# nonl4331/raytracing-rust

Hardware: AMD Instinct MI355X
Metric: Msamples/s on rtweekend1.ssml 1920x1080x1024spp (higher is better)
Workload: dtype f32

## Files before the change

### include/rt_hip.h

```cpp
#ifndef RT_HIP_H
#define RT_HIP_H

#include <stdint.h>

#ifdef __cplusplus
extern "C" {
#endif

#define RT_ABI_VERSION 2u

typedef enum rt_status {
	RT_OK = 0,
	RT_ERR_INVALID_ARGUMENT = -1,
	RT_ERR_NO_DEVICE = -2,
	RT_ERR_HIP = -3,
	RT_ERR_OUT_OF_MEMORY = -4,
	RT_ERR_UNSUPPORTED = -5
} rt_status;

typedef enum rt_texture_type {
	RT_TEX_CHECKERED = 0,
	RT_TEX_SOLID = 1,
	RT_TEX_IMAGE = 2,
	RT_TEX_LERP = 3,
// ... 113 lines not shown
	uint32_t max_depth;
	uint32_t rr_threshold;
	uint32_t shard_index;
	uint32_t shard_count;
	uint32_t tile_width;
	uint32_t tile_height;
	int32_t output_layout;
	uint32_t sample_split;
	uint32_t reserved0;
} rt_render_opts;

void rt_render_opts_default(rt_render_opts *opts);

typedef struct rt_hit_record {
	float t;
	float point[3];
	float error[3];
	float normal[3];
	float uv[2];
	int32_t has_uv;
	int32_t out;
	uint32_t material;
	uint32_t found;
	uint64_t index;
} rt_hit_record;

typedef struct rt_ray_desc {
	float origin[3];
	float direction[3];
} rt_ray_desc;

typedef struct rt_bvh_node {
	float min[3];
	float max[3];
	int64_t children[2];
	uint64_t primitive_offset;
	uint64_t number_primitives;
} rt_bvh_node;

typedef struct rt_scene rt_scene;

const char *rt_last_error(void);
uint32_t rt_abi_version(void);
int rt_device_count(void);

int rt_camera_new(rt_camera *out, const float origin[3], const float lookat[3], const float vup[3],
                  float fov_degrees, float aspect_ratio, float aperture, float focus_dist);

int rt_scene_create(const rt_scene_desc *desc, int device, rt_scene **out);
#define RT_DEVICE_NONE (-1)
void rt_scene_destroy(rt_scene *scene);

int rt_scene_create_multi(const rt_scene_desc *desc, const int *devices, uint32_t n_devices, rt_scene **out);
int rt_scene_device_count(const rt_scene *scene, uint32_t *n_devices);
typedef enum rt_gather_mode { RT_GATHER_NONE = 0, RT_GATHER_RCCL = 1, RT_GATHER_PEER = 2, RT_GATHER_PEER_STAGED = 3, RT_GATHER_SAME_DEVICE = 4 } rt_gather_mode;
int rt_scene_gather_info(const rt_scene *scene, int *mode, char *note, uint64_t note_capacity);
int rt_rccl_probe(int *usable, char *note, uint64_t note_capacity);
int rt_scene_auto_sample_split(const rt_scene *scene, const rt_render_opts *opts, uint32_t *split);

int rt_scene_counts(const rt_scene *scene, uint64_t *n_nodes, uint64_t *n_primitives, uint64_t *n_lights);
int rt_scene_get_nodes(const rt_scene *scene, rt_bvh_node *out, uint64_t capacity);
int rt_scene_get_primitive_order(const rt_scene *scene, uint64_t *out, uint64_t capacity);
int rt_scene_get_lights(const rt_scene *scene, uint64_t *out, uint64_t capacity);
int rt_scene_wide_info(const rt_scene *scene, uint64_t *n_wide_nodes, uint32_t *root_ref, uint32_t *stack_depth);
int rt_scene_get_wide_nodes(const rt_scene *scene, void *out, uint64_t capacity_nodes);
int rt_scene_get_leaf_boxes(const rt_scene *scene, float *out, uint64_t capacity_slots);
int rt_scene_get_wide_nodes_compact(const rt_scene *scene, void *out, uint64_t capacity_nodes);
int rt_scene_get_leaf_boxes_compact(const rt_scene *scene, float *out, uint64_t capacity_leaves, uint64_t *n_leaves);

typedef struct rt_sky_info {
	uint32_t res_x, res_y;
	uint32_t guide_k;
	uint32_t inv_res_ok;
	float inv_res_x, inv_res_y;
	uint64_t table_bytes;
} rt_sky_info;
int rt_scene_sky_info(const rt_scene *scene, rt_sky_info *info);
int rt_scene_get_sky_tables(const rt_scene *scene, float *row_cdf, uint64_t capacity_rows, float *marginal_cdf, uint64_t capacity_marginal,
                            uint8_t *guide, uint64_t capacity_guide);

int rt_scene_set_traversal(rt_scene *scene, int mode);
typedef enum rt_tuning_key { RT_TUNE_TRAVERSAL = 0, RT_TUNE_FEATURE_SET = 1, RT_TUNE_SCENE_IN_LDS = 2, RT_TUNE_SCHEDULE = 3, RT_TUNE_WALK = 4,
                             RT_TUNE_STACK_CAP = 5, RT_TUNE_EXCHANGE = 6, RT_TUNE_WHOLE_PIXEL_SHARE = 7, RT_TUNE_RADIANCE_GROUPS = 8,
                             RT_TUNE_SKY_RUN = 10 } rt_tuning_key;
int rt_scene_set_tuning(rt_scene *scene, int key, int value);
int rt_plan_work_items(const rt_render_opts *opts, uint32_t split, int share, uint64_t resident_waves, uint32_t *whole_claims,
                       uint64_t *n_items);

int rt_render(rt_scene *scene, const rt_camera *camera, const rt_render_opts *opts, float *out_rgb,
              uint64_t *rays_shot);

int rt_render_device(rt_scene *scene, const rt_camera *camera, const rt_render_opts *opts, float *d_out_rgb,
                     uint64_t *d_rays_shot, void *hip_stream);

int rt_render_output_floats(const rt_render_opts *opts, uint64_t *n_floats);
int rt_shard_pixel_order(const rt_render_opts *opts, uint64_t *out, uint64_t capacity);

typedef struct rt_sampler_progress {
	uint64_t samples_completed;
	uint64_t rays_shot;
	const float *current_image;
	uint64_t n_floats;
} rt_sampler_progress;
typedef int (*rt_presentation_update)(void *data, const rt_sampler_progress *progress, uint64_t samples_done);
int rt_sample_image(rt_scene *scene, const rt_camera *camera, const rt_render_opts *opts, uint64_t batch,
                    rt_presentation_update update, void *data);

int rt_last_kernel_ms(rt_scene *scene, float *ms, uint32_t *n_launches);

typedef struct rt_launch_info {
	int32_t method;
	int32_t pruned;
	int32_t fine;
	int32_t sky_in_lds;
	int32_t scene_in_lds;
	int32_t feature_set;
	uint32_t block_threads;
	uint32_t n_blocks;
	uint32_t blocks_per_cu;
	uint32_t waves_per_simd;
	uint32_t lds_bytes;
	uint32_t n_cus;
	uint32_t sample_split;
	uint32_t whole_claims;
	uint64_t n_items;
	uint32_t sky_run;
	uint32_t reserved;
	char kernel[152];
} rt_launch_info;
int rt_last_launch_info(const rt_scene *scene, rt_launch_info *out);

int rt_output_rgb8(const float *rgb, uint64_t n_values, float gamma, uint8_t *out);
int rt_output_save(const char *filename, const float *rgb, uint32_t width, uint32_t height, float gamma);

int rt_output_rgb8_device(rt_scene *scene, const float *d_rgb, uint64_t n_values, float gamma, uint8_t *d_out, void *hip_stream);
int rt_render_rgb8(rt_scene *scene, const rt_camera *camera, const rt_render_opts *opts, float gamma, uint8_t *out_rgb8,
                   uint64_t *rays_shot);

int rt_check_hit(rt_scene *scene, const rt_ray_desc *rays, uint64_t n_rays, rt_hit_record *out);
int rt_check_hit_index(rt_scene *scene, const rt_ray_desc *rays, const uint64_t *object_index, uint64_t n_rays,
                       rt_hit_record *out);

typedef struct rt_radiance_opts {
	uint64_t seed, sample_begin;
	uint32_t samples_per_ray;
	int32_t  render_method;
	uint32_t max_depth;
	uint32_t rr_threshold;
	uint32_t reserved[2];
} rt_radiance_opts;
int rt_radiance_opts_default(rt_radiance_opts *out);
int rt_radiance(rt_scene *scene, const rt_ray_desc *rays, const uint64_t *streams , uint64_t n_rays,
                const rt_radiance_opts *opts, float *out_rgb);
int rt_radiance_device(rt_scene *scene, const rt_ray_desc *d_rays, const uint64_t *d_streams , uint64_t n_rays,
                       const rt_radiance_opts *opts, float *d_out_rgb, void *hip_stream);

typedef struct rt_aov_buffers {
	float *albedo;
	float *normal;
	float *depth;
	float *coverage;
	uint32_t *primitive;
	uint32_t *material;
} rt_aov_buffers;
int rt_render_aov(rt_scene *scene, const rt_camera *camera, const rt_render_opts *opts, const rt_aov_buffers *host_out);
int rt_render_aov_device(rt_scene *scene, const rt_camera *camera, const rt_render_opts *opts, const rt_aov_buffers *device_out,
                         void *hip_stream);
// ... 266 lines not shown
	uint32_t reserved[6];
} rt_bloom_opts;
int rt_bloom_opts_default(rt_bloom_opts *out);
int rt_bloom_workspace_bytes(const rt_bloom_opts *opts, uint64_t *bytes);
int rt_bloom_device(rt_scene *scene, const float *d_rgb, const rt_bloom_opts *opts, const rt_display_state *d_state, void *d_workspace,
                    float *d_out, void *hip_stream);
int rt_bloom(rt_scene *scene, const float *host_rgb, const rt_bloom_opts *opts, const rt_display_state *host_state, float *host_out);

typedef struct rt_upscale_opts {
	uint32_t src_width, src_height;
	uint32_t dst_width, dst_height;
	float sigma_normal;
	float depth_tolerance;
	uint32_t reserved[8];
} rt_upscale_opts;
typedef struct rt_upscale_inputs {
	const float *color;
	const float *src_albedo, *src_normal, *src_depth;
	const float *dst_albedo, *dst_normal, *dst_depth;
} rt_upscale_inputs;
int rt_upscale_opts_default(rt_upscale_opts *out);
int rt_upscale_device(rt_scene *scene, const rt_upscale_inputs *device_in, const rt_upscale_opts *opts, float *d_out, uint8_t *d_stage,
                      void *hip_stream);
int rt_upscale(rt_scene *scene, const rt_upscale_inputs *host_in, const rt_upscale_opts *opts, float *host_out, uint8_t *host_stage);
int rt_render_upscaled(rt_scene *scene, const rt_camera *camera, const rt_render_opts *opts, uint32_t src_width, uint32_t src_height,
                       const rt_denoise_opts *dopts, const rt_upscale_opts *uopts, float *out, float *out_src, uint64_t *rays_shot);

int rt_selftest_division(float divisor, float *reciprocal, int *exact);

#define RT_SELFTEST_LEAN_CLASSES 9
int rt_selftest_lean(int device, uint64_t n_per_thread, uint64_t seed, uint64_t mismatches[RT_SELFTEST_LEAN_CLASSES]);

enum {
	RT_SHORT_FORM_RCP_REFINED = 0,
	RT_SHORT_FORM_INV_ONE_PAIR = 1,
	RT_SHORT_FORM_INV_TWO_PAIRS = 2,
	RT_SHORT_FORM_SQRT_RAW = 3,
	RT_SHORT_FORM_SQRT_BOTH = 4
};
#define RT_SHORT_FORMS 5
enum { RT_SHORT_SITE_RAY_NEW_PAIR = 0, RT_SHORT_SITE_RAY_NEW_FULL = 1 };
#define RT_SHORT_SITES 2
typedef struct rt_short_form_count {
	uint64_t tested;
	uint64_t mismatches;
	uint32_t first_mismatch;
	uint32_t reserved;
} rt_short_form_count;
typedef struct rt_short_forms_result {
	rt_short_form_count form[RT_SHORT_FORMS];
	uint64_t sqrt_raw_exact, sqrt_raw_high, sqrt_raw_low, sqrt_raw_other;
	uint64_t site_tested;
	uint64_t site_mismatches[RT_SHORT_SITES];
	uint32_t in_use;
	uint32_t reserved;
} rt_short_forms_result;
int rt_selftest_short_forms(int device, const float *operands, uint64_t n_operands, rt_short_forms_result *out);

enum { RT_DIV_FORM_ONE_PAIR = 0, RT_DIV_FORM_TWO_PAIRS = 1 };
#define RT_DIV_FORMS 2
enum { RT_DIV_SITE_FIX = 0, RT_DIV_SITE_DIV3_FIX = 1, RT_DIV_SITE_MIS_LIGHT_TERM = 2, RT_DIV_SITE_ATAN2 = 3 };
#define RT_DIV_SITES 4
typedef struct rt_div_forms_slice {
	const uint32_t *denominators;
	uint64_t n_denominators;
	uint32_t first_denominator;
	uint32_t reserved;
	const int32_t *exponents;
	uint64_t n_exponent_pairs;
} rt_div_forms_slice;
typedef struct rt_div_forms_result {
	uint64_t tested;
	uint64_t mismatches[RT_DIV_FORMS];
	uint32_t first_numerator[RT_DIV_FORMS];
	uint32_t first_denominator[RT_DIV_FORMS];
	uint64_t site_tested;
	uint64_t site_in_domain;
	uint64_t site_mismatches[RT_DIV_SITES];
	uint32_t in_use;
	uint32_t reserved;
} rt_div_forms_result;
int rt_selftest_div_forms(int device, const rt_div_forms_slice *slice, const float *operands, uint64_t n_operand_pairs, rt_div_forms_result *out);
int rt_selftest_sky_pdf_forms(rt_scene *scene, const float *dirs, uint64_t m, float *out_pdf_pair, float *out_pdf_default);

enum { RT_FRAME_FORMS_TESTED = 0, RT_FRAME_FORMS_FRAME_MISMATCHES = 1, RT_FRAME_FORMS_FRAME_SHORT = 2, RT_FRAME_FORMS_FRAME_PLAIN = 3,
       RT_FRAME_FORMS_RAY_MISMATCHES = 4, RT_FRAME_FORMS_RAY_SHORT = 5, RT_FRAME_FORMS_RAY_PLAIN = 6, RT_FRAME_FORMS_IN_USE = 7 };
#define RT_FRAME_FORMS_COUNTS 8
enum { RT_FRAME_FORM_FRAME_SHORT = 0, RT_FRAME_FORM_RAY_NORM_ONE_PAIR = 1 };
int rt_selftest_frame_forms(int device, const float *vectors, uint64_t n_vectors, uint64_t counts[RT_FRAME_FORMS_COUNTS]);

enum { RT_GEN_KEYS_TESTED = 0, RT_GEN_KEYS_STATE_MISMATCHES = 1, RT_GEN_KEYS_DRAW_MISMATCHES = 2, RT_GEN_KEYS_ITEM_STATE_MISMATCHES = 3,
       RT_GEN_KEYS_ITEM_DRAW_MISMATCHES = 4, RT_GEN_KEYS_ZERO_BLOCKS = 5, RT_GEN_KEYS_IN_USE = 6 };
#define RT_GEN_KEYS_COUNTS 7
#define RT_GEN_KEYS_CASE_WORDS 4
enum { RT_GEN_KEYS_FORM_TABLE = 0, RT_GEN_KEYS_FORM_ITEM_PRODUCT = 1 };
int rt_selftest_gen_keys(int device, uint64_t seed, const uint32_t *cases, uint64_t n_cases, uint64_t counts[RT_GEN_KEYS_COUNTS]);
void rt_philox_round_keys(uint64_t seed, uint32_t keys[20]);

enum { RT_PAIR_SHADOW_TESTED = 0, RT_PAIR_SHADOW_MISMATCHES = 1, RT_PAIR_SHADOW_ASKED_MISMATCHES = 2, RT_PAIR_SHADOW_ASKED = 3 };
#define RT_PAIR_SHADOW_COUNTS 4
#define RT_PAIR_SHADOW_CASE_FLOATS 10
int rt_selftest_pair_shadow(int device, const float *cases, uint64_t n_cases, uint64_t counts[RT_PAIR_SHADOW_COUNTS]);
enum { RT_PAIR_SHADOW_WALK_TESTED = 0, RT_PAIR_SHADOW_WALK_MISMATCHES = 1, RT_PAIR_SHADOW_WALK_ASKED = 2, RT_PAIR_SHADOW_WALK_ASKED_BOTH = 3,
       RT_PAIR_SHADOW_WALK_ASKED_WITH_OCCLUDED = 4 };
#define RT_PAIR_SHADOW_WALK_COUNTS 5
#define RT_PAIR_SHADOW_WALK_CASE_FLOATS 16
int rt_selftest_pair_shadow_walk(int device, const float *cases, uint64_t n_cases, uint64_t counts[RT_PAIR_SHADOW_WALK_COUNTS]);

int rt_selftest_pair_primary(rt_scene *scene, const float origin[3], uint32_t *valid, uint64_t *mismatches);

int rt_selftest_sky_tiles(rt_scene *scene, const rt_camera *camera, const rt_render_opts *opts, uint8_t *out_flags, uint64_t n_tiles);

int rt_selftest_sky(rt_scene *scene, int tables_in_lds, uint64_t seed, uint64_t n, float *out_dirs, float *out_pdf_of_sample,
                    const float *dirs, uint64_t m, float *out_pdf);

#ifdef __cplusplus
}
#endif
#endif
```

### raytracing-rust_amd/abi.py

```python
import ctypes as C

RT_ABI_VERSION = 2
RT_GATHER_NONE, RT_GATHER_RCCL, RT_GATHER_PEER, RT_GATHER_PEER_STAGED, RT_GATHER_SAME_DEVICE = 0, 1, 2, 3, 4

RT_OK = 0
RT_ERR_INVALID_ARGUMENT = -1
RT_ERR_NO_DEVICE = -2
RT_ERR_HIP = -3
RT_ERR_OUT_OF_MEMORY = -4
RT_ERR_UNSUPPORTED = -5

RT_TEX_CHECKERED, RT_TEX_SOLID, RT_TEX_IMAGE, RT_TEX_LERP, RT_TEX_PERLIN = range(5)
RT_MAT_EMIT, RT_MAT_LAMBERTIAN, RT_MAT_TROWBRIDGE_REITZ, RT_MAT_REFLECT, RT_MAT_REFRACT = range(5)
RT_PRIM_SPHERE, RT_PRIM_TRIANGLE, RT_PRIM_MESH_TRIANGLE = range(3)
RT_SPLIT_SAH, RT_SPLIT_MIDDLE, RT_SPLIT_EQUAL_COUNTS = range(3)
RT_METHOD_NAIVE, RT_METHOD_MIS = range(2)
RT_LAYOUT_FRAME, RT_LAYOUT_SHARD = range(2)
RT_TUNE_TRAVERSAL, RT_TUNE_FEATURE_SET, RT_TUNE_SCENE_IN_LDS, RT_TUNE_SCHEDULE, RT_TUNE_WALK, RT_TUNE_STACK_CAP, RT_TUNE_EXCHANGE, RT_TUNE_WHOLE_PIXEL_SHARE = range(8)
RT_TUNE_RADIANCE_GROUPS = 8
RT_TUNE_SKY_RUN = 10

NO_INDEX = 0xFFFFFFFFFFFFFFFF
RT_DEVICE_NONE = -1

f32x3 = C.c_float * 3


class TextureDesc(C.Structure):
    _fields_ = [
        ("type", C.c_int32),
        ("colour_one", f32x3),
        ("colour_two", f32x3),
        ("image_rgb", C.POINTER(C.c_float)),
        ("image_width", C.c_uint32),
        ("image_height", C.c_uint32),
        ("perlin_ran_vecs", C.POINTER(C.c_float)),
        ("perlin_perm", C.POINTER(C.c_uint32)),
    ]


class MaterialDesc(C.Structure):
    _fields_ = [
        ("type", C.c_int32),
        ("texture", C.c_uint32),
        ("param", C.c_float),
        ("ior", f32x3),
        ("metallic", C.c_float),
    ]


class _Sphere(C.Structure):
    _fields_ = [("centre", f32x3), ("radius", C.c_float)]


class _MeshTriangle(C.Structure):
    _fields_ = [("mesh", C.c_uint32), ("point_indices", C.c_uint32 * 3), ("normal_indices", C.c_uint32 * 3)]


class _Triangle(C.Structure):
    _fields_ = [("data", C.c_uint64)]


class _PrimUnion(C.Union):
    _fields_ = [("sphere", _Sphere), ("mesh_triangle", _MeshTriangle), ("triangle", _Triangle)]


class PrimitiveDesc(C.Structure):
    _fields_ = [("type", C.c_int32), ("material", C.c_uint32), ("u", _PrimUnion)]


class TriangleData(C.Structure):
    _fields_ = [("points", C.c_float * 9), ("normals", C.c_float * 9)]


class MeshDesc(C.Structure):
    _fields_ = [
        ("vertices", C.POINTER(C.c_float)),
        ("n_vertices", C.c_uint64),
        ("normals", C.POINTER(C.c_float)),
        ("n_normals", C.c_uint64),
    ]


class SkyDesc(C.Structure):
    _fields_ = [
        ("texture", C.c_uint32),
        ("material", C.c_uint32),
        ("sampler_res_x", C.c_uint32),
        ("sampler_res_y", C.c_uint32),
    ]


class SceneDesc(C.Structure):
    _fields_ = [
        ("abi_version", C.c_uint32),
        ("n_textures", C.c_uint32),
        ("textures", C.POINTER(TextureDesc)),
        ("n_materials", C.c_uint32),
        ("n_meshes", C.c_uint32),
        ("materials", C.POINTER(MaterialDesc)),
        ("meshes", C.POINTER(MeshDesc)),
        ("n_primitives", C.c_uint64),
# ... 523 lines not shown
    "rt_sampler_progress": (SamplerProgressC, 32),
    "rt_launch_info": (LaunchInfo, 224),
    "rt_sky_info": (SkyInfo, 32),
    "rt_aov_buffers": (AovBuffers, 48),
    "rt_aov_chain_opts": (AovChainOpts, 32),
    "rt_aov_chain_buffers": (AovChainBuffers, 56),
    "rt_matte_opts": (MatteOpts, 32),
    "rt_matte_buffers": (MatteBuffers, 24),
    "rt_ao_opts": (AoOpts, 32),
    "rt_ao_buffers": (AoBuffers, 16),
    "rt_radiance_opts": (RadianceOpts, 40),
    "rt_noise_opts": (NoiseOpts, 32),
    "rt_noise_summary": (NoiseSummary, 16),
    "rt_noise_buffers": (NoiseBuffers, 40),
    "rt_noise_result": (NoiseResult, 40),
    "rt_adaptive_result": (AdaptiveResult, 40),
    "rt_lens_camera": (LensCamera, 100),
    "rt_robust_opts": (RobustOpts, 32),
    "rt_robust_buffers": (RobustBuffers, 40),
    "rt_denoise_opts": (DenoiseOpts, 48),
    "rt_denoise_inputs": (DenoiseInputs, 40),
    "rt_temporal_opts": (TemporalOpts, 96),
    "rt_temporal_inputs": (TemporalInputs, 32),
    "rt_display_opts": (DisplayOpts, 104),
    "rt_display_state": (DisplayState, 16),
    "rt_bloom_opts": (BloomOpts, 64),
    "rt_dof_opts": (DofOpts, 64),
    "rt_upscale_opts": (UpscaleOpts, 56),
    "rt_upscale_inputs": (UpscaleInputs, 56),
    "rt_short_form_count": (ShortFormCount, 24),
    "rt_short_forms_result": (ShortFormsResult, 184),
    "rt_div_forms_slice": (DivFormsSlice, 40),
    "rt_div_forms_result": (DivFormsResult, 96),
}

EXPORTED_SYMBOLS = [
    "rt_last_error",
    "rt_abi_version",
    "rt_device_count",
    "rt_render_opts_default",
    "rt_camera_new",
    "rt_scene_create",
    "rt_scene_create_multi",
    "rt_scene_device_count",
    "rt_scene_destroy",
    "rt_scene_counts",
    "rt_scene_get_nodes",
    "rt_scene_get_primitive_order",
    "rt_scene_get_lights",
    "rt_scene_wide_info",
    "rt_scene_get_wide_nodes",
    "rt_scene_get_leaf_boxes",
    "rt_scene_get_wide_nodes_compact",
    "rt_scene_auto_sample_split",
    "rt_scene_gather_info",
    "rt_rccl_probe",
    "rt_selftest_division",
    "rt_scene_get_leaf_boxes_compact",
    "rt_scene_sky_info",
    "rt_scene_get_sky_tables",
    "rt_scene_set_traversal",
    "rt_scene_set_tuning",
    "rt_render",
    "rt_sample_image",
    "rt_render_device",
    "rt_render_output_floats",
    "rt_shard_pixel_order",
    "rt_plan_work_items",
    "rt_last_kernel_ms",
    "rt_last_launch_info",
    "rt_output_rgb8",
    "rt_output_save",
    "rt_output_rgb8_device",
    "rt_render_rgb8",
    "rt_check_hit",
    "rt_check_hit_index",
    "rt_radiance_opts_default",
    "rt_radiance",
    "rt_radiance_device",
    "rt_selftest_lean",
    "rt_selftest_short_forms",
    "rt_selftest_div_forms",
    "rt_selftest_sky_pdf_forms",
    "rt_selftest_frame_forms",
    "rt_selftest_gen_keys",
    "rt_philox_round_keys",
    "rt_selftest_pair_shadow",
    "rt_selftest_pair_shadow_walk",
    "rt_selftest_pair_primary",
    "rt_selftest_sky_tiles",
    "rt_selftest_sky",
    "rt_render_aov",
    "rt_render_aov_device",
    "rt_aov_chain_opts_default",
    "rt_render_aov_chain",
    "rt_render_aov_chain_device",
    "rt_matte_opts_default",
    "rt_render_matte",
    "rt_render_matte_device",
    "rt_matte_extract",
    "rt_matte_extract_device",
    "rt_ao_opts_default",
    "rt_render_ao",
    "rt_render_ao_device",
    "rt_denoise_opts_default",
    "rt_denoise_workspace_bytes",
    "rt_denoise",
    "rt_denoise_device",
    "rt_render_denoised",
    "rt_noise_opts_default",
    "rt_render_noise",
    "rt_render_noise_device",
    "rt_noise_tiles",
    "rt_noise_tiles_device",
    "rt_render_converged",
    "rt_render_denoised_split",
    "rt_render_adaptive",
    "rt_render_tiles",
    "rt_render_tiles_device",
    "rt_noise_select_tiles",
    "rt_noise_select_tiles_device",
    "rt_lens_camera_new",
    "rt_render_lens",
    "rt_render_lens_device",
    "rt_robust_opts_default",
    "rt_render_robust",
    "rt_render_robust_device",
    "rt_robust_combine",
    "rt_robust_combine_device",
    "rt_render_denoised_robust",
    "rt_temporal_opts_default",
    "rt_temporal_history_bytes",
    "rt_temporal_workspace_bytes",
    "rt_denoise_temporal_device",
    "rt_denoise_temporal",
    "rt_denoise_temporal_reset",
    "rt_display_opts_default",
    "rt_display_workspace_bytes",
    "rt_display_output_bytes",
    "rt_display_device",
    "rt_display",
    "rt_display_reset",
    "rt_bloom_opts_default",
    "rt_bloom_workspace_bytes",
    "rt_bloom_device",
    "rt_bloom",
    "rt_dof_opts_default",
    "rt_dof_opts_from_camera",
    "rt_dof_workspace_bytes",
    "rt_dof_device",
    "rt_dof",
    "rt_render_dof",
    "rt_upscale_opts_default",
    "rt_upscale_device",
    "rt_upscale",
    "rt_render_upscaled",
]


def channels(table, struct):
    out = {}
    for name, shape in table.items():
        if isinstance(shape, dict):
            out.update(channels(shape, getattr(struct, name)))
        else:
            out[name] = (struct, dict(struct._fields_)[name]._type_, shape)
# ... 56 lines not shown
```

### raytracing-rust_amd/csrc/rt_api.cpp

```cpp
#include <hip/hip_runtime.h>

#include <cstdio>
#include <cstdlib>
#include <algorithm>
#include <cmath>
#include <cstring>
#include <string>
#include <vector>

#include "../../include/rt_hip.h"
#include "../../include/rt_detmath.h"
#include <dlfcn.h>
#include "rt_api_internal.h"
#include "rt_render.h"

using namespace rt;

thread_local std::string g_error;

constexpr uint32_t kFineAboveTriangles = 4096;
constexpr uint32_t kFineAboveSpheres = 32768;

struct RcclApi {
	void *lib = nullptr;
// ... 204 lines not shown
				return bail(rc);
		}
	}
	if ((rc = upload(s, h.dev_nodes.data(), h.dev_nodes.size(), &D.nodes)) != RT_OK) return bail(rc);
	if (!h.dev_nodes4.empty()) {
		if ((rc = upload(s, h.dev_nodes4c.data(), h.dev_nodes4c.size(), &D.nodes4)) != RT_OK) return bail(rc);
		if ((rc = upload(s, h.leaf_box_c.data(), h.leaf_box_c.size(), &D.leaf_box)) != RT_OK) return bail(rc);
	}
	if ((rc = upload(s, h.dev_prims.data(), h.dev_prims.size(), &D.prims)) != RT_OK) return bail(rc);
	if ((rc = upload(s, h.dev_shade.data(), h.dev_shade.size(), &D.shade)) != RT_OK) return bail(rc);
	if ((rc = upload(s, h.prim_rank.data(), h.prim_rank.size(), &D.prim_rank)) != RT_OK) return bail(rc);
	if (&h == &s->host && h.primitive_order.size() < 0xFFFFFFFFull) {
		std::vector<uint32_t> desc(h.primitive_order.size());
		for (size_t i = 0; i < desc.size(); ++i)
			desc[i] = (uint32_t)h.primitive_order[i];
		const uint32_t *d_desc = nullptr;
		if ((rc = upload(s, desc.data(), desc.size(), &d_desc)) != RT_OK) return bail(rc);
		s->d_prim_desc = const_cast<uint32_t *>(d_desc);
	}
	{
		const uint32_t *d_big = nullptr;
		if ((rc = upload(s, h.big_leaves.data(), h.big_leaves.size(), &d_big)) != RT_OK) return bail(rc);
		D.big_leaves = reinterpret_cast<const uint2 *>(d_big);
	}
	if ((rc = upload(s, h.materials.data(), h.materials.size(), &D.materials)) != RT_OK) return bail(rc);
	if ((rc = upload(s, textures.data(), textures.size(), &D.textures)) != RT_OK) return bail(rc);
	if ((rc = upload(s, h.dev_lights.data(), h.dev_lights.size(), &D.lights)) != RT_OK) return bail(rc);
	const float *d_sky = nullptr;
	if ((rc = upload(s, h.sky_cdf.data(), h.sky_cdf.size(), &d_sky)) != RT_OK) return bail(rc);
	const uint8_t *d_guide = nullptr;
	if ((rc = upload(s, h.sky_guide.data(), h.sky_guide.size(), &d_guide)) != RT_OK) return bail(rc);
	{
		auto pad16 = [](size_t n) { return (n + 15) & ~(size_t)15; };
		const size_t sizes[8] = {h.dev_nodes.size() * sizeof(DevNode),      h.dev_prims.size() * sizeof(DevPrim),
		                         h.dev_shade.size() * sizeof(DevShade),     h.prim_rank.size() * 4,
		                         h.materials.size() * sizeof(DevMaterial),  textures.size() * sizeof(DevTexture),
		                         h.dev_lights.size() * 4,                   h.big_leaves.size() * 4};
		const void *srcs[8] = {h.dev_nodes.data(), h.dev_prims.data(), h.dev_shade.data(), h.prim_rank.data(),
		                       h.materials.data(), textures.data(),  h.dev_lights.data(), h.big_leaves.data()};
		size_t total = 0;
		for (int i = 0; i < 8; ++i) {
			blob_off[i] = (uint32_t)total;
			total += pad16(sizes[i]);
		}
		if (total <= 12 * 1024) {
			blob.assign(total / 4, 0u);
			for (int i = 0; i < 8; ++i)
				if (sizes[i])
					std::memcpy(reinterpret_cast<char *>(blob.data()) + blob_off[i], srcs[i], sizes[i]);
			if ((rc = upload(s, blob.data(), blob.size(), &D.blob)) != RT_OK) return bail(rc);
			D.blob_bytes = (uint32_t)total;
			D.off_nodes = blob_off[0]; D.off_prims = blob_off[1]; D.off_shade = blob_off[2]; D.off_rank = blob_off[3];
			D.off_materials = blob_off[4]; D.off_textures = blob_off[5]; D.off_lights = blob_off[6]; D.off_big_leaves = blob_off[7];
		}
	}

	D.n_nodes = (uint32_t)h.dev_nodes.size();
	D.n_prims = (uint32_t)h.dev_prims.size();
	D.n_lights = (uint32_t)h.dev_lights.size();
	D.n_materials = (uint32_t)h.materials.size();
	D.n_textures = (uint32_t)h.textures.size();
	D.root_ref = h.root_ref;
	D.root4_ref = h.root4_ref;
	D.n_nodes4 = (uint32_t)h.dev_nodes4.size();
	std::memcpy(D.root_min, h.root_min, sizeof D.root_min);
	std::memcpy(D.root_max, h.root_max, sizeof D.root_max);
	D.stack_depth = h.stack_depth;
	s->stack_depth_narrow = h.stack_depth_narrow;
	D.has_triangles = h.has_triangles ? 1u : 0u;
	D.single_light = h.dev_lights.size() == 1 ? h.dev_lights[0] : kNoPrim;
	D.sky.texture = h.sky.texture;
	D.sky.material = mat_handle_make(h.sky.material, h.materials[h.sky.material].type, h.materials[h.sky.material].tex_type);
	D.sky.res_x = h.sky.sampler_res_x;
	D.sky.res_y = h.sky.sampler_res_y;
	D.sky.row_cdf = d_sky;
	D.sky.marginal_cdf = d_sky + (size_t)h.sky.sampler_res_y * (h.sky.sampler_res_x + 1u);
	D.sky.guide = h.sky_guide_k ? d_guide : nullptr;
	D.sky.guide_k = h.sky_guide_k;
	{
		float rc_pi = 0.0f, rc_tau = 0.0f;
		if (!verified_reciprocal(RT_PI, &rc_pi) || !verified_reciprocal(RT_TAU, &rc_tau) || rc_pi != 1.0f / RT_PI || rc_tau != 1.0f / RT_TAU)
			return bail(fail(RT_ERR_UNSUPPORTED, "self-check failed: division by pi / 2 pi through their reciprocals is not exact on this host (the kernels assume it)"));
		sky_reciprocals(h.sky, &D.sky.inv_res_ok, &D.sky.inv_res_x, &D.sky.inv_res_y);
		bool tame = true;
		for (const DevMaterial &m : h.materials) {
			if (m.type != RT_MAT_LAMBERTIAN)
				continue;
			tame = tame && m.tex_type == RT_TEX_SOLID;
			for (int k = 0; k < 3; ++k) {
				const float pr = std::fabs(m.tex_c1[k] * m.param);
				tame = tame && (pr == 0.0f || (pr >= 0x1p-30f && pr <= 0x1p30f));
			}
		}
		for (const DevShade &sh : h.dev_shade)
			for (int k = 0; k < 3; ++k)
				tame = tame && std::fabs(sh.n0[k]) <= 0x1p20f && std::fabs(sh.n1[k]) <= 0x1p20f && std::fabs(sh.n2[k]) <= 0x1p20f;
		D.lambert_tame = tame ? 1u : 0u;
	}

	void *p = nullptr;
	if (hipMalloc(&p, sizeof(uint32_t)) != hipSuccess) return bail(fail(RT_ERR_OUT_OF_MEMORY, "hipMalloc work counter"));
	s->allocations.push_back(p);
	s->d_work_counter = static_cast<uint32_t *>(p);
	if (hipMalloc(&p, sizeof(unsigned long long)) != hipSuccess) return bail(fail(RT_ERR_OUT_OF_MEMORY, "hipMalloc rays"));
	s->allocations.push_back(p);
	s->d_rays = static_cast<unsigned long long *>(p);
	if (hipStreamCreate(&s->stream) != hipSuccess) return bail(fail(RT_ERR_HIP, "hipStreamCreate failed"));
	if (hipEventCreate(&s->ev_start) != hipSuccess || hipEventCreate(&s->ev_stop) != hipSuccess)
		return bail(fail(RT_ERR_HIP, "hipEventCreate failed"));
	{
		bool cmat = false, ctex = false;
		for (const DevMaterial &m : h.materials)
			cmat = cmat || (m.type != RT_MAT_EMIT && m.type != RT_MAT_LAMBERTIAN);
		for (const DevTexture &t : textures)
			ctex = ctex || (t.type != RT_TEX_SOLID && t.type != RT_TEX_LERP);
		if (cmat || ctex)
			s->feature_set = 2;
		else if (h.has_triangles || !h.lights.empty())
			s->feature_set = 1;
		else
			s->feature_set = 0;
		s->min_feature_set = s->feature_set;
		if (h.dev_nodes.size() == 1 && (h.root_ref & kLeafFlag) == 0u) {
			const DevNode &n0 = h.dev_nodes[0];
			s->pair_tree = (n0.c0 & kLeafFlag) && (n0.c1 & kLeafFlag) && ((n0.c0 >> 26) & 31u) == 1u && ((n0.c1 >> 26) & 31u) == 1u;
			for (const DevPrim &q : h.dev_prims) {
				uint32_t meta;
				std::memcpy(&meta, &q.a[3], sizeof meta);
				const DevMaterial &m = h.materials[mat_handle_index(meta >> 2)];
				s->pair_tree = s->pair_tree && m.type == RT_MAT_LAMBERTIAN && m.tex_type == RT_TEX_SOLID;
			}
			s->pair_tree = s->pair_tree && h.materials[h.sky.material].type == RT_MAT_EMIT;
			s->pair_tree = s->pair_tree && D.lambert_tame != 0u;
			for (const DevPrim &q : h.dev_prims)
				s->pair_tree = s->pair_tree && q.b[1] != 0.0f;
			if (s->pair_tree) {
				DevPairScene &q = s->pair;
				std::memcpy(q.c0min, n0.c0min, sizeof q.c0min); std::memcpy(q.c0max, n0.c0max, sizeof q.c0max);
				std::memcpy(q.c1min, n0.c1min, sizeof q.c1min); std::memcpy(q.c1max, n0.c1max, sizeof q.c1max);
				q.slot0 = n0.c0 & kLeafSlotMask;
				q.slot1 = n0.c1 & kLeafSlotMask;
				q.rank0 = h.prim_rank[q.slot0];
				q.rank1 = h.prim_rank[q.slot1];
				const uint32_t slots[2] = {q.slot0, q.slot1};
				for (int k = 0; k < 2; ++k) {
					const DevPrim &pr = h.dev_prims[slots[k]];
					uint32_t meta;
					std::memcpy(&meta, &pr.a[3], sizeof meta);
					const DevMaterial &m = h.materials[mat_handle_index(meta >> 2)];
					q.sphere[k][0] = pr.a[0]; q.sphere[k][1] = pr.a[1]; q.sphere[k][2] = pr.a[2]; q.sphere[k][3] = pr.b[0];
					q.lambert[k][0] = m.tex_c1[0]; q.lambert[k][1] = m.tex_c1[1]; q.lambert[k][2] = m.tex_c1[2]; q.lambert[k][3] = m.param;
				}
				q.inv_radius[0] = h.dev_prims[q.slot0].b[1];
				q.inv_radius[1] = h.dev_prims[q.slot1].b[1];
				const DevMaterial &sky = h.materials[h.sky.material];
				q.sky_param = sky.param;
				q.sky_tex_type = sky.tex_type;
				std::memcpy(q.sky_c1, sky.tex_c1, sizeof q.sky_c1);
				std::memcpy(q.sky_c2, sky.tex_c2, sizeof q.sky_c2);
			}
		}
	}
	if (const char *e = std::getenv("RT_HIP_TRAVERSAL")) {
		if (std::strcmp(e, "exhaustive") == 0) s->traversal_mode = 0;
		if (std::strcmp(e, "pruned") == 0) s->traversal_mode = 1;
	}
// ... 202 lines not shown
	}
	return RT_OK;
}

int rt_scene_device_count(const rt_scene *s, uint32_t *n_devices)
{
	if (!s || !n_devices)
		return fail(RT_ERR_INVALID_ARGUMENT, "null argument");
	*n_devices = s->device == RT_DEVICE_NONE ? 0u : (uint32_t)(1 + s->peers.size());
	return RT_OK;
}

int rt_scene_set_traversal(rt_scene *s, int mode)
{
	if (!s || mode < -1 || mode > 1)
		return fail(RT_ERR_INVALID_ARGUMENT, "bad arguments");
	s->traversal_mode = mode;
	for (rt_scene *m : s->peers)
		m->traversal_mode = mode;
	return RT_OK;
}

static int set_tuning_one(rt_scene *s, int key, int value);
int rt_scene_set_tuning(rt_scene *s, int key, int value)
{
	if (!s)
		return fail(RT_ERR_INVALID_ARGUMENT, "null scene");
	const int rc = set_tuning_one(s, key, value);
	for (rt_scene *m : s->peers)
		if (rc == RT_OK) {
			(void)set_tuning_one(m, key, value);
		}
	return rc;
}
static int set_tuning_one(rt_scene *s, int key, int value)
{
	switch (key) {
	case RT_TUNE_TRAVERSAL:
		return rt_scene_set_traversal(s, value);
	case RT_TUNE_FEATURE_SET:
		if (value < s->min_feature_set || value > 2)
			return fail(RT_ERR_INVALID_ARGUMENT, "feature set must be between the scene's own and 2");
		s->feature_set = value;
		s->feature_set_forced = true;
		return RT_OK;
	case RT_TUNE_SCHEDULE:
		if (value < -1 || value > 1)
			return fail(RT_ERR_INVALID_ARGUMENT, "schedule must be -1, 0 or 1");
		s->schedule_mode = value;
		return RT_OK;
	case RT_TUNE_SCENE_IN_LDS:
		s->scene_lds_allowed = value != 0;
		return RT_OK;
	case RT_TUNE_STACK_CAP:
		if (value < 0 || value > 96)
			return fail(RT_ERR_INVALID_ARGUMENT, "stack cap must be 0 (automatic) or 1..96 entries");
		s->stack_cap_override = (uint32_t)value;
		return RT_OK;
	case RT_TUNE_EXCHANGE:
		if (value < 0 || value > 1)
			return fail(RT_ERR_INVALID_ARGUMENT, "exchange must be 0 (off) or 1 (on where the kernel has it)");
		s->exchange_mode = value;
		return RT_OK;
	case RT_TUNE_WHOLE_PIXEL_SHARE:
		if (value < -1 || value > 16)
			return fail(RT_ERR_INVALID_ARGUMENT, "whole-pixel share must be -1 (automatic) or 0..16 (sixteenths of a shard's tiles)");
		s->whole_share = value;
		return RT_OK;
	case RT_TUNE_WALK:
		if (value < 0 || value > 1)
			return fail(RT_ERR_INVALID_ARGUMENT, "walk must be 0 (automatic) or 1 (two-child walk for every ray)");
		s->dev.narrow_only = (uint32_t)value;
		return RT_OK;
	case RT_TUNE_RADIANCE_GROUPS:
		if (value < 0 || value > 65536)
			return fail(RT_ERR_INVALID_ARGUMENT, "radiance groups must be 0 (automatic) or 1..65536 workgroups");
		s->radiance_groups = (uint32_t)value;
		return RT_OK;
	case RT_TUNE_SKY_RUN:
		if (value < -1 || value > 1)
			return fail(RT_ERR_INVALID_ARGUMENT, "sky run must be -1 (automatic), 0 (off) or 1 (on where the kernel has it)");
		s->sky_run = value;
		return RT_OK;
	default:
		return fail(RT_ERR_INVALID_ARGUMENT, "unknown tuning key");
	}
}

int rt_scene_counts(const rt_scene *s, uint64_t *n_nodes, uint64_t *n_primitives, uint64_t *n_lights)
{
	if (!s)
		return fail(RT_ERR_INVALID_ARGUMENT, "null scene");
	if (n_nodes) *n_nodes = s->host.nodes.size();
	if (n_primitives) *n_primitives = s->host.primitive_order.size();
	if (n_lights) *n_lights = s->host.lights.size();
	return RT_OK;
}
int rt_scene_get_nodes(const rt_scene *s, rt_bvh_node *out, uint64_t capacity)
{
	if (!s || !out || capacity < s->host.nodes.size())
		return fail(RT_ERR_INVALID_ARGUMENT, "bad arguments");
	for (size_t i = 0; i < s->host.nodes.size(); ++i) {
		const HostNode &n = s->host.nodes[i];
		std::memcpy(out[i].min, n.min, 12);
		std::memcpy(out[i].max, n.max, 12);
		out[i].children[0] = n.child[0];
		out[i].children[1] = n.child[1];
		out[i].primitive_offset = n.primitive_offset;
		out[i].number_primitives = n.number_primitives;
	}
	return RT_OK;
}
int rt_scene_get_primitive_order(const rt_scene *s, uint64_t *out, uint64_t capacity)
{
	if (!s || !out || capacity < s->host.primitive_order.size())
		return fail(RT_ERR_INVALID_ARGUMENT, "bad arguments");
	std::memcpy(out, s->host.primitive_order.data(), s->host.primitive_order.size() * sizeof(uint64_t));
	return RT_OK;
}
int rt_scene_wide_info(const rt_scene *s, uint64_t *n_wide_nodes, uint32_t *root_ref, uint32_t *stack_depth)
{
	if (!s)
		return fail(RT_ERR_INVALID_ARGUMENT, "null scene");
	if (n_wide_nodes) *n_wide_nodes = s->host.dev_nodes4.size();
	if (root_ref) *root_ref = s->host.root4_ref;
	if (stack_depth) *stack_depth = s->host.stack_depth;
	return RT_OK;
}
int rt_scene_get_wide_nodes(const rt_scene *s, void *out, uint64_t capacity_nodes)
{
	if (!s || !out || capacity_nodes < s->host.dev_nodes4.size())
		return fail(RT_ERR_INVALID_ARGUMENT, "bad arguments");
	std::memcpy(out, s->host.dev_nodes4.data(), s->host.dev_nodes4.size() * sizeof(DevNodeQ4));
	return RT_OK;
}
int rt_scene_get_leaf_boxes(const rt_scene *s, float *out, uint64_t capacity_slots)
{
	if (!s || !out || capacity_slots < s->host.leaf_box.size())
		return fail(RT_ERR_INVALID_ARGUMENT, "bad arguments");
	std::memcpy(out, s->host.leaf_box.data(), s->host.leaf_box.size() * sizeof(DevLeafBox));
	return RT_OK;
}
int rt_scene_get_wide_nodes_compact(const rt_scene *s, void *out, uint64_t capacity_nodes)
{
	if (!s || !out || capacity_nodes < s->host.dev_nodes4c.size())
		return fail(RT_ERR_INVALID_ARGUMENT, "bad arguments");
	std::memcpy(out, s->host.dev_nodes4c.data(), s->host.dev_nodes4c.size() * sizeof(DevNodeQ4));
	return RT_OK;
}
int rt_scene_get_leaf_boxes_compact(const rt_scene *s, float *out, uint64_t capacity_leaves, uint64_t *n_leaves)
{
	if (!s)
		return fail(RT_ERR_INVALID_ARGUMENT, "null scene");
	if (n_leaves)
		*n_leaves = s->host.leaf_box_c.size();
	if (!out)
		return n_leaves ? RT_OK : fail(RT_ERR_INVALID_ARGUMENT, "bad arguments");
	if (capacity_leaves < s->host.leaf_box_c.size())
		return fail(RT_ERR_INVALID_ARGUMENT, "bad arguments");
	std::memcpy(out, s->host.leaf_box_c.data(), s->host.leaf_box_c.size() * sizeof(DevLeafBox));
	return RT_OK;
}
int rt_scene_sky_info(const rt_scene *s, rt_sky_info *info)
{
	if (!s || !info)
		return fail(RT_ERR_INVALID_ARGUMENT, "null argument");
// ... 540 lines not shown
				if (head->gather_mode == RT_GATHER_RCCL)
					HIP_TRY(hipStreamWaitEvent(stream, members[m]->ev_shard, 0));
				HIP_TRY(hipMemcpyPeerAsync(head->d_gather_rays + m, head->device, members[m]->d_member_rays, members[m]->device, sizeof(unsigned long long), stream));
			}
		}
		HIP_TRY(launch_sum_u64(stream, head->d_gather_rays, n, reinterpret_cast<unsigned long long *>(d_rays_shot)));
	}
	if (!capturing) {
		HIP_TRY(hipEventRecord(head->ev_gathered, stream));
		head->gathered_once = true;
	}
	return RT_OK;
}

int rt_render_device(rt_scene *s, const rt_camera *camera, const rt_render_opts *o, float *d_out_rgb, uint64_t *d_rays_shot,
                     void *hip_stream)
{
	if (!s || !camera || !o || !d_out_rgb)
		return fail(RT_ERR_INVALID_ARGUMENT, "null argument");
	if (!s->peers.empty() && !s->member_call) {
		if (s->device == RT_DEVICE_NONE)
			return fail(RT_ERR_NO_DEVICE, "host-only scene");
		return render_device_multi(s, camera, o, d_out_rgb, d_rays_shot, static_cast<hipStream_t>(hip_stream));
	}
	ShardGeometry g;
	int rc = shard_geometry(o, g);
	if (rc != RT_OK)
		return rc;
	if (s->device == RT_DEVICE_NONE)
		return fail(RT_ERR_NO_DEVICE, "host-only scene (RT_DEVICE_NONE): rendering needs a GPU, there is no CPU fallback");
	if (o->render_method != RT_METHOD_NAIVE && o->render_method != RT_METHOD_MIS)
		return fail(RT_ERR_INVALID_ARGUMENT, "unknown render method");
	if (o->samples_per_pixel == 0 || o->samples_per_pixel >= (1ull << 32))
		return fail(RT_ERR_INVALID_ARGUMENT, "samples_per_pixel must be in [1, 2^32)");
	if (o->output_layout != RT_LAYOUT_FRAME && o->output_layout != RT_LAYOUT_SHARD)
		return fail(RT_ERR_INVALID_ARGUMENT, "unknown output layout");
	HIP_TRY(hipSetDevice(s->device));
	hipStream_t stream = static_cast<hipStream_t>(hip_stream);
	if (g.n_work == 0) {
		HIP_TRY(launch_reset(stream, s->d_work_counter, reinterpret_cast<unsigned long long *>(d_rays_shot), d_out_rgb,
		                     o->output_layout == RT_LAYOUT_FRAME ? (size_t)(o->width * o->height * 3) : 0));
		s->timed = false;
		return RT_OK;
	}

	RenderLaunchPlan plan;
	rc = plan_render_launch(s, o, g, &plan);
	if (rc != RT_OK)
		return rc;
	const DevRenderParams &P = plan.P;
	float *render_target = d_out_rgb;
	if (plan.split > 1u) {
		const size_t need = (size_t)g.n_work * plan.split * 3;
		rc = grow_device_buffer(s->d_partial, s->partial_floats, need);
		if (rc != RT_OK)
			return rc;
		render_target = s->d_partial;
	}
	if (P.stack_ovf_depth != 0u) {
		const size_t need = (size_t)plan.n_blocks * plan.block_threads * P.stack_ovf_depth;
		rc = grow_device_buffer(s->d_stack_ovf, s->stack_ovf_words, need);
		if (rc != RT_OK)
			return rc;
	}
	{
		size_t zero_floats = 0;
		if (o->output_layout == RT_LAYOUT_FRAME && o->shard_count > 1)
			zero_floats = (size_t)(o->width * o->height * 3);
		if (o->output_layout == RT_LAYOUT_SHARD)
			zero_floats = (size_t)(g.n_work * 3);
		HIP_TRY(launch_reset(stream, s->d_work_counter, reinterpret_cast<unsigned long long *>(d_rays_shot), d_out_rgb, zero_floats));
	}
	fill_launch_info(plan, o, s->n_cus, &s->last_launch);
	const bool sky_run = sky_run_applies(s, plan.feature_set, g.n_work, P.tile_log2_w != 0xFFFFFFFFu);
	s->last_launch.sky_run = sky_run ? 1u : 0u;
	const DevCamera cam = dev_camera(camera);
	DevPairPrimary primary{};
	if (plan.feature_set == 3)
		pair_primary_terms(s->pair, plan.dev.root_min, plan.dev.root_max, v3(cam.origin[0], cam.origin[1], cam.origin[2]), primary);
	const DevSkyTiles sky_tiles = sky_tiles_block(s, primary, cam, (uint32_t)o->width, (uint32_t)o->height, sky_run);
	HIP_TRY(hipEventRecord(s->ev_start, stream));
	HIP_TRY(launch_render(o->render_method, plan.prune, plan.fine, plan.sky_lds, plan.feature_set, plan.n_blocks, plan.lds_bytes, stream, plan.dev, cam, P,
	                      render_target, reinterpret_cast<unsigned long long *>(d_rays_shot), s->d_work_counter, s->d_stack_ovf, plan.xchg,
	                      plan.feature_set == 3 ? &s->pair : nullptr, plan.feature_set == 3 ? &primary : nullptr, plan.block_threads, sky_tiles));
	HIP_TRY(hipEventRecord(s->ev_stop, stream));
	if (plan.split > 1u)
		HIP_TRY(launch_combine(stream, P, s->d_partial, d_out_rgb));
	s->timed = true;
	s->n_launches = 1;
	return RT_OK;
}

int rt_render(rt_scene *s, const rt_camera *camera, const rt_render_opts *o, float *out_rgb, uint64_t *rays_shot)
{
	if (!s || !camera || !o)
		return fail(RT_ERR_INVALID_ARGUMENT, "null argument");
	if (int rc = need_device(s); rc != RT_OK)
		return rc;
	uint64_t n_floats = 0;
	int rc = rt_render_output_floats(o, &n_floats);
	if (rc != RT_OK)
		return rc;
	if (n_floats == 0) {
		if (rays_shot)
			*rays_shot = 0;
		return RT_OK;
	}
	if (!out_rgb)
		return fail(RT_ERR_INVALID_ARGUMENT, "null argument");
	HIP_TRY(hipSetDevice(s->device));
	rc = ensure_frame_buffers(s, n_floats, false);
	if (rc != RT_OK)
		return rc;
	float *d_out = s->d_prog[0];
	rc = rt_render_device(s, camera, o, d_out, reinterpret_cast<uint64_t *>(s->d_rays), s->stream);
	if (rc != RT_OK)
		return rc;
	Staging st{s};
	st.download(out_rgb, d_out, n_floats * sizeof(float));
	st.download(rays_shot, s->d_rays, sizeof(uint64_t));
	return st.finish("render");
}

int rt_output_rgb8_device(rt_scene *s, const float *d_rgb, uint64_t n_values, float gamma, uint8_t *d_out, void *hip_stream)
{
	if (!s || !d_rgb || !d_out)
		return fail(RT_ERR_INVALID_ARGUMENT, "null argument");
	if (s->device == RT_DEVICE_NONE)
		return fail(RT_ERR_NO_DEVICE, "host-only scene (RT_DEVICE_NONE): this call needs a GPU (rt_output_rgb8 is the host-side conversion)");
	if (n_values == 0)
		return RT_OK;
	HIP_TRY(hipSetDevice(s->device));
	HIP_TRY(launch_quantise(static_cast<hipStream_t>(hip_stream), d_rgb, (size_t)n_values, 1.0f / gamma, d_out));
	return RT_OK;
}

int rt_render_rgb8(rt_scene *s, const rt_camera *camera, const rt_render_opts *o, float gamma, uint8_t *out_rgb8, uint64_t *rays_shot)
{
	if (!s || !camera || !o)
		return fail(RT_ERR_INVALID_ARGUMENT, "null argument");
	if (int rc = need_device(s); rc != RT_OK)
		return rc;
	uint64_t n_values = 0;
	int rc = rt_render_output_floats(o, &n_values);
	if (rc != RT_OK)
		return rc;
	if (n_values == 0) {
		if (rays_shot)
			*rays_shot = 0;
		return RT_OK;
	}
	if (!out_rgb8)
		return fail(RT_ERR_INVALID_ARGUMENT, "null argument");
	HIP_TRY(hipSetDevice(s->device));
	rc = ensure_frame_buffers(s, n_values, false);
	if (rc != RT_OK)
		return rc;
	rc = grow_device_buffer(s->d_rgb8, s->d_rgb8_bytes, (size_t)n_values);
	if (rc != RT_OK)
		return rc;
	float *d_frame = s->d_prog[0];
	rc = rt_render_device(s, camera, o, d_frame, reinterpret_cast<uint64_t *>(s->d_rays), s->stream);
	if (rc != RT_OK)
		return rc;
	Staging st{s};
	st.e = launch_quantise(s->stream, d_frame, (size_t)n_values, 1.0f / gamma, s->d_rgb8);
	st.download(out_rgb8, s->d_rgb8, n_values);
// ... 116 lines not shown
```

### raytracing-rust_amd/csrc/rt_api_internal.h

```cpp
#pragma once
#include <hip/hip_runtime.h>

#include <cstdint>
#include <cstring>
#include <string>
#include <vector>

#include "../../include/rt_hip.h"
#include "rt_build.h"
#include "rt_layout.h"
#include "rt_types.h"
#include "rt_sky_tiles.h"

extern thread_local std::string g_error;

inline int fail(int code, const std::string &msg)
{
	g_error = msg;
	return code;
}
inline int hip_fail(hipError_t e, const char *what)
{
	g_error = std::string(what) + ": " + hipGetErrorString(e);
	return e == hipErrorOutOfMemory ? RT_ERR_OUT_OF_MEMORY : RT_ERR_HIP;
}
#define HIP_TRY(expr)                       \
	do {                                    \
		hipError_t e_ = (expr);             \
		if (e_ != hipSuccess)               \
			return hip_fail(e_, #expr);     \
	} while (0)
#define RT_TRY(expr)            \
	do {                        \
		const int rc_ = (expr); \
		if (rc_ != RT_OK)       \
			return rc_;         \
	} while (0)

constexpr uint32_t kPruneAbove = 100;

constexpr int kWholeShareDefault = -1;

struct rt_scene {
	int device = 0;
	rt::HostScene host;
	rt::DevScene dev{};
	std::vector<void *> allocations;
	hipStream_t stream = nullptr;
	uint32_t *d_work_counter = nullptr;
	unsigned long long *d_rays = nullptr;
	hipEvent_t ev_start = nullptr, ev_stop = nullptr;
	bool timed = false;
	uint32_t n_launches = 0;
	int n_cus = 0;
	int traversal_mode = -1;
	int schedule_mode = -1;
	int feature_set = 2;
	int min_feature_set = 0;
	bool pair_tree = false, feature_set_forced = false;
	rt::DevPairScene pair{};
	bool scene_lds_allowed = true;
	float *d_partial = nullptr;
	size_t partial_floats = 0;
	float *d_prog[2] = {nullptr, nullptr};
	float *h_prog[2] = {nullptr, nullptr};
	unsigned long long *d_prog_rays = nullptr;
	unsigned long long *h_prog_rays = nullptr;
	size_t d_prog_floats[2] = {0, 0}, h_prog_floats[2] = {0, 0};
	hipStream_t copy_stream = nullptr;
	hipEvent_t ev_batch[2] = {nullptr, nullptr}, ev_copy[2] = {nullptr, nullptr};
	size_t max_lds = 65536;
	rt_launch_info last_launch{};
	uint32_t stack_cap_override = 0;
	int exchange_mode = 0;
	int whole_share = kWholeShareDefault;
	uint32_t radiance_groups = 0;
	int sky_run = -1;
	uint32_t stack_depth_narrow = 2;
	uint32_t *d_stack_ovf = nullptr;
	size_t stack_ovf_words = 0;
	uint8_t *d_rgb8 = nullptr;
	size_t d_rgb8_bytes = 0;
	std::vector<rt_scene *> peers;
	bool member_call = false;
	float *d_shard = nullptr;
	size_t shard_floats = 0;
	unsigned long long *d_member_rays = nullptr;
	hipEvent_t ev_shard = nullptr;
	hipEvent_t ev_begin = nullptr;
	float *d_gather = nullptr;
	size_t gather_floats = 0;
	unsigned long long *d_gather_rays = nullptr;
	void *nccl_comms = nullptr;
	int gather_mode = 0;
	std::string gather_note;
	hipEvent_t ev_gathered = nullptr;
	bool gathered_once = false;
	uint32_t *d_prim_desc = nullptr;
	char *d_denoise = nullptr;
	size_t d_denoise_bytes = 0;
	char *d_temporal = nullptr;
	uint32_t temporal_w = 0, temporal_h = 0;
	int temporal_cur = -1;
	rt_camera temporal_prev{};
	char *d_display = nullptr;
	size_t d_display_bytes = 0;
	uint32_t display_w = 0, display_h = 0;
	bool display_has_state = false;
	char *d_noise = nullptr;
	size_t d_noise_bytes = 0;
	char *d_bloom = nullptr;
	size_t d_bloom_bytes = 0;
	char *d_dof = nullptr;
	size_t d_dof_bytes = 0;
};

uint32_t auto_sample_split(int n_cus, uint64_t frame_pixels, uint64_t spp, uint32_t n_sharers);
struct WorkItems { uint64_t whole_claims, n_items; };
WorkItems plan_work_items(uint64_t tiles, uint64_t tile_pixels, uint32_t split, bool tiled, int share, uint64_t resident_waves);

constexpr size_t kSkyLdsLimit = 96 * 1024;
inline size_t sky_table_bytes(uint32_t res_x, uint32_t res_y, uint32_t guide_k)
{
	if ((res_x | res_y) == 0u)
		return 0;
	return ((size_t)res_y * (res_x + 1u) + res_y + 1u) * 4 + (size_t)(res_y + 1u) * guide_k;
}

inline bool scene_prunes(const rt_scene *s)
{
	return s->traversal_mode == -1 ? s->dev.n_prims > kPruneAbove : s->traversal_mode == 1;
}

inline int four_wave_traversal(const rt_scene *s, bool *prune, rt::DevScene *dev)
{
	*prune = scene_prunes(s);
	*dev = s->dev;
	const bool walks_wide = *prune && dev->nodes4 != nullptr && dev->narrow_only == 0u;
	if (!walks_wide || rt::four_wave_stack_lds_bytes(*dev) > s->max_lds) {
		if (walks_wide)
			dev->narrow_only = 1u;
		dev->stack_depth = s->stack_depth_narrow;
	}
	if (rt::four_wave_stack_lds_bytes(*dev) > s->max_lds)
		return fail(RT_ERR_UNSUPPORTED, "traversal stacks exceed the LDS of one CU");
	return RT_OK;
}

inline uint32_t path_lane_groups(const rt_scene *s, size_t lds_bytes, uint32_t waves, uint64_t wanted)
{
	const uint64_t by_lds = std::max<uint64_t>(1, (160u * 1024u) / std::max<size_t>(1, lds_bytes));
	const uint64_t resident = (uint64_t)std::max(1, s->n_cus) * std::min<uint64_t>(waves, by_lds);
	uint64_t groups = std::min<uint64_t>(wanted, resident);
	if (s->radiance_groups != 0u)
		groups = std::min<uint64_t>(groups, s->radiance_groups);
	return (uint32_t)std::max<uint64_t>(groups, 1);
}


struct TileGrid { uint32_t tiles_x; uint64_t count; };
// ... 144 lines not shown
```

### raytracing-rust_amd/csrc/rt_api_query.cpp

```cpp
#include <hip/hip_runtime.h>

#include <algorithm>
#include <cstring>
#include <vector>

#include "../../include/rt_hip.h"
#include "rt_api_internal.h"
#include "rt_query.h"
#include "rt_radiance.h"
#include "rt_selftest.h"
#include "rt_gen_keys.h"

using namespace rt;

#ifdef RT_STATS
extern "C" int rt_debug_trace_queue(rt_scene *s, const rt_ray_desc *rays, uint64_t n, int waves, uint32_t cap, float *out_t, uint32_t *out_prim,
                                    float *ms, unsigned long long *node_steps)
{
	if (!s || !rays || !out_t || !out_prim || n == 0 || n >= (1ull << 31) || s->device == RT_DEVICE_NONE || s->dev.nodes4 == nullptr)
		return fail(RT_ERR_INVALID_ARGUMENT, "bad arguments (or no wide tree)");
	HIP_TRY(hipSetDevice(s->device));
	cap = std::min(std::max(cap, 1u), s->dev.stack_depth);
	const uint32_t ovf_depth = s->dev.stack_depth - cap;
	const uint32_t n_blocks = (uint32_t)s->n_cus * (uint32_t)waves;
// ... 304 lines not shown
	out->in_use = short_forms_in_use();
	return RT_OK;
}

int rt_selftest_div_forms(int device, const rt_div_forms_slice *slice, const float *operands, uint64_t n_operand_pairs, rt_div_forms_result *out)
{
	if (!out || (slice != nullptr) == (operands != nullptr))
		return fail(RT_ERR_INVALID_ARGUMENT, "bad arguments (a slice or operands, not both)");
	if (operands && (n_operand_pairs == 0 || n_operand_pairs > (1ull << 20)))
		return fail(RT_ERR_INVALID_ARGUMENT, "bad arguments (1 to 2^20 operand pairs)");
	if (slice) {
		if (!slice->exponents || slice->n_denominators == 0 || slice->n_exponent_pairs == 0 || slice->n_denominators > (1ull << 17) ||
		    slice->n_exponent_pairs > (1ull << 17) || slice->n_denominators * slice->n_exponent_pairs > (1ull << 17))
			return fail(RT_ERR_INVALID_ARGUMENT, "bad slice (n_denominators * n_exponent_pairs in [1, 2^17])");
		if (!slice->denominators && (uint64_t)slice->first_denominator + slice->n_denominators > (1ull << 23))
			return fail(RT_ERR_INVALID_ARGUMENT, "bad slice (the range leaves the 2^23 significands)");
		for (uint64_t k = 0; k < 2 * slice->n_exponent_pairs; ++k)
			if (slice->exponents[k] < -126 || slice->exponents[k] > 127)
				return fail(RT_ERR_INVALID_ARGUMENT, "bad slice (binary exponents in [-126, 127])");
	}
	unsigned long long host[kDivCounts] = {};
	for (int k = 0; k < RT_DIV_FORMS; ++k)
		host[kDivCountFirst + k] = ~0ull;
	if (operands) {
		RT_TRY(run_cases(device, operands, (size_t)n_operand_pairs * 2 * sizeof(float), host, kDivCounts, "selftest_div_forms",
		                 [&](unsigned long long *d, void *d_pairs) { return launch_div_sites(nullptr, static_cast<const float *>(d_pairs), n_operand_pairs, d); }));
	} else {
		const uint64_t n_den = slice->denominators ? slice->n_denominators : 0, n_exp = 2 * slice->n_exponent_pairs;
		std::vector<uint32_t> tail(n_exp + n_den);
		std::memcpy(tail.data(), slice->exponents, n_exp * sizeof(int32_t));
		if (n_den)
			std::memcpy(tail.data() + n_exp, slice->denominators, n_den * sizeof(uint32_t));
		RT_TRY(run_cases(device, tail.data(), tail.size() * sizeof(uint32_t), host, kDivCounts, "selftest_div_forms", [&](unsigned long long *d, void *d_tail) {
			DevDivForms D;
			D.exponents = static_cast<const int32_t *>(d_tail);
			D.n_exponent_pairs = (uint32_t)slice->n_exponent_pairs;
			D.denominators = n_den ? static_cast<const uint32_t *>(d_tail) + n_exp : nullptr;
			D.n_denominators = (uint32_t)slice->n_denominators;
			D.first_denominator = slice->first_denominator;
			D.counts = d;
			return launch_div_forms(nullptr, D);
		}));
	}
	std::memset(out, 0, sizeof *out);
	out->tested = host[kDivCountTested];
	for (int k = 0; k < RT_DIV_FORMS; ++k) {
		out->mismatches[k] = host[kDivCountBad + k];
		if (slice && out->mismatches[k]) {
			const unsigned long long index = host[kDivCountFirst + k];
			const uint64_t pair_index = index >> 23, ep = pair_index / slice->n_denominators, j = pair_index - ep * slice->n_denominators;
			const uint32_t d_sig = (slice->denominators ? slice->denominators[j] : slice->first_denominator + (uint32_t)j) & 0x007FFFFFu;
			out->first_numerator[k] = (uint32_t)(127 + slice->exponents[2 * ep]) << 23 | ((uint32_t)index & 0x007FFFFFu);
			out->first_denominator[k] = (uint32_t)(127 + slice->exponents[2 * ep + 1]) << 23 | d_sig;
		}
	}
	out->site_tested = host[kDivCountSiteTested];
	out->site_in_domain = host[kDivCountSiteInDomain];
	for (int k = 0; k < RT_DIV_SITES; ++k)
		out->site_mismatches[k] = host[kDivCountSiteBad + k];
	out->in_use = div_forms_in_use();
	return RT_OK;
}

int rt_selftest_sky_pdf_forms(rt_scene *s, const float *dirs, uint64_t m, float *out_pdf_pair, float *out_pdf_default)
{
	if (!s || !dirs || !out_pdf_pair || !out_pdf_default || m == 0 || m > (1ull << 24))
		return fail(RT_ERR_INVALID_ARGUMENT, "bad arguments (1 to 2^24 directions)");
	if ((s->host.sky.sampler_res_x | s->host.sky.sampler_res_y) == 0u)
		return fail(RT_ERR_INVALID_ARGUMENT, "the sky is not samplable (sampler_res 0 x 0)");
	if (int rc = need_device(s); rc != RT_OK)
		return rc;
	Layout L;
	const auto p_dirs = L.add<float>(3 * m), p_pair = L.add<float>(m), p_default = L.add<float>(m);
	RT_TRY(sky_buffer(s, L));
	Staging st{s};
	st.put(L, p_dirs, dirs);
	if (st.ok())
		st.e = launch_sky_pdf_forms(s->stream, s->dev, L.at(p_dirs), m, L.at(p_pair), L.at(p_default));
	st.get(out_pdf_pair, L, p_pair);
	st.get(out_pdf_default, L, p_default);
	return sky_finish(st, L, "selftest_sky_pdf_forms");
}

int rt_selftest_pair_shadow(int device, const float *cases, uint64_t n_cases, uint64_t counts[RT_PAIR_SHADOW_COUNTS])
{
	return run_case_table<RT_PAIR_SHADOW_COUNTS>(device, cases, n_cases, RT_PAIR_SHADOW_CASE_FLOATS * sizeof(float), counts, "selftest_pair_shadow",
	                                             launch_pair_shadow);
}
int rt_selftest_pair_shadow_walk(int device, const float *cases, uint64_t n_cases, uint64_t counts[RT_PAIR_SHADOW_WALK_COUNTS])
{
	return run_case_table<RT_PAIR_SHADOW_WALK_COUNTS>(device, cases, n_cases, RT_PAIR_SHADOW_WALK_CASE_FLOATS * sizeof(float), counts,
	                                                  "selftest_pair_shadow_walk", launch_pair_shadow_walk);
}
int rt_selftest_frame_forms(int device, const float *vectors, uint64_t n_vectors, uint64_t counts[RT_FRAME_FORMS_COUNTS])
{
	RT_TRY(run_case_table<RT_FRAME_FORMS_COUNTS>(device, vectors, n_vectors, 3 * sizeof(float), counts, "selftest_frame_forms", launch_frame_forms));
	counts[RT_FRAME_FORMS_IN_USE] = frame_forms_in_use();
	return RT_OK;
}
int rt_selftest_gen_keys(int device, uint64_t seed, const uint32_t *cases, uint64_t n_cases, uint64_t counts[RT_GEN_KEYS_COUNTS])
{
	RT_TRY(run_case_table<RT_GEN_KEYS_COUNTS>(device, cases, n_cases, RT_GEN_KEYS_CASE_WORDS * sizeof(uint32_t), counts, "selftest_gen_keys",
	                                          [seed](hipStream_t stream, const uint32_t *d_cases, uint64_t n, unsigned long long *d_counts) {
		                                          return launch_gen_keys(stream, seed, d_cases, n, d_counts);
	                                          }));
	counts[RT_GEN_KEYS_IN_USE] = gen_keys_in_use();
	return RT_OK;
}

void rt_philox_round_keys(uint64_t seed, uint32_t keys[20])
{
	if (!keys)
		return;
	DevGenKeys K;
	philox_round_keys(seed, K);
	for (int r = 0; r < 10; ++r) {
		keys[2 * r] = K.key[r][0];
		keys[2 * r + 1] = K.key[r][1];
	}
}

int rt_selftest_pair_primary(rt_scene *s, const float origin[3], uint32_t *valid, uint64_t *mismatches)
{
	if (!s || !origin || !valid || !mismatches)
		return fail(RT_ERR_INVALID_ARGUMENT, "null argument");
	if (int rc = need_device(s); rc != RT_OK)
		return rc;
	if (!s->pair_tree)
		return fail(RT_ERR_UNSUPPORTED, "not a scene the two-sphere kernels take");
	DevPairPrimary host{};
	pair_primary_terms(s->pair, s->dev.root_min, s->dev.root_max, v3(origin[0], origin[1], origin[2]), host);
	unsigned long long bad = 0;
	RT_TRY(run_cases(s->device, nullptr, 0, &bad, 1, "selftest_pair_primary", [&](unsigned long long *d, void *) {
		return launch_selftest_pair_primary(nullptr, s->pair, s->dev.root_min, s->dev.root_max, origin, host, d);
	}));
	*valid = host.valid;
	*mismatches = bad;
	return RT_OK;
}

int rt_selftest_sky_tiles(rt_scene *s, const rt_camera *camera, const rt_render_opts *o, uint8_t *out_flags, uint64_t n_tiles)
{
	if (!s || !camera || !o || !out_flags)
		return fail(RT_ERR_INVALID_ARGUMENT, "null argument");
	if (int rc = need_device(s); rc != RT_OK)
		return rc;
	if (o->width < 2 || o->height < 2 || o->width >= 65536 || o->height >= 65536)
		return fail(RT_ERR_INVALID_ARGUMENT, "width and height must be in [2, 65536)");
	const FrameTiling t = frame_tiling(o);
	if (n_tiles != (uint64_t)t.tiles_x * t.tiles_y)
		return fail(RT_ERR_INVALID_ARGUMENT, "n_tiles must be the tiles of the frame the options describe");
	std::memset(out_flags, 0, (size_t)n_tiles);
	uint32_t log2_w = 0;
	while (log2_w < 7u && (1u << log2_w) != t.tile_w)
		++log2_w;
	if (!s->pair_tree || t.tile_w * t.tile_h != 64u || log2_w >= 7u)
		return RT_OK;
	const DevCamera cam = dev_camera(camera);
	DevPairPrimary primary{};
	pair_primary_terms(s->pair, s->dev.root_min, s->dev.root_max, v3(cam.origin[0], cam.origin[1], cam.origin[2]), primary);
	const DevSkyTiles block = sky_tiles_block(s, primary, cam, (uint32_t)o->width, (uint32_t)o->height, true);
	std::vector<unsigned long long> words((size_t)((n_tiles + 7u) / 8u), 0ull);
	RT_TRY(run_cases(s->device, nullptr, 0, words.data(), words.size(), "selftest_sky_tiles", [&](unsigned long long *d, void *) {
		return launch_sky_tiles(nullptr, block, (uint32_t)o->width, (uint32_t)o->height, log2_w, t.tiles_x, n_tiles, reinterpret_cast<uint8_t *>(d));
	}));
	std::memcpy(out_flags, words.data(), (size_t)n_tiles);
// ... 5 lines not shown
```

### raytracing-rust_amd/csrc/rt_lean.h

```cpp
#pragma once

#include "rt_vec.h"

namespace rt {


RT_FN void lean_sincos(float x, float &s, float &c)
{
	const float k = rintf(x * 0.636619746685028076172f);
	float r = fmaf(-k, 1.57079637050628662109f, x);
	r = fmaf(-k, -4.37113882867379282984e-08f, r);
	r = fmaf(-k, -1.71512451000588185479e-15f, r);
	const int q = (int)k;
	const float sk = rt_sin_kernel(r), ck = rt_cos_kernel(r);
	const bool odd = (q & 1) != 0;
	const float sv = odd ? ck : sk;
	const float cv = odd ? sk : ck;
	s = (q & 2) ? -sv : sv;
	c = ((q + 1) & 2) ? -cv : cv;
}

RT_FN float lean_acos_with(float x, float sqrt_half_one_minus_abs)
{
	const bool big = fabsf(x) > 0.5f;
	const float k = rt_asin_kernel(big ? sqrt_half_one_minus_abs : x);
	const float two_k = 2.0f * k;
	return big ? (x > 0.0f ? two_k : RT_PI - two_k) : RT_FRAC_PI_2 - k;
}
RT_FN float lean_acos(float x) { return lean_acos_with(x, sqrtf(0.5f * (1.0f - fabsf(x)))); }

RT_FN float lean_atan_unit_with(float t, float q)
{
	const bool upper = t > 0.414213567972183227539f;
	const float u = upper ? q : t;
	const float z = u * u;
	float p = fmaf(8.05374449538e-2f, z, -1.38776856032e-1f);
	p = fmaf(p, z, 1.99777106478e-1f);
	p = fmaf(p, z, -3.33329491539e-1f);
	return (upper ? RT_FRAC_PI_4 : 0.0f) + fmaf(p * z, u, u);
}
template <class DivA, class DivB> RT_FN float lean_atan2_with(float y, float x, DivA div_ratio, DivB div_octant)
{
	const float ax = fabsf(x), ay = fabsf(y);
	const bool swap = ay > ax;
	const float t = div_ratio(swap ? ax : ay, swap ? ay : ax);
	const float a = lean_atan_unit_with(t, div_octant(t - 1.0f, t + 1.0f));
	float r = swap ? RT_FRAC_PI_2 - a : a;
	r = (ax == ay) ? RT_FRAC_PI_4 : r;
	r = (ax == 0.0f && ay == 0.0f) ? 0.0f : r;
	if (rt_f32_bits(x) & 0x80000000u)
		r = RT_PI - r;
	r = (rt_f32_bits(y) & 0x80000000u) ? -r : r;
	return (x != x || y != y) ? x + y : r;
}
RT_FN float lean_atan2_portable(float y, float x)
{
	return lean_atan2_with(y, x, [](float n, float d) { return n / d; }, [](float n, float d) { return n / d; });
}

RT_FN float div_by_verified(float x, float c, float rc)
{
	const float q0 = x * rc;
	const float e = fmaf(-c, q0, x);
	return fmaf(e, rc, q0);
}
constexpr float kRcpPi = 1.0f / RT_PI, kRcpTau = 1.0f / RT_TAU;

enum class LeanInvForm { two_pairs, refined };
constexpr LeanInvForm lean_inv_form(bool pair) { return pair ? LeanInvForm::refined : LeanInvForm::two_pairs; }
enum class LeanDivForm { two_pairs, one_pair };
constexpr LeanDivForm lean_div_form(bool pair) { return pair ? LeanDivForm::one_pair : LeanDivForm::two_pairs; }
#ifndef RT_PAIR_RAY_NORM_SHORT
#define RT_PAIR_RAY_NORM_SHORT 1
#endif
#ifndef RT_PAIR_FRAME_SHORT
#define RT_PAIR_FRAME_SHORT 1
#endif
constexpr bool lean_ray_norm_short(bool pair) { return pair && RT_PAIR_RAY_NORM_SHORT != 0; }
enum class LeanFrameForm { plain, guarded_short };
constexpr LeanFrameForm lean_frame_form(bool pair) { return pair && RT_PAIR_FRAME_SHORT != 0 ? LeanFrameForm::guarded_short : LeanFrameForm::plain; }
#ifndef RT_PAIR_GEN_KEYS
#define RT_PAIR_GEN_KEYS 0
#endif
#ifndef RT_PAIR_GEN_ITEM_PRODUCT
#define RT_PAIR_GEN_ITEM_PRODUCT 0
#endif
constexpr bool lean_gen_keys(bool pair) { return pair && RT_PAIR_GEN_KEYS != 0; }
constexpr int lean_gen_keys_lead(bool pair) { return lean_gen_keys(pair) ? RT_PAIR_GEN_KEYS - 1 : 0; }
constexpr bool lean_gen_item_product(bool pair) { return lean_gen_keys(pair) && RT_PAIR_GEN_ITEM_PRODUCT != 0; }

#if defined(__HIP_DEVICE_COMPILE__)

__device__ __forceinline__ float lean_rcp_refined(float d)
{
	const float r0 = __builtin_amdgcn_rcpf(d);
	const float e = __builtin_fmaf(-d, r0, 1.0f);
	return __builtin_fmaf(e, r0, r0);
}
__device__ __forceinline__ float lean_div_core(float n, float d, float r1)
{
	const float q0 = n * r1;
	const float e1 = __builtin_fmaf(-d, q0, n);
	const float q1 = __builtin_fmaf(e1, r1, q0);
	const float e2 = __builtin_fmaf(-d, q1, n);
	return __builtin_fmaf(e2, r1, q1);
}
__device__ __forceinline__ float lean_div(float n, float d) { return lean_div_core(n, d, lean_rcp_refined(d)); }
__device__ __forceinline__ float lean_div_fix(float n, float d)
{
	return __builtin_amdgcn_div_fixupf(lean_div_core(n, d, lean_rcp_refined(d)), d, n);
}
__device__ __forceinline__ float lean_inv(float d)
{
	const float r1 = lean_rcp_refined(d);
	const float e1 = __builtin_fmaf(-d, r1, 1.0f);
	const float q1 = __builtin_fmaf(e1, r1, r1);
	const float e2 = __builtin_fmaf(-d, q1, 1.0f);
	return __builtin_fmaf(e2, r1, q1);
}
__device__ __forceinline__ float lean_inv_gfx950(float d) { return lean_rcp_refined(d); }
template <bool PAIR> __device__ __forceinline__ float lean_inv_for(float d)
{
	return lean_inv_form(PAIR) == LeanInvForm::refined ? lean_inv_gfx950(d) : lean_inv(d);
}
__device__ __forceinline__ V3 lean_div3(V3 v, float d)
{
	const float r1 = lean_rcp_refined(d);
	return V3{lean_div_core(v.x, d, r1), lean_div_core(v.y, d, r1), lean_div_core(v.z, d, r1)};
}
__device__ __forceinline__ V3 lean_div3_fix(V3 v, float d)
{
	const float r1 = lean_rcp_refined(d);
	return V3{__builtin_amdgcn_div_fixupf(lean_div_core(v.x, d, r1), d, v.x), __builtin_amdgcn_div_fixupf(lean_div_core(v.y, d, r1), d, v.y),
	          __builtin_amdgcn_div_fixupf(lean_div_core(v.z, d, r1), d, v.z)};
}

__device__ __forceinline__ float lean_div_core_gfx950(float n, float d, float r1)
{
	const float q0 = n * r1;
	const float e = __builtin_fmaf(-d, q0, n);
	return __builtin_fmaf(e, r1, q0);
}
template <bool PAIR> __device__ __forceinline__ float lean_div_core_for(float n, float d, float r1)
{
	return lean_div_form(PAIR) == LeanDivForm::one_pair ? lean_div_core_gfx950(n, d, r1) : lean_div_core(n, d, r1);
}
template <bool PAIR> __device__ __forceinline__ float lean_div_for(float n, float d) { return lean_div_core_for<PAIR>(n, d, lean_rcp_refined(d)); }
template <bool PAIR> __device__ __forceinline__ float lean_div_fix_for(float n, float d)
{
	return __builtin_amdgcn_div_fixupf(lean_div_core_for<PAIR>(n, d, lean_rcp_refined(d)), d, n);
}
template <bool PAIR> __device__ __forceinline__ V3 lean_div3_for(V3 v, float d)
{
	const float r1 = lean_rcp_refined(d);
	return V3{lean_div_core_for<PAIR>(v.x, d, r1), lean_div_core_for<PAIR>(v.y, d, r1), lean_div_core_for<PAIR>(v.z, d, r1)};
}
template <bool PAIR> __device__ __forceinline__ V3 lean_div3_fix_for(V3 v, float d)
{
	const float r1 = lean_rcp_refined(d);
	return V3{__builtin_amdgcn_div_fixupf(lean_div_core_for<PAIR>(v.x, d, r1), d, v.x), __builtin_amdgcn_div_fixupf(lean_div_core_for<PAIR>(v.y, d, r1), d, v.y),
	          __builtin_amdgcn_div_fixupf(lean_div_core_for<PAIR>(v.z, d, r1), d, v.z)};
}

__device__ __forceinline__ float lean_sqrt(float x)
{
	const float s = __builtin_amdgcn_sqrtf(x);
	const float s_dn = __uint_as_float(__float_as_uint(s) - 1u);
	const float s_up = __uint_as_float(__float_as_uint(s) + 1u);
	const float r_dn = __builtin_fmaf(-s_dn, s, x);
	const float r_up = __builtin_fmaf(-s_up, s, x);
	float r = (r_dn <= 0.0f) ? s_dn : s;
	r = (r_up > 0.0f) ? s_up : r;
// ... 38 lines not shown
```

### raytracing-rust_amd/csrc/rt_render.h

```cpp
#pragma once
#include <hip/hip_runtime.h>
#include "rt_types.h"
#include "rt_sky_tiles.h"

namespace rt {
size_t render_lds_bytes(const DevScene &S, bool sky_lds, bool scene_lds, uint32_t waves_per_block, uint32_t stack_cap);
uint32_t render_waves_per_simd(int feature_set, bool fine);
uint32_t render_block_threads(int feature_set, bool fine, bool xchg = false);
uint32_t render_max_block_threads(int feature_set, bool fine, bool xchg);
hipError_t render_occupancy(int method, bool prune, bool fine, bool sky_lds, int feature_set, size_t lds_bytes, int *blocks_per_cu, bool xchg,
                            uint32_t block_threads = 0);
bool render_exchange_available(int method, bool prune, bool fine, int feature_set);
size_t render_exchange_lds_bytes(uint32_t slots);
uint32_t render_exchange_max_slots();
size_t render_exchange_fine_lds_bytes(uint32_t waves_per_block);

hipError_t launch_reset(hipStream_t stream, uint32_t *work_counter, unsigned long long *rays_shot, float *out, size_t n_out_floats);
hipError_t launch_render(int method, bool prune, bool fine, bool sky_lds, int feature_set, uint32_t n_blocks, size_t lds_bytes, hipStream_t stream,
                         const DevScene &S, const DevCamera &cam, const DevRenderParams &P, float *out,
                         unsigned long long *rays_shot, uint32_t *work_counter, uint32_t *stack_ovf, bool xchg, const DevPairScene *pair,
                         const DevPairPrimary *primary, uint32_t block_threads, const DevSkyTiles &sky_tiles);
hipError_t launch_combine(hipStream_t stream, const DevRenderParams &P, const float *partial, float *out);
hipError_t launch_scatter_shard(hipStream_t stream, const DevRenderParams &P, const float *shard, float *frame);
hipError_t launch_sum_u64(hipStream_t stream, const unsigned long long *parts, uint32_t n, unsigned long long *out);
hipError_t launch_quantise(hipStream_t stream, const float *rgb, size_t n_values, float inv_gamma, uint8_t *out);
}
```

### raytracing-rust_amd/csrc/rt_render.hip

```cpp
#include "rt_shade.h"
#include "rt_gen_keys.h"
#include "rt_sky_tiles.h"
#include "rt_render.h"

namespace rt {

enum : int {
	PH_GEN = 0,
	PH_NODE = 1,
	PH_LEAF = 2,
	PH_SHADE = 3,
	PH_LIGHT = 4,
	PH_SCATTER = 5,
	PH_NARROW = 6,
	PH_COUNT = 7,
	PH_NEED_PIXEL = 7,
	PH_DONE = 8,
	PH_WALK = 9
};

#ifndef RT_PQ_SPLIT
#define RT_PQ_SPLIT 1
#endif
#ifndef RT_LIGHT_PHASE_THRESHOLD
// ... 37 lines not shown
#endif
#ifndef RT_FUSE_REGIONS
#define RT_FUSE_REGIONS(spheres_only) true
#endif
#ifndef RT_BODY_ALWAYS
#define RT_BODY_ALWAYS(spheres_only) true
#endif
#ifndef RT_SPHERES_MAX_BLOCK
#define RT_SPHERES_MAX_BLOCK 768
#endif
#ifndef RT_PAIR_WAVES
#define RT_PAIR_WAVES 6
#endif
#ifndef RT_SPHERES_WAVES
#define RT_SPHERES_WAVES 4
#endif
#ifndef RT_SPHERES_COARSE_WAVES
#define RT_SPHERES_COARSE_WAVES 6
#endif

__device__ __forceinline__ float power_heuristic(float pdf_a, float pdf_b)
{
	const float a_sq = pdf_a * pdf_a;
	return a_sq / (a_sq + pdf_b * pdf_b);
}

__device__ __forceinline__ bool work_to_pixel(const DevRenderParams &P, uint32_t w, uint32_t &x, uint32_t &y)
{
	const uint32_t tile_pixels = P.tile_w * P.tile_h;
	const uint32_t k = w / tile_pixels;
	const uint32_t in = w - k * tile_pixels;
	const uint32_t tile = P.shard_index + k * P.shard_count;
	const uint32_t ty = tile / P.tiles_x;
	const uint32_t tx = tile - ty * P.tiles_x;
	x = tx * P.tile_w + in % P.tile_w;
	y = ty * P.tile_h + in / P.tile_w;
	return x < P.width && y < P.height;
}

template <class F, bool FINE = false, bool XCHG = false> struct KernelShape {
	static constexpr bool spheres_only = !(F::tri || F::lights || F::cmat || F::ctex);
	static constexpr bool simple = !spheres_only && !(F::cmat || F::ctex);
	static constexpr int waves_per_simd = (F::cmat || F::ctex) ? (FINE ? RT_FULL_FINE_WAVES : (XCHG ? 3 : RT_FULL_WAVES))
	                                      : (F::pair ? RT_PAIR_WAVES : (spheres_only ? ((FINE || XCHG) ? RT_SPHERES_WAVES : RT_SPHERES_COARSE_WAVES)
	                                                                                 : (FINE ? RT_SIMPLE_FINE_WAVES : (XCHG ? 4 : RT_SIMPLE_COARSE_WAVES))));
	static constexpr int block = (FINE && XCHG) ? 512 : (spheres_only ? RT_SPHERES_BLOCK : ((simple && !FINE) ? RT_SIMPLE_COARSE_BLOCK : 256));
	static constexpr int max_block = ((spheres_only || simple) && !FINE && !XCHG && block == 512) ? RT_SPHERES_MAX_BLOCK : block;
};

#ifdef RT_STATS
#define RT_SECTION(k) do { const unsigned long long now_ = wall_clock64(); st_sect[(k)] += now_ - st_mark; st_mark = now_; } while (0)
#else
#define RT_SECTION(k) do { } while (0)
#endif
#ifdef RT_STATS
__device__ unsigned long long g_stats[64];
__device__ unsigned long long g_hist[4][65];
#endif

constexpr uint32_t kXchgBStride = 44, kXchgPStride = 12;
constexpr uint32_t kXchgMaxSlots = 64;
constexpr uint32_t kXchgMinLanes = 4;
constexpr uint32_t kXchgRecWords = 60;
constexpr uint32_t kXchgFineSlots = 64;
constexpr uint32_t kXchgFineHdr = 8 + 2 * 64;
#ifndef RT_XCHG_SHADERS
#define RT_XCHG_SHADERS 1
#endif
constexpr uint32_t kXchgShaderWaves = RT_XCHG_SHADERS;
enum : uint32_t { XS_EMPTY = 0, XS_FULL = 1, XS_BUSY = 2 };

struct RenderArgs {
	DevScene S;
	DevCamera cam;
	DevRenderParams P;
	float *out;
	unsigned long long *rays_shot;
	uint32_t *work_counter;
	uint32_t *stack_ovf;
	DevPairScene pair;
	DevPairPrimary primary;
	DevGenKeys gen_keys;
	DevSkyTiles sky_tiles;
};
#if defined(__HIP_DEVICE_COMPILE__)
typedef const __attribute__((address_space(4))) RenderArgs *KArgs;
#else
typedef const RenderArgs *KArgs;
#endif

template <int METHOD, bool PRUNE, bool FINE, bool SKY_LDS, class F, bool XCHG = false>
__global__ __launch_bounds__((KernelShape<F, FINE, XCHG>::max_block), (KernelShape<F, FINE, XCHG>::waves_per_simd)) void render_kernel(const RenderArgs args_by_value)
{
	extern __shared__ __align__(16) uint32_t lds[];
	const uint32_t lane = threadIdx.x & 63u;
	const uint32_t wave = threadIdx.x >> 6;

	(void)args_by_value;
#if defined(__HIP_DEVICE_COMPILE__)
	const KArgs K = (KArgs)__builtin_amdgcn_kernarg_segment_ptr();
	auto kargs = [&]() -> KArgs {
		KArgs k = K;
		asm volatile("" : "+s"(k));
		return k;
	};
#else
	const KArgs K = &args_by_value;
	auto kargs = [&]() -> KArgs { return K; };
#endif
	DevPairScene PS = {};
	auto load_pair_boxes = [&]() {
		if constexpr (F::pair) {
			const KArgs k = kargs();
#pragma unroll
			for (int i = 0; i < 3; ++i) {
				PS.c0min[i] = k->pair.c0min[i]; PS.c0max[i] = k->pair.c0max[i];
				PS.c1min[i] = k->pair.c1min[i]; PS.c1max[i] = k->pair.c1max[i];
			}
		}
	};
	auto load_pair_scene = [&](auto with_boxes) {
		if constexpr (F::pair) {
			if constexpr (decltype(with_boxes)::value)
				load_pair_boxes();
			const KArgs k = kargs();
#pragma unroll
			for (int i = 0; i < 3; ++i) {
				PS.sky_c1[i] = k->pair.sky_c1[i]; PS.sky_c2[i] = k->pair.sky_c2[i];
			}
			PS.slot0 = k->pair.slot0; PS.slot1 = k->pair.slot1; PS.rank0 = k->pair.rank0; PS.rank1 = k->pair.rank1;
#pragma unroll
			for (int i = 0; i < 4; ++i) {
				PS.sphere[0][i] = k->pair.sphere[0][i]; PS.sphere[1][i] = k->pair.sphere[1][i];
				PS.lambert[0][i] = k->pair.lambert[0][i]; PS.lambert[1][i] = k->pair.lambert[1][i];
			}
			PS.inv_radius[0] = k->pair.inv_radius[0]; PS.inv_radius[1] = k->pair.inv_radius[1];
			PS.sky_param = k->pair.sky_param;
			PS.sky_tex_type = k->pair.sky_tex_type;
		}
	};
	DevPairPrimary PP = {};
	auto load_pair_primary = [&]() {
		if constexpr (F::pair) {
			const KArgs k = kargs();
#pragma unroll
			for (int i = 0; i < 3; ++i) {
				PP.box[0][0][i] = k->primary.box[0][0][i]; PP.box[0][1][i] = k->primary.box[0][1][i];
				PP.box[1][0][i] = k->primary.box[1][0][i]; PP.box[1][1][i] = k->primary.box[1][1][i];
			}
#pragma unroll
			for (int i = 0; i < 4; ++i) {
				PP.sphere[0][i] = k->primary.sphere[0][i]; PP.sphere[1][i] = k->primary.sphere[1][i];
			}
			PP.valid = k->primary.valid;
		}
	};
	const DevScene S_global = K->S;
	const DevRenderParams P = K->P;
	uint32_t *const stack_ovf = K->stack_ovf;
	DevScene S = S_global;

	SkyTables T;
	uint32_t sky_words = 0;
	if (SKY_LDS) {
		const uint32_t n_rows = S.sky.res_y * (S.sky.res_x + 1u);
		const uint32_t n_all = n_rows + S.sky.res_y + 1u;
// ... 23 lines not shown
	if (!FINE && P.scene_in_lds) {
		uint32_t *lds_blob = lds + sky_words;
		blob_words = S.blob_bytes / 4u;
		for (uint32_t i = threadIdx.x; i < blob_words; i += blockDim.x)
			lds_blob[i] = S.blob[i];
		__syncthreads();
		const char *b = reinterpret_cast<const char *>(lds_blob);
		S.nodes = reinterpret_cast<const DevNode *>(b + S.off_nodes);
		S.prims = reinterpret_cast<const DevPrim *>(b + S.off_prims);
		S.shade = reinterpret_cast<const DevShade *>(b + S.off_shade);
		S.prim_rank = reinterpret_cast<const uint32_t *>(b + S.off_rank);
		S.materials = reinterpret_cast<const DevMaterial *>(b + S.off_materials);
		S.textures = reinterpret_cast<const DevTexture *>(b + S.off_textures);
		S.lights = reinterpret_cast<const uint32_t *>(b + S.off_lights);
		S.big_leaves = reinterpret_cast<const uint2 *>(b + S.off_big_leaves);
	}
	StackMem SM;
	SM.cap = P.stack_cap;
	SM.ovf_depth = P.stack_ovf_depth;
	SM.ovf = stack_ovf;
	SM.region = lds + sky_words + blob_words;
	uint32_t *stk = SM.region + wave * (P.stack_cap * kStackStride) + lane;
	uint32_t *pool = nullptr;
	if constexpr (XCHG) {
		pool = lds + (((uint32_t)(SM.region - lds) + (blockDim.x >> 6) * (P.stack_cap * kStackStride) + 3u) & ~3u);
		if (FINE) {
			if (threadIdx.x < kXchgFineHdr)
				pool[threadIdx.x] = threadIdx.x == 3u ? kXchgShaderWaves : (threadIdx.x == 4u ? (blockDim.x >> 6) - kXchgShaderWaves : 0u);
		} else if (threadIdx.x < 4u) {
			pool[threadIdx.x] = 0u;
		}
		__syncthreads();
	}

#ifdef RT_STATS
	unsigned long long st_iters[2] = {0, 0}, st_active[2] = {0, 0}, st_gen = 0, st_hist[8] = {};
	unsigned long long st_sect[16] = {}, st_mark = wall_clock64();
	unsigned long long st_fine_clock[PH_COUNT + 1] = {};
	unsigned long long st_fine_iters[PH_COUNT] = {}, st_fine_active[PH_COUNT] = {};
#endif
	const bool sky_samplable = sky_can_sample(S);
	constexpr bool kWholeItems = F::pair && !FINE;
	static_assert(!(kWholeItems && XCHG), "the exchange's records carry chunk_begin and chunk_end, not chunk_c: no whole-pixel items there");
	constexpr int known_path = F::known_materials ? kMatLambertian : kMatRead;
	constexpr bool kKeyedGen = kWholeItems && lean_gen_keys(F::pair);
	constexpr bool kItemProduct = kWholeItems && lean_gen_item_product(F::pair);
	constexpr bool kSkyRun = kWholeItems && RT_PAIR_SKY_RUN != 0;

	int ph = PH_NEED_PIXEL;
	rt_rng rng = {1u, 2u, 3u, 4u};
	Ray ray;
	ray.o = ray.d = ray.inv = ray.shear = v3s(0.0f);
	uint32_t node = kRefDone;
	int sp = 0;
	float best_t = 0.0f;
	uint32_t best_prim = kNoPrim;
	bool any_hit = false;
	V3 thr = v3s(1.0f), outp = v3s(0.0f), mean = v3s(0.0f), wo = v3s(0.0f);
	Hit hit;
	hit.t = 0.0f;
	hit.point = hit.error = hit.normal = v3s(0.0f);
	hit.err_dot = 0.0f;
	hit.uvx = hit.uvy = 0.0f;
	hit.has_uv = hit.out = false;
	uint32_t mat = 0;
	uint32_t depth = 0, out_index = 0, pixel_index = 0, px = 0, py = 0;
	uint32_t sample_i = 0, chunk_begin = 0, chunk_end = P.spp, chunk_c = 0;
	uint32_t ray_count = 0;
	unsigned long long rays_total = 0;
	bool primary = true;
	uint32_t gen_hi0 = 0, gen_lo0 = 0;
	struct LightCtx {
		V3 l_wi;
		float pdf_multiplier;
		float t_limit;
		uint32_t skip;
		bool have_shadow, shadow_is_sky;
	};
	LightCtx PL;
	PL.l_wi = v3s(0.0f);
	PL.pdf_multiplier = 1.0f;
	PL.t_limit = 0.0f;
	PL.skip = kNoPrim;
	PL.have_shadow = PL.shadow_is_sky = false;

	auto begin_walk = [&](bool shadow) {
		any_hit = shadow;
		best_t = 0.0f;
		best_prim = kNoPrim;
		sp = 0;
		if (!FINE) {
			ph = PH_NODE;
			return;
		}
		if (XCHG) {
			ph = PH_WALK;
			return;
		}
		if (root_box_misses(S, ray)) {
			node = kRefDone;
			ph = shadow ? PH_SCATTER : PH_SHADE;
		} else if (S.narrow_only != 0u || !ray_is_regular(ray)) {
			ph = PH_NARROW;
		} else {
			node = S.root4_ref;
			ph = ref_is_leaf(node) ? PH_LEAF : PH_NODE;
		}
	};
	auto start_walk = [&]() {
		sp = 0;
		if (root_box_misses(S, ray)) {
			node = kRefDone;
			ph = any_hit ? PH_SCATTER : PH_SHADE;
		} else if (S.narrow_only != 0u || !ray_is_regular(ray)) {
			ph = PH_NARROW;
		} else {
			node = S.root4_ref;
			ph = ref_is_leaf(node) ? PH_LEAF : PH_NODE;
		}
	};
	auto after_step = [&]() {
		if (node == kRefDone)
			ph = any_hit ? PH_SCATTER : PH_SHADE;
		else
			ph = ref_is_leaf(node) ? PH_LEAF : PH_NODE;
	};
	auto finalize = [&](bool filter) {
		V3 c = outp;
		if (filter && (contains_nan(c) || !is_finite_any(c)))
			c = v3s(0.0f);
		if (P.sample_split > 1u) {
			mean.x += c.x;
			mean.y += c.y;
			mean.z += c.z;
		} else {
			const float i_f = (float)(sample_i + 1u);
			mean.x += (c.x - mean.x) / i_f;
			mean.y += (c.y - mean.y) / i_f;
			mean.z += (c.z - mean.z) / i_f;
		}
		rays_total += ray_count;
		sample_i += 1;
		if (sample_i == chunk_end) {
			const KArgs k = kargs();
			float *const out = k->out;
			out[3u * (size_t)out_index + 0u] = mean.x;
			out[3u * (size_t)out_index + 1u] = mean.y;
			out[3u * (size_t)out_index + 2u] = mean.z;
			ph = PH_NEED_PIXEL;
			if constexpr (kWholeItems) {
				const uint32_t log2_s = k->P.tile_log2_w >> 8;
				const uint32_t c1 = (chunk_c & (kWholePixel - 1u)) + 1u;
				if ((chunk_c & kWholePixel) != 0u && (c1 >> log2_s) == 0u) {
					chunk_c += 1u;
					chunk_end = (uint32_t)(((uint64_t)(c1 + 1u) * k->P.spp) >> log2_s);
					out_index += k->P.n_work;
					mean = v3s(0.0f);
					ph = PH_GEN;
				}
			}
		} else {
			ph = PH_GEN;
		}
	};

	auto do_gen = [&]() {
		const KArgs k = kargs();
		const uint64_t seed = ((uint64_t)k->P.seed_hi << 32) | k->P.seed_lo;
		const uint64_t sample_begin = ((uint64_t)k->P.sample_begin_hi << 32) | k->P.sample_begin_lo;
		const V3 cam_o = v3(k->cam.origin[0], k->cam.origin[1], k->cam.origin[2]);
		const V3 cam_ll = v3(k->cam.lower_left[0], k->cam.lower_left[1], k->cam.lower_left[2]);
		const V3 cam_h = v3(k->cam.horizontal[0], k->cam.horizontal[1], k->cam.horizontal[2]);
		const V3 cam_v = v3(k->cam.vertical[0], k->cam.vertical[1], k->cam.vertical[2]);
		const uint32_t w1 = here_(k->P.width - 1u), h1 = here_(k->P.height - 1u);
		if constexpr (kKeyedGen) {
			uint32_t hi0 = gen_hi0, lo0 = gen_lo0;
			if constexpr (!kItemProduct)
				philox_pixel_product(pixel_index, hi0, lo0);
			rng_seed_keyed<lean_gen_keys_lead(F::pair)>(&rng, &k->gen_keys, hi0, lo0, sample_begin + chunk_begin + sample_i);
		} else {
			rt_rng_seed(&rng, seed, (uint64_t)pixel_index, sample_begin + chunk_begin + sample_i);
		}
		RT_SECTION(15);
		const float jx = rt_rng_range_f32(&rng, 0.0f, 1.0f) + (float)px, jy = rt_rng_range_f32(&rng, 0.0f, 1.0f) + (float)py;
		float u, v;
		if (here_(k->P.w1h1_ok) != 0u) {
			u = div_by_verified(jx, (float)w1, k->P.inv_w1);
			v = 1.0f - div_by_verified(jy, (float)h1, k->P.inv_h1);
		} else {
			u = div_tame_fix_(jx, (float)w1);
			v = 1.0f - div_tame_fix_(jy, (float)h1);
		}
		ray = ray_new<F>(cam_o, cam_ll + cam_h * u + cam_v * v - cam_o);
		(void)rt_rng_f32(&rng);
		thr = v3s(1.0f);
		outp = v3s(0.0f);
		depth = 0;
		ray_count = 0;
		primary = true;
		begin_walk(false);
	
	};

	auto gen_direction = [&]() -> V3 {
		const KArgs k = kargs();
		const uint64_t seed = ((uint64_t)k->P.seed_hi << 32) | k->P.seed_lo;
		const uint64_t sample_begin = ((uint64_t)k->P.sample_begin_hi << 32) | k->P.sample_begin_lo;
		const V3 cam_o = v3(k->cam.origin[0], k->cam.origin[1], k->cam.origin[2]);
		const V3 cam_ll = v3(k->cam.lower_left[0], k->cam.lower_left[1], k->cam.lower_left[2]);
		const V3 cam_h = v3(k->cam.horizontal[0], k->cam.horizontal[1], k->cam.horizontal[2]);
		const V3 cam_v = v3(k->cam.vertical[0], k->cam.vertical[1], k->cam.vertical[2]);
		const uint32_t w1 = here_(k->P.width - 1u), h1 = here_(k->P.height - 1u);
		if constexpr (kKeyedGen) {
			uint32_t hi0 = gen_hi0, lo0 = gen_lo0;
			if constexpr (!kItemProduct)
				philox_pixel_product(pixel_index, hi0, lo0);
			rng_seed_keyed<lean_gen_keys_lead(F::pair)>(&rng, &k->gen_keys, hi0, lo0, sample_begin + chunk_begin + sample_i);
		} else {
			rt_rng_seed(&rng, seed, (uint64_t)pixel_index, sample_begin + chunk_begin + sample_i);
		}
		RT_SECTION(15);
		const float jx = rt_rng_range_f32(&rng, 0.0f, 1.0f) + (float)px, jy = rt_rng_range_f32(&rng, 0.0f, 1.0f) + (float)py;
		float u, v;
		if (here_(k->P.w1h1_ok) != 0u) {
			u = div_by_verified(jx, (float)w1, k->P.inv_w1);
			v = 1.0f - div_by_verified(jy, (float)h1, k->P.inv_h1);
		} else {
			u = div_tame_fix_(jx, (float)w1);
			v = 1.0f - div_tame_fix_(jy, (float)h1);
		}
		return cam_ll + cam_h * u + cam_v * v - cam_o;
	};
	auto do_sky_sample = [&]() {
		const V3 d = ray_new_dir<F>(gen_direction());
		Hit nh;
		uint32_t nmat;
		make_sky_hit_lean<F>(S, nh, nmat);
		outp = v3s(0.0f) + emission_of_hit<F>(S, PS, nmat, true, nh, d);
		ray_count = METHOD == 0 ? 1u : 0u;
		finalize(METHOD == 0);
	};

#ifdef RT_STATS
	unsigned long long st_lane_nodes = 0, st_lane_prims = 0, st_lane_maxsp = 0, st_sky_samples = 0, st_sky_runs = 0, st_sky_clock = 0, st_allsky_clock = 0, st_allsky_iters = 0, st_iter_t0 = 0;
#endif
	auto do_node = [&]() {
#ifdef RT_STATS
		st_lane_nodes += 1;
		if ((unsigned long long)sp > st_lane_maxsp)
			st_lane_maxsp = (unsigned long long)sp;
#endif
		const bool limit_valid = any_hit ? !(PL.t_limit != PL.t_limit) : (best_prim != kNoPrim);
		if (SM.ovf_depth == 0u)
			node = descend4<PRUNE, false>(S, SM, ray, node, stk, sp, limit_valid, any_hit ? PL.t_limit : best_t);
		else
			node = descend4<PRUNE, true>(S, SM, ray, node, stk, sp, limit_valid, any_hit ? PL.t_limit : best_t);
		after_step();
	
	};

	auto do_leaf = [&]() {
		uint32_t first, count, leaf_ref;
		const bool candidate = wide_leaf_hit(S, node, ray, leaf_ref);
		leaf_range(S, leaf_ref, first, count);
		if (!candidate)
			count = 0u;
		bool occluded = false;
		for (uint32_t slot = first; slot < first + count; ++slot) {
			if (any_hit && slot == PL.skip)
				continue;
#ifdef RT_STATS
			st_lane_prims += 1;
#endif
			const PrimGeom g = load_prim<F>(S, slot);
			float t;
			if (prim_t<F>(g, ray, t) && t > 0.0f) {
				if (any_hit) {
					if (!(t >= PL.t_limit)) {
						occluded = true;
						break;
					}
				} else {
					bool take;
					if (best_prim == kNoPrim)
						take = true;
					else if (t < best_t)
						take = true;
					else if (t == best_t)
						take = S.prim_rank[slot] < S.prim_rank[best_prim];
					else
						take = false;
					if (take) {
						best_t = t;
						best_prim = slot;
					}
				}
			}
		}
		if (occluded) {
			best_prim = 0u;
			node = kRefDone;
		} else if (sp == 0) {
			node = kRefDone;
		} else {
			--sp;
			node = SM.ovf_depth == 0u ? stack_load<false>(SM, stk, sp) : stack_load<true>(SM, stk, sp);
		}
		after_step();
	
	};

	auto do_shade = [&](auto arm_tag) {
		constexpr int arm = decltype(arm_tag)::value;
		const uint32_t prim = best_prim;
		bool finish = false;
		bool filter = true;
		Hit nh;
		uint32_t nmat;
		if (prim != kNoPrim)
			make_hit<F>(S, prim, ray, best_t, nh, nmat, PS);
		else
			make_sky_hit_lean<F>(S, nh, nmat);
		const int known_new = F::known_materials ? (prim == kNoPrim ? kMatEmit : kMatLambertian) : kMatRead;

		if (METHOD == 0) {
			ray_count += 1;
			const V3 wo_n = ray.d;
// ... 47 lines not shown
			}
		} else {
			const V3 m_wi = ray.d;
			const float m_pdf = mat_scattering_pdf<F>(S, mat, hit, wo, m_wi, known_path);
			const V3 le = emission_of_hit<F>(S, PS, nmat, prim == kNoPrim, hit , m_wi);
			thr = thr * mat_eval_over_pdf<F>(S, mat, hit, wo, m_wi, known_path, PS);
			RT_SECTION(11);
			if (!is_zero(le)) {
				const bool on_light = F::lights && (prim != kNoPrim) && mat_is_light(S, nmat) && !mat_is_delta<F>(S, mat);
				if (on_light || (prim == kNoPrim && sky_samplable)) {
					const uint32_t n_l = F::lights ? S.n_lights : 0u;
					const uint32_t n_choices = sky_samplable ? n_l + 1u : n_l;
					float l_pdf;
					if (prim == kNoPrim) {
						l_pdf = div_by_count(sky_pdf<F::pair>(S, T, m_wi), n_choices);
					} else {
						const PrimGeom g = load_prim<F>(S, prim);
						l_pdf = div_by_count(prim_scattering_pdf<F>(g, hit.point, m_wi, nh), n_choices);
					}
					const float mis_weight = power_heuristic(m_pdf, l_pdf);
					outp = outp + thr * le * mis_weight;
				} else {
					outp = outp + thr * le;
				}
			}
			RT_SECTION(12);
			if (mat_is_light<F>(S, nmat, known_new)) {
				finish = true;
			} else {
				if (depth > P.rr_threshold) {
					const float p = component_max(thr);
					if (rt_rng_f32(&rng) > p)
						finish = true;
					else
						thr = thr / p;
				}
				if (!finish) {
					wo = m_wi;
					hit = nh;
					mat = nmat;
					depth += 1;
					if (!(depth < P.max_depth))
						finish = true;
				}
			}
		}
		if (finish)
			finalize(filter);
		else if (METHOD == 1)
			ph = PH_LIGHT;
		else
			begin_walk(false);
	
	};

	auto do_light = [&](LightCtx &L, Ray &sr) {
		ray_count += 1;
		L.have_shadow = false;
		L.shadow_is_sky = false;
		L.pdf_multiplier = 1.0f;
		L.skip = kNoPrim;
		const uint32_t samplable_len = F::lights ? S.n_lights : 0u;
		bool pick_sky = false, pick_light = false;
		uint32_t light_slot = 0;
		if (samplable_len == 0u) {
			pick_sky = sky_samplable;
		} else if (!sky_samplable) {
			L.pdf_multiplier = 1.0f / (float)samplable_len;
			light_slot = rt_rng_below(&rng, samplable_len);
			pick_light = true;
		} else {
			L.pdf_multiplier = 1.0f / (float)(samplable_len + 1u);
			light_slot = rt_rng_below(&rng, samplable_len + 1u);
			if (light_slot == samplable_len)
				pick_sky = true;
			else
				pick_light = true;
		}
		const V3 shadow_origin = hit.point + 0.0001f * hit.normal;
		PrimGeom g;
		g.type = g.material = 0u;
		g.p0 = g.p1 = g.p2 = v3s(0.0f);
		if (pick_sky) {
			L.l_wi = sky_sample(S, T, rng);
			RT_SECTION(9);
			L.t_limit = __uint_as_float(0x7FC00000u);
			L.have_shadow = true;
			L.shadow_is_sky = true;
		} else if (pick_light) {
			if (S.single_light != kNoPrim) {
				L.skip = S.single_light;
				g = load_prim_uniform<F>(&S_global.prims[L.skip]);
			} else {
				L.skip = S.lights[light_slot];
				g = load_prim<F>(S, L.skip);
			}
			L.l_wi = prim_sample_visible_from_point<F>(g, hit.point, rng);
		}
		if (pick_sky || pick_light)
			sr = ray_new<F>(shadow_origin, L.l_wi);
		if (pick_light) {
			float lt;
			if (prim_t<F>(g, sr, lt) && lt > 0.0f) {
				L.t_limit = lt;
				L.have_shadow = true;
			}
		}
		if (L.have_shadow) {
			begin_walk(true);
		} else {
			best_prim = kNoPrim;
			ph = PH_SCATTER;
		}
	
	};

	auto do_scatter = [&](LightCtx &L, Ray &sr) {
		const bool occluded = best_prim != kNoPrim;
		if (L.have_shadow && !occluded) {
			bool valid = false;
			V3 le = v3s(0.0f);
			float l_pdf = 0.0f;
			if (L.shadow_is_sky) {
				le = emission_of_hit<F>(S, PS, S.sky.material, true, hit, L.l_wi);
				l_pdf = sky_pdf<F::pair>(S, T, L.l_wi) * L.pdf_multiplier;
				valid = true;
			} else {
				Hit lh;
				uint32_t lm;
				PrimGeom g;
				if (S.single_light != kNoPrim) {
					g = load_prim_uniform<F>(&S_global.prims[L.skip]);
					if (!F::tri || g.type == kPrimSphere) {
						make_sphere_hit_by_reciprocal(g.p0, g.p1.x, g.p1.y, sr, L.t_limit, lh);
						lm = g.material;
					} else {
						make_hit<F>(S, L.skip, sr, L.t_limit, lh, lm);
					}
				} else {
					make_hit<F>(S, L.skip, sr, L.t_limit, lh, lm);
					g = load_prim<F>(S, L.skip);
				}
				const float p = prim_scattering_pdf<F>(g, hit.point, L.l_wi, lh);
				if (p > 0.0f) {
					le = mat_get_emission<F>(S, lm, lh, L.l_wi);
					l_pdf = p * L.pdf_multiplier;
					valid = true;
				}
			}
			if (valid) {
				const float m_pdf = mat_scattering_pdf<F>(S, mat, hit, wo, L.l_wi, known_path);
				if constexpr (F::pair) {
					outp = outp + mis_light_term_short(thr * mat_eval<F>(S, mat, hit, wo, L.l_wi, known_path, PS), le, l_pdf, m_pdf);
				} else {
					const float mis_weight = power_heuristic(l_pdf, m_pdf);
					outp = outp + thr * mat_eval<F>(S, mat, hit, wo, L.l_wi, known_path, PS) * mis_weight * le / l_pdf;
				}
			}
		}
		RT_SECTION(10);
		ray.d = wo;
		if (mat_scatter_ray<F>(S, mat, ray, hit, rng, known_path))
			finalize(true);
		else
			begin_walk(false);
	
	};

	auto do_narrow = [&]() {
		if (any_hit) {
			best_prim = trace_any<F, PRUNE, true>(S, S_global, SM, ray, stk, PL.t_limit, PL.skip) ? 0u : kNoPrim;
			ph = PH_SCATTER;
		} else {
			trace_closest<F, PRUNE, true>(S, S_global, SM, ray, stk, best_t, best_prim);
			ph = PH_SHADE;
		}
		node = kRefDone;
		sp = 0;
	};

	auto walk_closest_pending = [&]() {
		if (ph == PH_NODE && !any_hit) {
			trace_closest<F, PRUNE>(S, S_global, SM, ray, stk, best_t, best_prim, PS);
			ph = PH_SHADE;
		}
	};
	auto walk_closest_primary = [&]() {
		if constexpr (F::pair) {
			if (PP.valid != 0u) {
				if (ph == PH_NODE && !any_hit) {
					trace_closest_pair_primary(ray, best_t, best_prim, PS, PP);
					ph = PH_SHADE;
				}
				return;
			}
			load_pair_boxes();
		}
		walk_closest_pending();
	};
	auto walk_shadow_pending = [&](const LightCtx &L, const Ray &sr) {
		if (ph == PH_NODE && any_hit) {
			best_prim = trace_any<F, PRUNE>(S, S_global, SM, sr, stk, L.t_limit, L.skip, PS) ? 0u : kNoPrim;
			ph = PH_SCATTER;
		}
	};

	auto record_store = [&](uint32_t *rec) {
		uint4 *d = reinterpret_cast<uint4 *>(rec);
// ... 591 lines not shown
					}
#endif
				}
			}
			const uint32_t n_light = (uint32_t)__popcll(__ballot(ph == PH_LIGHT));
			const uint32_t n_trace = (METHOD == 1 && RT_PQ_SPLIT) ? (uint32_t)__popcll(__ballot(ph == PH_GEN))
			                                                      : (uint32_t)__popcll(__ballot(ph == PH_GEN || ph == PH_NODE || ph == PH_LEAF || ph == PH_SHADE));
			constexpr bool kBodyAlways = RT_BODY_ALWAYS(KernelShape<F>::spheres_only);
			if (kBodyAlways) {
				alive = (n_light + n_trace != 0u) || __ballot(ph == PH_NEED_PIXEL) != 0ull;
				if (XCHG && METHOD == 1 && !alive)
					alive = __hip_atomic_load(&pool[1], __ATOMIC_RELAXED, __HIP_MEMORY_SCOPE_WORKGROUP) != 0u ||
					        __hip_atomic_load(&pool[2], __ATOMIC_RELAXED, __HIP_MEMORY_SCOPE_WORKGROUP) != 0u;
			}
			if (kBodyAlways || n_light + n_trace != 0u) {
				const bool run_light = (METHOD == 1) && (n_light >= kLightPhaseThreshold || n_trace == 0u || (kStarveLimit != 0u && waited >= kStarveLimit));
				waited = run_light ? 0u : waited + n_light;
	#ifdef RT_STATS
				if (lane == 0u) {
					if (!run_light) {
						st_iters[0] += 1; st_active[0] += n_trace;
						st_hist[((n_trace ? n_trace : 1u) - 1u) >> 3] += 1;
#ifndef RT_STATS_NO_HIST
						atomicAdd(&g_hist[0][n_trace], 1ull);
						atomicAdd(&g_hist[1][n_light], 1ull);
#endif
						st_gen += (unsigned long long)__popcll(__ballot(ph == PH_GEN));
					} else {
						st_iters[1] += 1; st_active[1] += n_light;
#ifndef RT_STATS_NO_HIST
						atomicAdd(&g_hist[3][n_light], 1ull);
#endif
					}
				}
	#endif
				RT_SECTION(0);
				constexpr bool kFuseRegions = METHOD == 1 && RT_PQ_SPLIT && RT_FUSE_REGIONS(KernelShape<F>::spheres_only);
				bool run_q = run_light;
				if (!run_light) {
					if (kFuseRegions) {
						if (ph == PH_GEN) {
							load_pair_scene(std::false_type{});
							do_gen();
							load_pair_primary();
							RT_SECTION(1);
							walk_closest_primary();
							RT_SECTION(2);
							do_shade(std::integral_constant<int, 1>{});
						}
						RT_SECTION(3);
#ifdef RT_STATS
						if (n_light == 0u && n_trace != 0u && __ballot(ph == PH_LIGHT) == 0ull) {
							st_allsky_clock += wall_clock64() - st_iter_t0;
							st_allsky_iters += 1;
						}
#endif
						const uint32_t n_light_now = (uint32_t)__popcll(__ballot(ph == PH_LIGHT));
						run_q = n_light_now >= kLightPhaseThreshold;
						if (run_q)
							waited = 0u;
	#ifdef RT_STATS
						if (run_q && lane == 0u) {
							st_iters[1] += 1; st_active[1] += n_light_now;
						}
	#endif
					} else {
						load_pair_scene(std::true_type{});
						if (ph == PH_GEN)
							do_gen();
						RT_SECTION(1);
						walk_closest_pending();
						RT_SECTION(2);
						if (ph == PH_SHADE)
							do_shade(std::integral_constant<int, (METHOD == 1 && RT_PQ_SPLIT) ? 1 : 0>{});
						RT_SECTION(3);
					}
				}
				if (run_q) {
					LightCtx L;
					L.l_wi = v3s(0.0f);
					L.pdf_multiplier = 1.0f;
					L.t_limit = 0.0f;
					L.skip = kNoPrim;
					L.have_shadow = L.shadow_is_sky = false;
					Ray sray;
					sray.o = sray.d = sray.inv = sray.shear = v3s(0.0f);
					if (kFuseRegions) {
						if (ph == PH_LIGHT) {
							load_pair_scene(std::true_type{});
							do_light(L, sray);
							RT_SECTION(4);
							walk_shadow_pending(L, sray);
							RT_SECTION(5);
							do_scatter(L, sray);
							RT_SECTION(6);
							if (ph == PH_NODE) {
								walk_closest_pending();
								RT_SECTION(7);
								do_shade(std::integral_constant<int, 2>{});
							}
						}
						RT_SECTION(8);
					} else {
						load_pair_scene(std::true_type{});
						if (ph == PH_LIGHT)
							do_light(L, sray);
						RT_SECTION(4);
						walk_shadow_pending(L, sray);
						RT_SECTION(5);
						if (ph == PH_SCATTER)
							do_scatter(L, sray);
						RT_SECTION(6);
	#if RT_PQ_SPLIT
						walk_closest_pending();
						RT_SECTION(7);
						if (ph == PH_SHADE)
							do_shade(std::integral_constant<int, 2>{});
						RT_SECTION(8);
	#endif
					}
				}
	#if RT_PQ_SPLIT
				if (METHOD == 1) {
					ray.o = ray.d = ray.inv = ray.shear = v3s(0.0f);
					best_t = 0.0f;
					best_prim = kNoPrim;
					node = kRefDone;
					sp = 0;
					any_hit = false;
				}
	#endif
			} else {
				alive = __ballot(ph == PH_NEED_PIXEL) != 0ull;
				if (XCHG && METHOD == 1)
					alive = alive || __hip_atomic_load(&pool[1], __ATOMIC_RELAXED, __HIP_MEMORY_SCOPE_WORKGROUP) != 0u ||
					        __hip_atomic_load(&pool[2], __ATOMIC_RELAXED, __HIP_MEMORY_SCOPE_WORKGROUP) != 0u;
			}
		}
	}
#ifdef RT_STATS
	atomicAdd(&g_stats[20], st_lane_nodes);
	atomicAdd(&g_stats[21], st_lane_prims);
	atomicMax(&g_stats[22], st_lane_maxsp);
	if (lane == 0u) {
		for (int k = 0; k < 9; ++k)
			atomicAdd(&g_stats[40 + k], st_sect[k]);
		if (!FINE)
			for (int k = 9; k < 16; ++k)
				atomicAdd(&g_stats[40 + k], st_sect[k]);
		for (int k = 0; k < 8; ++k)
			atomicAdd(&g_stats[24 + k], st_hist[k]);
		for (int k = 0; k <= PH_COUNT; ++k)
			atomicAdd(&g_stats[50 + k], st_fine_clock[k]);
		atomicAdd(&g_stats[0], st_iters[0]); atomicAdd(&g_stats[1], st_active[0]);
		atomicAdd(&g_stats[2], st_iters[1]); atomicAdd(&g_stats[3], st_active[1]);
		atomicAdd(&g_stats[4], st_gen);
		atomicAdd(&g_stats[58], st_sky_samples);
		atomicAdd(&g_stats[59], st_sky_runs);
		atomicAdd(&g_stats[60], st_sky_clock);
		atomicAdd(&g_stats[61], st_allsky_clock);
		atomicAdd(&g_stats[62], st_allsky_iters);
		for (int k = 0; k < PH_COUNT; ++k) {
			atomicAdd(&g_stats[5 + k], st_fine_iters[k]);
			atomicAdd(&g_stats[5 + PH_COUNT + k], st_fine_active[k]);
		}
	}
#endif
	unsigned long long *const rays_shot = K->rays_shot;
	if (rays_shot != nullptr) {
		for (int off = 32; off > 0; off >>= 1)
			rays_total += __shfl_down(rays_total, off);
		if (lane == 0u)
			atomicAdd(rays_shot, rays_total);
	}
}

__global__ __launch_bounds__(256) void combine_chunks_kernel(const DevRenderParams P, const float *__restrict__ partial, float *__restrict__ out)
{
	const uint32_t wp = blockIdx.x * blockDim.x + threadIdx.x;
	if (wp >= P.n_work)
		return;
	uint32_t x, y;
	if (!work_to_pixel(P, wp, x, y))
		return;
	V3 acc = v3s(0.0f);
	for (uint32_t c = 0; c < P.sample_split; ++c) {
		const float *m = partial + 3u * ((size_t)c * P.n_work + wp);
		acc.x = acc.x + m[0];
		acc.y = acc.y + m[1];
		acc.z = acc.z + m[2];
	}
	const size_t o = P.shard_layout ? (size_t)wp : (size_t)y * P.width + x;
	out[3u * o + 0u] = acc.x / (float)P.spp;
	out[3u * o + 1u] = acc.y / (float)P.spp;
	out[3u * o + 2u] = acc.z / (float)P.spp;
}

__global__ __launch_bounds__(256) void reset_kernel(uint32_t *__restrict__ work_counter, unsigned long long *__restrict__ rays_shot,
                                                    float *__restrict__ out, size_t n_out_floats)
{
	const size_t i = (size_t)blockIdx.x * blockDim.x + threadIdx.x;
	if (i == 0) {
		*work_counter = 0u;
		if (rays_shot)
			*rays_shot = 0ull;
	}
	for (size_t k = i; k < n_out_floats; k += (size_t)gridDim.x * blockDim.x)
		out[k] = 0.0f;
}
hipError_t launch_reset(hipStream_t stream, uint32_t *work_counter, unsigned long long *rays_shot, float *out, size_t n_out_floats)
{
	size_t blocks = (n_out_floats + 255) / 256;
	if (blocks < 1)
		blocks = 1;
	if (blocks > 4096)
		blocks = 4096;
	hipLaunchKernelGGL(reset_kernel, dim3((uint32_t)blocks), dim3(256), 0, stream, work_counter, rays_shot, out, n_out_floats);
	return hipGetLastError();
}

__global__ __launch_bounds__(256) void quantise_kernel(const float *__restrict__ rgb, size_t n_values, float inv_gamma, uint8_t *__restrict__ out)
{
	const size_t stride = (size_t)gridDim.x * blockDim.x;
	const size_t n4 = n_values / 4;
	for (size_t i = (size_t)blockIdx.x * blockDim.x + threadIdx.x; i < n4; i += stride) {
		const float4 v = reinterpret_cast<const float4 *>(rgb)[i];
// ... 142 lines not shown
using FeatSimple = Feat<true, true, false, false>;

template <class F> static render_fn pick_render_f(int method, bool prune, bool fine, bool sky_lds, bool xchg)
{
#ifdef RT_ONLY_HEADLINE
	if constexpr (!(F::cmat || F::ctex))
		if (method == 1 && !prune && !fine && sky_lds && !xchg)
			return render_kernel<1, false, false, true, F>;
#ifdef RT_HEADLINE_RUNNABLE
	if constexpr (!(F::cmat || F::ctex))
		if (method == 1 && !prune && !fine && !sky_lds && !xchg)
			return render_kernel<1, false, false, false, F>;
#endif
	return nullptr;
#else
	if constexpr (F::pair) {
		if (xchg || prune || fine)
			return nullptr;
		if (method == 0)
			return render_kernel<0, false, false, false, F>;
		return sky_lds ? render_kernel<1, false, false, true, F> : render_kernel<1, false, false, false, F>;
	} else {
	if (xchg) {
		if (method == 1 && !prune && !fine)
			return sky_lds ? render_kernel<1, false, false, true, F, true> : render_kernel<1, false, false, false, F, true>;
		if (fine && method == 0)
			return render_kernel<0, true, true, false, F, true>;
		if (fine && method == 1)
			return sky_lds ? render_kernel<1, true, true, true, F, true> : render_kernel<1, true, true, false, F, true>;
		return nullptr;
	}
#define RT_PICK(M, P, G, L) \
	if (method == M && prune == P && fine == G && sky_lds == L) \
		return render_kernel<M, P, G, L, F>;
	RT_PICK(0, false, false, false)
	RT_PICK(0, true, false, false)
	RT_PICK(0, true, true, false)
	RT_PICK(1, false, false, false)
	RT_PICK(1, false, false, true)
	RT_PICK(1, true, false, false)
	RT_PICK(1, true, false, true)
	RT_PICK(1, true, true, false)
	RT_PICK(1, true, true, true)
#undef RT_PICK
	return nullptr;
	}
#endif
}

static render_fn pick_render(int method, bool prune, bool fine, bool sky_lds, int feature_set, bool xchg = false)
{
	if (method == 0)
		sky_lds = false;
	if (fine)
		prune = true;
	if (feature_set == 0)
		return pick_render_f<FeatSpheres>(method, prune, fine, sky_lds, xchg);
	if (feature_set == 1)
		return pick_render_f<FeatSimple>(method, prune, fine, sky_lds, xchg);
	if (feature_set == 3)
		return pick_render_f<FeatPair>(method, prune, fine, sky_lds, xchg);
	return pick_render_f<FeatFull>(method, prune, fine, sky_lds, xchg);
}
bool render_exchange_available(int method, bool prune, bool fine, int feature_set) { (void)feature_set; return fine || (method == 1 && !prune); }
size_t render_exchange_lds_bytes(uint32_t slots) { return (size_t)(4u + 4u + (kXchgBStride + kXchgPStride) * slots) * sizeof(uint32_t); }
uint32_t render_exchange_max_slots() { return kXchgMaxSlots; }
size_t render_exchange_fine_lds_bytes(uint32_t waves_per_block) { return (size_t)(4u + kXchgFineHdr + waves_per_block * 64u + 2u * kXchgFineSlots * kXchgRecWords) * sizeof(uint32_t); }

hipError_t render_occupancy(int method, bool prune, bool fine, bool sky_lds, int feature_set, size_t lds_bytes, int *blocks_per_cu, bool xchg,
                            uint32_t block_threads)
{
	render_fn fn = pick_render(method, prune, fine, sky_lds, feature_set, xchg);
	if (!fn)
		return hipErrorInvalidValue;
	hipError_t e = hipFuncSetAttribute(reinterpret_cast<const void *>(fn), hipFuncAttributeMaxDynamicSharedMemorySize, (int)lds_bytes);
	if (e != hipSuccess)
		return e;
	return hipOccupancyMaxActiveBlocksPerMultiprocessor(blocks_per_cu, fn, block_threads ? block_threads : render_block_threads(feature_set, fine, xchg), lds_bytes);
}

hipError_t launch_render(int method, bool prune, bool fine, bool sky_lds, int feature_set, uint32_t n_blocks, size_t lds_bytes, hipStream_t stream,
                         const DevScene &S, const DevCamera &cam, const DevRenderParams &P, float *out,
                         unsigned long long *rays_shot, uint32_t *work_counter, uint32_t *stack_ovf, bool xchg, const DevPairScene *pair,
                         const DevPairPrimary *primary, uint32_t block_threads, const DevSkyTiles &sky_tiles)
{
	render_fn fn = pick_render(method, prune, fine, sky_lds, feature_set, xchg);
	if (!fn)
		return hipErrorInvalidValue;
	RenderArgs A;
	A.S = S;
	A.cam = cam;
	A.P = P;
	A.out = out;
	A.rays_shot = rays_shot;
	A.work_counter = work_counter;
	A.stack_ovf = stack_ovf;
	A.pair = pair ? *pair : DevPairScene{};
	A.primary = primary ? *primary : DevPairPrimary{};
	A.sky_tiles = sky_tiles;
	philox_round_keys(((uint64_t)P.seed_hi << 32) | P.seed_lo, A.gen_keys);
	hipLaunchKernelGGL(fn, dim3(n_blocks), dim3(block_threads ? block_threads : render_block_threads(feature_set, fine, xchg)), lds_bytes, stream, A);
	return hipGetLastError();
}

}
```

### raytracing-rust_amd/csrc/rt_selftest.h

```cpp
#pragma once

#include <hip/hip_runtime.h>

#include "../../include/rt_hip.h"
#include "rt_types.h"
#include "rt_sky_tiles.h"

namespace rt {

hipError_t launch_selftest_lean(hipStream_t stream, uint32_t blocks, uint64_t n_per_thread, uint64_t seed, unsigned long long *mismatches);
hipError_t launch_selftest_pair_primary(hipStream_t stream, const DevPairScene &pair, const float root_min[3], const float root_max[3], const float origin[3],
                                        const DevPairPrimary &host_block, unsigned long long *mismatches);

struct DevSkySelftest {
	uint64_t seed;
	uint64_t n;
	float *out_dirs;
	float *out_pdf_s;
	const float *dirs;
	uint64_t m;
	float *out_pdf;
};

size_t sky_selftest_lds_bytes(const DevScene &S);
hipError_t launch_sky_selftest(bool tables_in_lds, hipStream_t stream, const DevScene &S, const DevSkySelftest &P);



constexpr uint32_t kShortFormsRcpExponentCount = 8;
struct DevShortForms {
	unsigned long long *tested;
	unsigned long long *mismatches;
	unsigned long long *first_index;
	unsigned long long *sqrt_raw;
	unsigned long long *site_tested;
	unsigned long long *site_mismatches;
};
uint32_t short_forms_input_bits(int form, uint64_t index);
uint32_t short_forms_in_use();
hipError_t launch_short_forms(hipStream_t stream, const DevShortForms &D, const float *operands, uint64_t n_operands);

enum { kDivCountTested = 0, kDivCountBad = 1, kDivCountFirst = 1 + RT_DIV_FORMS, kDivCountSiteTested = 1 + 2 * RT_DIV_FORMS, kDivCountSiteInDomain,
       kDivCountSiteBad, kDivCounts = kDivCountSiteBad + RT_DIV_SITES };
struct DevDivForms {
	const uint32_t *denominators;
	uint32_t n_denominators, first_denominator;
	const int32_t *exponents;
	uint32_t n_exponent_pairs;
	unsigned long long *counts;
};
uint32_t div_forms_in_use();
hipError_t launch_div_forms(hipStream_t stream, const DevDivForms &D);
hipError_t launch_div_sites(hipStream_t stream, const float *operand_pairs, uint64_t n_pairs, unsigned long long *counts);
hipError_t launch_sky_pdf_forms(hipStream_t stream, const DevScene &S, const float *dirs, uint64_t m, float *out_pair, float *out_default);

uint32_t frame_forms_in_use();
hipError_t launch_frame_forms(hipStream_t stream, const float *vectors, uint64_t n_vectors, unsigned long long *counts);

uint32_t gen_keys_in_use();
hipError_t launch_gen_keys(hipStream_t stream, uint64_t seed, const uint32_t *cases, uint64_t n_cases, unsigned long long *counts);

hipError_t launch_pair_shadow(hipStream_t stream, const float *cases, uint64_t n_cases, unsigned long long *counts);
hipError_t launch_pair_shadow_walk(hipStream_t stream, const float *cases, uint64_t n_cases, unsigned long long *counts);

hipError_t launch_sky_tiles(hipStream_t stream, const DevSkyTiles &T, uint32_t width, uint32_t height, uint32_t log2_w, uint32_t tiles_x, uint64_t n_tiles, uint8_t *out);

}
```

### raytracing-rust_amd/csrc/rt_selftest_forms.hip

```cpp
#include "rt_shade.h"
#include "rt_gen_keys.h"
#include "rt_selftest.h"
#include "rt_selftest_dev.h"

namespace rt {

__host__ __device__ inline uint32_t short_forms_rcp_input(uint64_t index)
{
	static_assert(kShortFormsRcpExponentCount == 8, "one case per exponent");
	int e = 0;
	switch ((uint32_t)(index >> 24)) {
	case 0: e = -81; break;
	case 1: e = -60; break;
	case 2: e = -24; break;
	case 3: e = -1; break;
	case 4: e = 0; break;
	case 5: e = 1; break;
	case 6: e = 24; break;
	default: e = 41; break;
	}
	return ((uint32_t)(index >> 23) & 1u) << 31 | (uint32_t)(127 + e) << 23 | ((uint32_t)index & 0x007FFFFFu);
}

using FormTally = Tally<RT_SHORT_FORMS>;
// ... 191 lines not shown
}
hipError_t launch_div_forms(hipStream_t stream, const DevDivForms &D) { return launch_cases(div_forms_kernel, stream, div_forms_items(D), 4096u, D); }
constexpr uint32_t div_form_bit(LeanDivForm f) { return 1u << (f == LeanDivForm::one_pair ? RT_DIV_FORM_ONE_PAIR : RT_DIV_FORM_TWO_PAIRS); }
uint32_t div_forms_in_use() { return div_form_bit(lean_div_form(true)); }

__device__ __noinline__ V3 mis_light_term_plain(V3 te, V3 le, float l_pdf, float m_pdf)
{
	const float a_sq = l_pdf * l_pdf;
	const float mis_weight = a_sq / (a_sq + m_pdf * m_pdf);
	return te * mis_weight * le / l_pdf;
}
__device__ __noinline__ V3 div3_plain(V3 v, float d) { return v / d; }
__device__ __forceinline__ bool same_v3(V3 a, V3 b) { return same_f32(a.x, b.x) && same_f32(a.y, b.y) && same_f32(a.z, b.z); }
__device__ __forceinline__ bool div_fix_domain(float n, float d)
{
	const float an = fabsf(n), ad = fabsf(d);
	const bool d_tame = ad >= 0x1p-81f && ad <= 0x1p41f;
	const bool n_tame = an >= 0x1p-81f && an <= 0x1p41f;
	const int apart = (int)(__float_as_uint(an) >> 23) - (int)(__float_as_uint(ad) >> 23);
	return d_tame && ((n_tame && apart < 96 && apart > -96) || an == 0.0f || an == INFINITY || n != n);
}
__global__ __launch_bounds__(256) void div_sites_kernel(const float *__restrict__ pairs, uint64_t n_pairs, unsigned long long *counts)
{
	Tally<kDivCounts> T;
	for_each_case(n_pairs, [&](uint64_t i) {
		const float n = pairs[2u * i], d = pairs[2u * i + 1u];
		if (div_fix_domain(n, d)) {
			T.add(kDivCountSiteInDomain);
			T.add(kDivCountSiteBad + RT_DIV_SITE_FIX, !same_f32(lean_div_fix_for<true>(n, d), n / d));
			const V3 v = v3(n, 0.0f, -INFINITY);
			T.add(kDivCountSiteBad + RT_DIV_SITE_DIV3_FIX, !same_v3(lean_div3_fix_for<true>(v, d), div3_plain(v, d)));
		}
		const V3 one = v3s(1.0f), te = v3(1.0f, 0.75f, -0.5f);
		bool ok = same_v3(mis_light_term_short(te, one, d, n), mis_light_term_plain(te, one, d, n));
		ok = ok && same_v3(mis_light_term_short(te, one, n, d), mis_light_term_plain(te, one, n, d));
		const V3 tx = v3(2.0f * n, 0.75f, -0.5f), tz = v3(0.75f, -0.5f, 2.0f * n), ta = v3s(2.0f * n);
		ok = ok && same_v3(mis_light_term_short(tx, one, 1.0f, 1.0f), mis_light_term_plain(tx, one, 1.0f, 1.0f));
		ok = ok && same_v3(mis_light_term_short(tz, one, d, d), mis_light_term_plain(tz, one, d, d));
		ok = ok && same_v3(mis_light_term_short(ta, v3(1.0f, d, -1.0f), 1.0f, 1.0f), mis_light_term_plain(ta, v3(1.0f, d, -1.0f), 1.0f, 1.0f));
		T.add(kDivCountSiteBad + RT_DIV_SITE_MIS_LIGHT_TERM, !ok);
		T.add(kDivCountSiteBad + RT_DIV_SITE_ATAN2,
		      !(same_f32(lean_atan2_for<true>(n, d), lean_atan2(n, d)) && same_f32(lean_atan2_for<true>(d, n), lean_atan2(d, n)) &&
		        same_f32(lean_atan2_for<true>(-n, d), rt_atan2f(-n, d))));
		T.add(kDivCountSiteTested);
	});
	T.flush(counts);
}
hipError_t launch_div_sites(hipStream_t stream, const float *operand_pairs, uint64_t n_pairs, unsigned long long *counts)
{
	return launch_cases(div_sites_kernel, stream, n_pairs, 2048u, operand_pairs, n_pairs, counts);
}

struct SkyPdfFormsArgs {
	DevScene S;
	const float *dirs;
	uint64_t m;
	float *out_pair, *out_default;
};
__global__ __launch_bounds__(256) void sky_pdf_forms_kernel(const SkyPdfFormsArgs A)
{
	SkyTables T;
	T.row_cdf = A.S.sky.row_cdf;
	T.marginal_cdf = A.S.sky.marginal_cdf;
	T.guide = A.S.sky.guide;
	T.guide_k = A.S.sky.guide_k;
	T.inv_res = nullptr;
	for_each_case(A.m, [&](uint64_t j) {
		const V3 wi = v3(A.dirs[3 * j], A.dirs[3 * j + 1], A.dirs[3 * j + 2]);
		A.out_pair[j] = sky_pdf<true>(A.S, T, wi);
		A.out_default[j] = sky_pdf(A.S, T, wi);
	});
}
hipError_t launch_sky_pdf_forms(hipStream_t stream, const DevScene &S, const float *dirs, uint64_t m, float *out_pair, float *out_default)
{
	SkyPdfFormsArgs A;
	A.S = S;
	A.dirs = dirs;
	A.m = m;
	A.out_pair = out_pair;
	A.out_default = out_default;
	return launch_cases(sky_pdf_forms_kernel, stream, m, 2048u, A);
}

__device__ __noinline__ Coord coord_from_z_plain(V3 z) { return coord_from_z(z); }
__device__ __forceinline__ Coord pair_kernels_frame(V3 z)
{
	return lean_frame_form(true) == LeanFrameForm::guarded_short ? coord_from_z_pair(z) : coord_from_z(z);
}
__global__ __launch_bounds__(256) void frame_forms_kernel(const float *__restrict__ vectors, uint64_t n_vectors, unsigned long long *counts)
{
	Tally<RT_FRAME_FORMS_COUNTS> T;
	for_each_case(n_vectors, [&](uint64_t i) {
		const V3 v = v3(vectors[3u * i], vectors[3u * i + 1u], vectors[3u * i + 2u]);
		const Coord got = pair_kernels_frame(v), want = coord_from_z_plain(v);
		T.add(RT_FRAME_FORMS_FRAME_MISMATCHES, !(same_v3(got.x, want.x) && same_v3(got.y, want.y) && same_v3(got.z, want.z)));
		const float a = fabsf(v.x) > fabsf(v.y) ? v.x : v.y;
		T.add(RT_FRAME_FORMS_FRAME_SHORT, frame_guard_(a, v.z, a * a + v.z * v.z));
		const Ray r = ray_new<FeatPair>(v3s(0.0f), v), p = ray_new_plain(v3s(0.0f), v);
		T.add(RT_FRAME_FORMS_RAY_MISMATCHES, !(same_v3(r.d, p.d) && same_v3(r.inv, p.inv)));
		const float m2 = dot(v, v);
		T.add(RT_FRAME_FORMS_RAY_SHORT, fminf(fminf(fabsf(v.x), fabsf(v.y)), fabsf(v.z)) >= 0x1p-60f && m2 >= 0x1p-40f && m2 <= 0x1p40f);
		T.add(RT_FRAME_FORMS_TESTED);
	});
	T.add(RT_FRAME_FORMS_FRAME_PLAIN, T.n[RT_FRAME_FORMS_TESTED] - T.n[RT_FRAME_FORMS_FRAME_SHORT]);
	T.add(RT_FRAME_FORMS_RAY_PLAIN, T.n[RT_FRAME_FORMS_TESTED] - T.n[RT_FRAME_FORMS_RAY_SHORT]);
	T.flush(counts);
}
hipError_t launch_frame_forms(hipStream_t stream, const float *vectors, uint64_t n_vectors, unsigned long long *counts)
{
	return launch_cases(frame_forms_kernel, stream, n_vectors, 2048u, vectors, n_vectors, counts);
}
uint32_t frame_forms_in_use()
{
	return (lean_frame_form(true) == LeanFrameForm::guarded_short ? 1u << RT_FRAME_FORM_FRAME_SHORT : 0u) |
	       (lean_ray_norm_short(true) ? 1u << RT_FRAME_FORM_RAY_NORM_ONE_PAIR : 0u);
}

struct GenKeysSelftestArgs {
	DevGenKeys keys;
	uint64_t seed;
	const uint32_t *cases;
	uint64_t n_cases;
	unsigned long long *counts;
};
__device__ __forceinline__ bool same_stream(rt_rng a, rt_rng b, bool &draws_differ)
{
	const bool same = a.s0 == b.s0 && a.s1 == b.s1 && a.s2 == b.s2 && a.s3 == b.s3;
	draws_differ = false;
	for (int d = 0; d < 8; ++d)
		draws_differ |= rt_rng_u32(&a) != rt_rng_u32(&b);
	return same;
}
__global__ __launch_bounds__(256) void gen_keys_kernel(const GenKeysSelftestArgs args_by_value)
{
#if defined(__HIP_DEVICE_COMPILE__)
	const auto *A = (const __attribute__((address_space(4))) GenKeysSelftestArgs *)__builtin_amdgcn_kernarg_segment_ptr();
	(void)args_by_value;
#else
	const GenKeysSelftestArgs *A = &args_by_value;
#endif
	constexpr int lead = lean_gen_keys_lead(true);
	const uint64_t seed = A->seed, n_cases = A->n_cases;
	const uint32_t *const cases = A->cases;
	Tally<RT_GEN_KEYS_COUNTS> T;
	for_each_case(n_cases, [&](uint64_t i) {
		const uint32_t pixel = cases[4u * i], sample_i = cases[4u * i + 1u];
		const uint64_t sample_begin = ((uint64_t)cases[4u * i + 3u] << 32) | cases[4u * i + 2u];
		const uint64_t sample = sample_begin + sample_i;
		rt_rng want, keyed, item;
		rt_rng_seed(&want, seed, (uint64_t)pixel, sample);
		uint32_t hi0, lo0;
		philox_pixel_product(pixel, hi0, lo0);
		rng_seed_keyed<lead>(&keyed, &A->keys, hi0, lo0, sample);
		uint32_t hi0_item, lo0_item;
		philox_pixel_product(pixel, hi0_item, lo0_item);
#if defined(__HIP_DEVICE_COMPILE__)
		asm volatile("" : "+v"(hi0_item), "+v"(lo0_item));
#endif
		rng_seed_keyed<lead>(&item, &A->keys, hi0_item, lo0_item, sample);
		bool draws;
		T.add(RT_GEN_KEYS_STATE_MISMATCHES, !same_stream(keyed, want, draws));
		T.add(RT_GEN_KEYS_DRAW_MISMATCHES, draws);
		T.add(RT_GEN_KEYS_ITEM_STATE_MISMATCHES, !same_stream(item, want, draws));
		T.add(RT_GEN_KEYS_ITEM_DRAW_MISMATCHES, draws);
		T.add(RT_GEN_KEYS_ZERO_BLOCKS, want.s0 == 1u && (want.s1 | want.s2 | want.s3) == 0u);
		T.add(RT_GEN_KEYS_TESTED);
// ... 42 lines not shown
```

### raytracing-rust_amd/csrc/rt_shade.h

```cpp
#pragma once

#include "rt_intersect.h"

namespace rt {

__device__ __forceinline__ float sqrt_unit_(float x)
{
#if defined(__HIP_DEVICE_COMPILE__) && !defined(RT_NO_LEAN)
	return lean_sqrt(x);
#else
	return sqrtf(x);
#endif
}
__device__ __forceinline__ float div_tame_fix_(float n, float d)
{
#if defined(__HIP_DEVICE_COMPILE__) && !defined(RT_NO_LEAN)
	return lean_div_fix(n, d);
#else
	return n / d;
#endif
}

constexpr float kSitePdfMin = 0x1p-27f, kSitePdfMax = 0x1p20f;
constexpr float kSiteNumMin = 0x1p-75f, kSiteNumMax = 0x1p41f;
// ... 230 lines not shown
	return texture_colour<F>(S, m.texture, direction, point);
}

struct LambertRec {
	V3 colour;
	float albedo;
};
template <class F> __device__ __forceinline__ LambertRec lambert_record(const DevScene &S, const DevMaterial &m, uint32_t mat, V3 direction, V3 point, const DevPairScene &ps)
{
	LambertRec L;
	if constexpr (F::known_materials) {
		const bool first = mat == ps.slot0;
		L.colour = first ? v3(ps.lambert[0][0], ps.lambert[0][1], ps.lambert[0][2]) : v3(ps.lambert[1][0], ps.lambert[1][1], ps.lambert[1][2]);
		L.albedo = first ? ps.lambert[0][3] : ps.lambert[1][3];
	} else {
		L.colour = material_texture_colour<F>(S, m, mat, direction, point);
		L.albedo = m.param;
	}
	return L;
}

__device__ __forceinline__ uint32_t here_(uint32_t uniform)
{
#if defined(__HIP_DEVICE_COMPILE__)
	asm volatile("" : "+s"(uniform));
#endif
	return uniform;
}

__device__ __forceinline__ float div_by_count(float x, uint32_t n)
{
	if ((n & (n - 1u)) == 0u && n != 0u)
		return x * __uint_as_float((127u - (uint32_t)__builtin_ctz(n)) << 23);
	return x / (float)n;
}

__device__ __forceinline__ uint32_t dist1d_sample(const float *cdf, uint32_t n, const uint8_t *guide, uint32_t guide_k, rt_rng &rng)
{
	const float num = rt_rng_f32(&rng);
	uint32_t first;
	if (guide != nullptr) {
		first = guide[(uint32_t)(num * (float)guide_k)];
		for (;;) {
			const float c0 = cdf[first > n ? n : first], c1 = cdf[first + 1u > n ? n : first + 1u];
			const bool b0 = first <= n && c0 <= num;
			const bool b1 = b0 && first + 1u <= n && c1 <= num;
			first += (b0 ? 1u : 0u) + (b1 ? 1u : 0u);
			if (!b1)
				break;
		}
	} else {
		first = 0;
		uint32_t len = n + 1;
		while (len > 0) {
			const uint32_t half = len >> 1;
			const uint32_t middle = first + half;
			if (cdf[middle] <= num) {
				first = middle + 1;
				len -= half + 1;
			} else {
				len = half;
			}
		}
	}
	const uint32_t v = first - 1u;
	return v > n - 1u ? n - 1u : v;
}

#if defined(__HIP_DEVICE_COMPILE__)
typedef const __attribute__((address_space(4))) uint32_t *KWords;
#else
typedef const uint32_t *KWords;
#endif
struct SkyTables {
	const float *row_cdf;
	const float *marginal_cdf;
	const uint8_t *guide;
	uint32_t guide_k;
	KWords inv_res;
};

__device__ __forceinline__ bool sky_can_sample(const DevScene &S) { return (S.sky.res_x | S.sky.res_y) != 0u; }

template <bool SHORT = false> __device__ __forceinline__ float sky_pdf(const DevScene &S, const SkyTables &T, V3 wi)
{
	const float sin_theta = sqrt_unit_(1.0f - wi.z * wi.z);
	if (sin_theta <= 0.0f)
		return 0.0f;
	const float theta = lean_acos_dev(wi.z);
	float phi = SHORT ? lean_atan2_for<true>(wi.y, wi.x) : lean_atan2(wi.y, wi.x);
	if (phi < 0.0f)
		phi += 2.0f * kPi;
	const float u = div_by_verified(phi, kTau, kRcpTau);
	const float v = div_by_verified(theta, kPi, kRcpPi);
	const uint32_t rx = here_(S.sky.res_x), ry = here_(S.sky.res_y);
	uint32_t ui = f32_as_index((float)rx * u);
	uint32_t vi = f32_as_index((float)ry * v);
	ui = ui > rx - 1u ? rx - 1u : ui;
	vi = vi > ry - 1u ? ry - 1u : vi;
	const float ypdf = T.marginal_cdf[vi + 1u] - T.marginal_cdf[vi];
	const float *row = T.row_cdf + (size_t)vi * (rx + 1u);
	const float xpdf = row[ui + 1u] - row[ui];
	return (float)rx * (float)ry * (ypdf * xpdf) / (sin_theta * kTau * kPi);
}

__device__ __forceinline__ V3 sky_sample(const DevScene &S, const SkyTables &T, rt_rng &rng)
{
	const uint32_t rx = here_(S.sky.res_x), ry = here_(S.sky.res_y);
	const bool guided = T.guide_k != 0u;
	const uint32_t sv = dist1d_sample(T.marginal_cdf, ry, guided ? T.guide + (size_t)ry * T.guide_k : nullptr, T.guide_k, rng);
	const uint32_t su = dist1d_sample(T.row_cdf + (size_t)sv * (rx + 1u), rx, guided ? T.guide + (size_t)sv * T.guide_k : nullptr, T.guide_k, rng);
	const float nu = next_float((float)su + rt_rng_f32(&rng)), nv = next_float((float)sv + rt_rng_f32(&rng));
	float u, v;
	KWords inv = T.inv_res;
#if defined(__HIP_DEVICE_COMPILE__)
	asm volatile("" : "+s"(inv));
#endif
	if (inv != nullptr && inv[0] != 0u) {
		u = div_by_verified(nu, (float)rx, __uint_as_float(inv[1]));
		v = div_by_verified(nv, (float)ry, __uint_as_float(inv[2]));
	} else {
		u = nu / (float)rx;
		v = nv / (float)ry;
	}
	const float phi = u * 2.0f * kPi;
	const float theta = v * kPi;
	float st, ct, sp, cp;
	lean_sincos(theta, st, ct);
	lean_sincos(phi, sp, cp);
	return v3(st * cp, st * sp, ct);
}

__device__ __forceinline__ V3 lambertian_sample(V3 normal, rt_rng &rng)
{
	const float cos_theta = sqrt_unit_(1.0f - rt_rng_f32(&rng));
	const float sin_theta = sqrt_unit_(1.0f - cos_theta * cos_theta);
	const float phi = 2.0f * kPi * rt_rng_f32(&rng);
	float sin_phi, cos_phi;
	lean_sincos(phi, sin_phi, cos_phi);
	const V3 local = v3(cos_phi * sin_theta, sin_phi * sin_theta, cos_theta);
	const Coord c = coord_from_z(normal);
	return to_coord(c, local);
}
template <bool ZSEL = false, bool PAIR_FRAME = false> __device__ __forceinline__ V3 lambertian_sample_(V3 normal, rt_rng &rng)
{
	const float cos_theta = sqrt_unit_(1.0f - rt_rng_f32(&rng));
	const float sin_theta = sqrt_unit_(1.0f - cos_theta * cos_theta);
	const float phi = 2.0f * kPi * rt_rng_f32(&rng);
	float sin_phi, cos_phi;
	lean_sincos(phi, sin_phi, cos_phi);
	const V3 local = v3(cos_phi * sin_theta, sin_phi * sin_theta, cos_theta);
	const Coord c = PAIR_FRAME ? coord_from_z_pair(normal) : (ZSEL ? coord_from_z_zsel(normal) : coord_from_z(normal));
	return to_coord(c, local);
}
__device__ __forceinline__ float tr_d(float alpha, float cos_theta)
{
	if (cos_theta <= 0.0f)
		return 0.0f;
	const float a_sq = alpha * alpha;
	const float tmp = cos_theta * cos_theta * (a_sq - 1.0f) + 1.0f;
	return a_sq / (kPi * tmp * tmp);
}
__device__ __forceinline__ float tr_g2(float alpha, V3 normal, V3 h, V3 incoming, V3 outgoing)
{
	if (dot(incoming, h) / dot(incoming, normal) <= 0.0f || dot(outgoing, h) / dot(outgoing, normal) <= 0.0f)
		return 0.0f;
	const float alpha_sq = alpha * alpha;
	const float one_minus_alpha_sq = 1.0f - alpha_sq;
	const float cos_i = dot(normal, incoming);
	const float tmp_a = alpha_sq + one_minus_alpha_sq * (cos_i * cos_i);
	const float cos_o = dot(normal, outgoing);
	const float tmp_b = alpha_sq + one_minus_alpha_sq * (cos_o * cos_o);
	return 2.0f * cos_i * cos_o / (cos_o * sqrtf(tmp_a) + cos_i * sqrtf(tmp_b));
}
__device__ __forceinline__ float tr_g1(float alpha, V3 normal, V3 h, V3 v)
{
	if (dot(v, h) / dot(v, normal) <= 0.0f)
		return 0.0f;
	const float c = dot(normal, v);
	const float alpha_sq = alpha * alpha;
	const float tmp = alpha_sq + (1.0f - alpha_sq) * (c * c);
	return 2.0f * c / (sqrtf(tmp) + c);
}
__device__ __forceinline__ float tr_vndf(float a, V3 h, V3 incoming)
{
	if (h.z < 0.0f)
		return 0.0f;
	return tr_g1(a, v3(0.0f, 0.0f, 1.0f), h, incoming) * fmax_(dot(incoming, h), 0.0f) * tr_d(a, h.z) / incoming.z;
}
__device__ inline V3 tr_sample_vndf(float a_x, float a_y, V3 incoming, rt_rng &rng)
{
	const V3 vh = normalised(v3(a_x * incoming.x, a_y * incoming.y, incoming.z));
	const float len_sq = vh.x * vh.x + vh.y * vh.y;
	const V3 basis_two = len_sq > 0.0f ? v3(-vh.y, vh.x, 0.0f) / sqrtf(len_sq) : v3(1.0f, 0.0f, 0.0f);
	const V3 basis_three = cross(vh, basis_two);
	const float r = sqrtf(rt_rng_f32(&rng));
	const float phi = kTau * rt_rng_f32(&rng);
	float sin_phi, cos_phi;
	lean_sincos(phi, sin_phi, cos_phi);
	const float tx = r * cos_phi;
	float ty = r * sin_phi;
	const float s = 0.5f * (1.0f + vh.z);
	ty = (1.0f - s) * sqrtf(1.0f - tx * tx) + s * ty;
	const V3 hh = tx * basis_two + ty * basis_three + sqrtf(fmax_(1.0f - tx * tx - ty * ty, 0.0f)) * vh;
	return normalised(v3(a_x * hh.x, a_y * hh.y, fmax_(hh.z, 0.0f)));
}
__device__ inline V3 tr_sample(float alpha, V3 incoming, V3 normal, rt_rng &rng)
{
	const Coord coord = coord_from_z(normal);
	const Coord inverse = coord_inverse(coord);
	const V3 h = to_coord(coord, tr_sample_vndf(alpha, alpha, to_coord(inverse, incoming), rng));
	return reflected(incoming, h);
}
// ... 255 lines not shown
```

### raytracing-rust_amd/csrc/rt_types.h

```cpp
#pragma once

#include <stdint.h>
#include "rt_vec.h"

namespace rt {

constexpr uint32_t kNoPrim = 0xFFFFFFFFu;

template <bool TRI, bool LIGHTS, bool CMAT, bool CTEX> struct Feat {
	static constexpr bool tri = TRI;
	static constexpr bool lights = LIGHTS;
	static constexpr bool cmat = CMAT;
	static constexpr bool ctex = CTEX;
	static constexpr bool pair = false;
	static constexpr bool known_materials = false;
	static constexpr bool sky_shadows_only = false;
};
using FeatFull = Feat<true, true, true, true>;
struct FeatPair : Feat<false, false, false, false> {
	static constexpr bool pair = true;
	static constexpr bool known_materials = true;
	static constexpr bool sky_shadows_only = true;
};

constexpr uint32_t kLeafFlag = 0x80000000u;
constexpr uint32_t kLeafInlineMax = 31u;
constexpr uint32_t kLeafSlotMask = 0x03FFFFFFu;
struct alignas(64) DevNode {
	float c0min[3], c0max[3];
	float c1min[3], c1max[3];
	uint32_t c0, c1;
	uint32_t pad0, pad1;
};
static_assert(sizeof(DevNode) == 64, "DevNode must be one 64-byte record");

constexpr uint32_t kRefNone = 0x7FFFFFFEu;
struct alignas(64) DevNodeQ4 {
	float origin[3];
	uint32_t exps;
	uint32_t qlo[3];
	uint32_t qhi[3];
	uint32_t child[4];
	uint32_t pad[2];
};
static_assert(sizeof(DevNodeQ4) == 64, "DevNodeQ4 must be one 64-byte record");

struct alignas(32) DevLeafBox {
	float lo[3], pad0;
	float hi[3], pad1;
};

enum : uint32_t { kPrimSphere = 0, kPrimTriangle = 1, kPrimMeshTriangle = 2 };

constexpr uint32_t kMatHandleShift = 6u;
constexpr uint32_t kMatMaxCount = 1u << 24;
inline __host__ __device__ uint32_t mat_handle_make(uint32_t index, int32_t type, int32_t tex_type)
{
	return (index << kMatHandleShift) | (((uint32_t)tex_type & 7u) << 3) | ((uint32_t)type & 7u);
}
inline __host__ __device__ uint32_t mat_handle_index(uint32_t h) { return h >> kMatHandleShift; }
inline __host__ __device__ int32_t mat_handle_type(uint32_t h) { return (int32_t)(h & 7u); }
inline __host__ __device__ int32_t mat_handle_tex_type(uint32_t h) { return (int32_t)((h >> 3) & 7u); }

struct alignas(16) DevPrim {
	float a[4], b[4], c[4];
};
static_assert(sizeof(DevPrim) == 48, "DevPrim must be three 16-byte lanes");

struct alignas(16) DevShade {
	float n0[4], n1[4], n2[4];
};

struct alignas(16) DevMaterial {
	int32_t type;
	uint32_t texture;
	float param;
	int32_t tex_type;
	float tex_c1[3];
	float tex_c2[3];
	float ior[3];
	float metallic;
	uint32_t pad[2];
};
static_assert(sizeof(DevMaterial) == 64, "DevMaterial must be 64 bytes");

struct DevTexture {
	int32_t type;
	float c1[3];
	float c2[3];
	uint32_t dim_x, dim_y;
	uint32_t pad;
	const float *image;
	const float *perlin_vecs;
	const uint32_t *perlin_perm;
};

struct DevSky {
	uint32_t texture, material;
	uint32_t res_x, res_y;
	const float *row_cdf;
	const float *marginal_cdf;
	const uint8_t *guide;
	uint32_t guide_k;
	uint32_t inv_res_ok;
	float inv_res_x, inv_res_y;
};

struct DevScene {
	const DevNode *nodes;
	const DevPrim *prims;
	const DevShade *shade;
	const uint32_t *prim_rank;
	const DevMaterial *materials;
	const DevTexture *textures;
	const uint32_t *lights;
	const uint2 *big_leaves;
	uint32_t n_nodes, n_prims, n_lights, n_materials, n_textures;
	uint32_t root_ref;
	float root_min[3], root_max[3];
	const uint32_t *blob;
	uint32_t blob_bytes;
	uint32_t off_nodes, off_prims, off_shade, off_rank, off_materials, off_textures, off_lights, off_big_leaves;
	uint32_t stack_depth;
	const DevNodeQ4 *nodes4;
	const DevLeafBox *leaf_box;
	uint32_t root4_ref;
	uint32_t n_nodes4;
	uint32_t narrow_only;
	uint32_t has_triangles;
	uint32_t lambert_tame;
	uint32_t single_light;
	DevSky sky;
};

constexpr int kStackStride = 64;
constexpr uint32_t kFourWaves = 4;
inline size_t four_wave_stack_lds_bytes(const DevScene &S) { return (size_t)kFourWaves * S.stack_depth * kStackStride * sizeof(uint32_t); }

struct alignas(64) DevPairScene {
	float c0min[3], c0max[3], c1min[3], c1max[3];
	uint32_t slot0, slot1;
	uint32_t rank0, rank1;
	float sphere[2][4];
	float lambert[2][4];
	float sky_param;
	int32_t sky_tex_type;
	float sky_c1[3], sky_c2[3];
	float inv_radius[2];
	uint32_t pad[6];
};
static_assert(sizeof(DevPairScene) == 192, "DevPairScene: three 64-byte lines");
__device__ static const DevPairScene kNoPairScene = {};

struct alignas(64) DevPairPrimary {
	float box[2][2][3];
	float sphere[2][4];
	uint32_t valid;
	float deltapdot[2];
	float root[2][3];
	uint32_t pad[3];
};
static_assert(sizeof(DevPairPrimary) == 128, "DevPairPrimary: two 64-byte lines");
constexpr int kPairPrimaryValues = 28;
RT_FN void pair_primary_terms(const DevPairScene &q, const float root_min[3], const float root_max[3], V3 o, DevPairPrimary &pp)
{
	const float oc[3] = {o.x, o.y, o.z};
	bool finite = finite_f(o.x) && finite_f(o.y) && finite_f(o.z);
	for (int k = 0; k < 3; ++k) {
		pp.box[0][0][k] = q.c0min[k] - oc[k]; pp.box[0][1][k] = q.c0max[k] - oc[k];
		pp.box[1][0][k] = q.c1min[k] - oc[k]; pp.box[1][1][k] = q.c1max[k] - oc[k];
		pp.root[0][k] = root_min[k] - oc[k]; pp.root[1][k] = root_max[k] - oc[k];
		finite = finite && finite_f(pp.box[0][0][k]) && finite_f(pp.box[0][1][k]) && finite_f(pp.box[1][0][k]) && finite_f(pp.box[1][1][k]) &&
		         finite_f(pp.root[0][k]) && finite_f(pp.root[1][k]);
	}
	for (int s = 0; s < 2; ++s) {
		const float radius = q.sphere[s][3];
		const V3 deltap = v3(q.sphere[s][0], q.sphere[s][1], q.sphere[s][2]) - o;
		const float deltapdot = dot(deltap, deltap);
		pp.sphere[s][0] = deltap.x; pp.sphere[s][1] = deltap.y; pp.sphere[s][2] = deltap.z;
		pp.deltapdot[s] = deltapdot;
		pp.sphere[s][3] = deltapdot - radius * radius;
		finite = finite && finite_f(deltap.x) && finite_f(deltap.y) && finite_f(deltap.z) && finite_f(deltapdot) && finite_f(pp.sphere[s][3]);
	}
	pp.valid = finite ? 1u : 0u;
	pp.pad[0] = pp.pad[1] = pp.pad[2] = 0u;
}

struct alignas(64) DevGenKeys {
	uint32_t key[10][2];
// ... 34 lines not shown
```

### raytracing-rust_amd/hip_backend.py

```python
import ctypes as C
import os
import sys

import numpy as np

from . import abi

_HERE = os.path.dirname(os.path.abspath(__file__))
LIB_PATH = os.environ.get("RT_HIP_LIB") or os.path.join(_HERE, "librt_hip.so")
_LIB = None


class RtHipError(RuntimeError):
    def __init__(self, code, message):
        super().__init__(f"rt_hip error {code}: {message}")
        self.code = code


def lib():
    global _LIB
    if _LIB is None:
        if not os.path.exists(LIB_PATH):
            raise RtHipError(abi.RT_ERR_NO_DEVICE, f"{LIB_PATH} not built (run `make -C raytracing-rust_amd/csrc`); "
                             "the HIP back end has no CPU fallback")
# ... 106 lines not shown

def _f3(v):
    return (C.c_float * 3)(*[float(np.float32(x)) for x in v])


def _in_use(names, mask):
    return [n for k, n in enumerate(names) if mask >> k & 1]


def _selftest_cases(test, cases, device, *lead):
    symbol, ctype, width, what, names, forms = abi.SELFTEST_CASE_TABLES[test]
    cases = np.ascontiguousarray(cases, dtype=np.dtype(ctype))
    if cases.ndim != 2 or cases.shape[1] != width:
        raise ValueError(f"{what} must be (n, {width}), got {cases.shape}")
    out = (C.c_uint64 * len(names))()
    _check(getattr(lib(), symbol)(C.c_int(device), *lead, _p(cases, ctype), C.c_uint64(cases.shape[0]), out))
    res = dict(zip(names, (int(x) for x in out)))
    if forms is not None:
        res["in_use"] = _in_use(forms, res["in_use"])
    return res


def rccl_probe():
    usable, note = C.c_int(), C.create_string_buffer(512)
    _check(lib().rt_rccl_probe(C.byref(usable), note, C.c_uint64(512)))
    return bool(usable.value), note.value.decode()


def device_count():
    return int(lib().rt_device_count())


def selftest_lean(device=0, n_per_thread=64, seed=1):
    out = (C.c_uint64 * 9)()
    _check(lib().rt_selftest_lean(C.c_int(device), C.c_uint64(n_per_thread), C.c_uint64(seed), out))
    return [int(x) for x in out]


def selftest_short_forms(device=0, operands=None):
    res = abi.ShortFormsResult()
    if operands is None:
        _check(lib().rt_selftest_short_forms(C.c_int(device), None, C.c_uint64(0), C.byref(res)))
        forms = {name: (int(f.tested), int(f.mismatches), int(f.first_mismatch) if f.mismatches else None)
                 for name, f in zip(abi.SHORT_FORM_NAMES, res.form)}
        raw = {k: int(getattr(res, "sqrt_raw_" + k)) for k in ("exact", "high", "low", "other")}
        return {"forms": forms, "sqrt_raw": raw, "in_use": _in_use(abi.SHORT_FORM_NAMES, res.in_use)}
    ops = np.ascontiguousarray(operands, dtype=np.float32).ravel()
    _check(lib().rt_selftest_short_forms(C.c_int(device), _p(ops, C.c_float), C.c_uint64(ops.size), C.byref(res)))
    return {"sites": dict(zip(abi.SHORT_SITE_NAMES, (int(x) for x in res.site_mismatches))), "tested": int(res.site_tested)}


def selftest_div_forms(denominators=None, exponents=((0, 0),), first_denominator=0, n_denominators=None, operands=None, device=0):
    res = abi.DivFormsResult()
    if operands is not None:
        ops = np.ascontiguousarray(operands, dtype=np.float32)
        if ops.ndim != 2 or ops.shape[1] != 2:
            raise ValueError(f"operands must be (n, 2), got {ops.shape}")
        _check(lib().rt_selftest_div_forms(C.c_int(device), None, _p(ops, C.c_float), C.c_uint64(ops.shape[0]), C.byref(res)))
        return {"tested": int(res.site_tested), "in_domain": int(res.site_in_domain),
                "sites": dict(zip(abi.DIV_SITE_NAMES, (int(x) for x in res.site_mismatches)))}
    exps = np.ascontiguousarray(exponents, dtype=np.int32).reshape(-1, 2)
    sl = abi.DivFormsSlice()
    sl.exponents, sl.n_exponent_pairs = _p(exps, C.c_int32), exps.shape[0]
    if denominators is not None:
        dens = np.ascontiguousarray(denominators, dtype=np.uint32).ravel()
        sl.denominators, sl.n_denominators = _p(dens, C.c_uint32), dens.size
    else:
        sl.denominators, sl.n_denominators, sl.first_denominator = None, int(n_denominators), int(first_denominator)
    _check(lib().rt_selftest_div_forms(C.c_int(device), C.byref(sl), None, C.c_uint64(0), C.byref(res)))
    forms = {name: (int(res.mismatches[k]), (int(res.first_numerator[k]), int(res.first_denominator[k])) if res.mismatches[k] else None)
             for k, name in enumerate(abi.DIV_FORM_NAMES)}
    return {"tested": int(res.tested), "forms": forms, "in_use": _in_use(abi.DIV_FORM_NAMES, res.in_use)}


def selftest_sky_pdf_forms(scene, dirs):
    dirs = np.ascontiguousarray(dirs, dtype=np.float32)
    if dirs.ndim != 2 or dirs.shape[1] != 3:
        raise ValueError(f"dirs must be (m, 3), got {dirs.shape}")
    a, b = np.empty(dirs.shape[0], dtype=np.float32), np.empty(dirs.shape[0], dtype=np.float32)
    _check(lib().rt_selftest_sky_pdf_forms(scene._h, _p(dirs, C.c_float), C.c_uint64(dirs.shape[0]), _p(a, C.c_float), _p(b, C.c_float)))
    return a, b


def selftest_frame_forms(vectors, device=0):
    return _selftest_cases("frame_forms", vectors, device)


def philox_round_keys(seed):
    keys = np.zeros((10, 2), dtype=np.uint32)
    lib().rt_philox_round_keys.restype = None
    lib().rt_philox_round_keys(C.c_uint64(seed & 0xFFFFFFFFFFFFFFFF), _p(keys, C.c_uint32))
    return keys


def selftest_gen_keys(seed, cases, device=0):
    return _selftest_cases("gen_keys", cases, device, C.c_uint64(seed & 0xFFFFFFFFFFFFFFFF))


def selftest_pair_shadow(cases, device=0):
    return _selftest_cases("pair_shadow", cases, device)


def selftest_pair_shadow_walk(cases, device=0):
    return _selftest_cases("pair_shadow_walk", cases, device)


def selftest_pair_primary(scene, origin):
    valid, bad = C.c_uint32(), C.c_uint64()
    _check(lib().rt_selftest_pair_primary(scene._h, _f3(origin), C.byref(valid), C.byref(bad)))
    return bool(valid.value), int(bad.value)


def selftest_sky_tiles(scene, camera, opts):
    tw, th = int(opts.tile_width) or 8, int(opts.tile_height) or 8
    tiles_x, tiles_y = (int(opts.width) + tw - 1) // tw, (int(opts.height) + th - 1) // th
    out = np.zeros(tiles_x * tiles_y, dtype=np.uint8)
    _check(lib().rt_selftest_sky_tiles(scene._h, C.byref(camera), C.byref(opts), _p(out, C.c_uint8), C.c_uint64(out.size)))
    return out.reshape(tiles_y, tiles_x)


def camera_new(origin, lookat, vup, fov, aspect_ratio, aperture, focus_dist):
    cam = abi.Camera()
    _check(lib().rt_camera_new(C.byref(cam), _f3(origin), _f3(lookat), _f3(vup), C.c_float(fov),
                               C.c_float(aspect_ratio), C.c_float(aperture), C.c_float(focus_dist)))
    return cam


def lens_camera_new(origin, lookat, vup, fov, aspect_ratio, aperture, focus_dist, projection="perspective"):
    if isinstance(projection, str):
        _known(projection, abi.PROJECTIONS, "projection")
        projection = abi.PROJECTIONS[projection]
    cam = abi.LensCamera()
    _check(lib().rt_lens_camera_new(C.byref(cam), _f3(origin), _f3(lookat), _f3(vup), C.c_float(fov), C.c_float(aspect_ratio),
                                    C.c_float(aperture), C.c_float(focus_dist), C.c_int32(projection)))
    return cam


HIT_DTYPE = np.dtype([("t", "<f4"), ("point", "<f4", 3), ("error", "<f4", 3), ("normal", "<f4", 3), ("uv", "<f4", 2),
                      ("has_uv", "<i4"), ("out", "<i4"), ("material", "<u4"), ("found", "<u4"), ("index", "<u8")])
NODE_DTYPE = np.dtype([("min", "<f4", 3), ("max", "<f4", 3), ("children", "<i8", 2), ("primitive_offset", "<u8"),
                       ("number_primitives", "<u8")])


WIDE_NODE_DTYPE = np.dtype([("origin", "<f4", 3), ("exps", "<u4"), ("qlo", "<u4", 3), ("qhi", "<u4", 3), ("child", "<u4", 4),
                            ("pad", "<u4", 2)])


def _pack_rays(origins, directions):
    o = np.asarray(origins, dtype=np.float32).reshape(-1, 3)
    d = np.asarray(directions, dtype=np.float32).reshape(-1, 3)
    return np.ascontiguousarray(np.concatenate([o, d], axis=1))


class HipScene:

    def __init__(self, scene_description, device=0, devices=None):
        self._desc = scene_description.desc()
        self._h = C.c_void_p()
        if devices is not None:
            devices = [int(d) for d in devices]
            self.device = devices[0]
            self.devices = devices
            arr = (C.c_int * len(devices))(*devices)
            _check(lib().rt_scene_create_multi(C.byref(self._desc), arr, C.c_uint32(len(devices)), C.byref(self._h)))
        else:
            self.device = device
# ... 763 lines not shown
```

Measured before the change: 42990.

## Carry sampled sky cell from light sampling to MIS pdf evaluation

When a light sample picks the sky, the sampled table cell (su, sv) is now packed into a register word. A flag bit marks whether the jitter sits far enough from the cell edges, per a host-proven error bound, that recomputing the cell from the direction would land on the same cell. The later sky pdf evaluation reuses the carried cell and skips the atan2/acos-style direction-to-cell inverse unless some lane in the wave lacks the guard. The change adds a guard computation, a tuning key, a selftest kernel and extra register pressure in the pair kernel. It also depends on the error bound holding, or pdfs could differ from recomputed ones.

```diff
diff --git a/include/rt_hip.h b/include/rt_hip.h
--- a/include/rt_hip.h
+++ b/include/rt_hip.h
@@ -219,7 +219,7 @@
 int rt_scene_set_traversal(rt_scene *scene, int mode);
 typedef enum rt_tuning_key { RT_TUNE_TRAVERSAL = 0, RT_TUNE_FEATURE_SET = 1, RT_TUNE_SCENE_IN_LDS = 2, RT_TUNE_SCHEDULE = 3, RT_TUNE_WALK = 4,
                              RT_TUNE_STACK_CAP = 5, RT_TUNE_EXCHANGE = 6, RT_TUNE_WHOLE_PIXEL_SHARE = 7, RT_TUNE_RADIANCE_GROUPS = 8,
-                             RT_TUNE_SKY_RUN = 10 } rt_tuning_key;
+                             RT_TUNE_SKY_RUN = 10, RT_TUNE_SKY_CELL = 11 } rt_tuning_key;
 int rt_scene_set_tuning(rt_scene *scene, int key, int value);
 int rt_plan_work_items(const rt_render_opts *opts, uint32_t split, int share, uint64_t resident_waves, uint32_t *whole_claims,
                        uint64_t *n_items);
@@ -652,6 +652,14 @@
 } rt_div_forms_result;
 int rt_selftest_div_forms(int device, const rt_div_forms_slice *slice, const float *operands, uint64_t n_operand_pairs, rt_div_forms_result *out);
 int rt_selftest_sky_pdf_forms(rt_scene *scene, const float *dirs, uint64_t m, float *out_pdf_pair, float *out_pdf_default);
+enum { RT_SKY_CELL_GUARDED_DISAGREE = 0, RT_SKY_CELL_UNGUARDED = 1, RT_SKY_CELL_UNGUARDED_AGREE = 2, RT_SKY_CELL_PDF_MISMATCHES = 3, RT_SKY_CELL_TESTED = 4,
+       RT_SKY_CELL_COUNTS = 5 };
+enum { RT_SKY_CELL_OUT_WORDS = 4 };
+#define RT_SKY_CELL_NO_CELL 0x7FFFFFFFu
+enum { RT_SKY_CELL_GUARD_PROVEN = 0, RT_SKY_CELL_GUARD_ENABLED = 1, RT_SKY_CELL_GUARD_DELTA_U = 2, RT_SKY_CELL_GUARD_DELTA_V = 3, RT_SKY_CELL_GUARD_ROW_LO = 4,
+       RT_SKY_CELL_GUARD_ROW_HI = 5, RT_SKY_CELL_GUARD_IN_USE = 6, RT_SKY_CELL_GUARD_WORDS = 8 };
+int rt_selftest_sky_cell(rt_scene *scene, const uint32_t *cases, uint64_t n, uint32_t axis, uint32_t su, uint32_t sv, uint32_t *out,
+                         uint64_t counts[RT_SKY_CELL_COUNTS], uint32_t guard[RT_SKY_CELL_GUARD_WORDS]);
 
 enum { RT_FRAME_FORMS_TESTED = 0, RT_FRAME_FORMS_FRAME_MISMATCHES = 1, RT_FRAME_FORMS_FRAME_SHORT = 2, RT_FRAME_FORMS_FRAME_PLAIN = 3,
        RT_FRAME_FORMS_RAY_MISMATCHES = 4, RT_FRAME_FORMS_RAY_SHORT = 5, RT_FRAME_FORMS_RAY_PLAIN = 6, RT_FRAME_FORMS_IN_USE = 7 };
diff --git a/raytracing-rust_amd/abi.py b/raytracing-rust_amd/abi.py
--- a/raytracing-rust_amd/abi.py
+++ b/raytracing-rust_amd/abi.py
@@ -18,6 +18,7 @@
 RT_LAYOUT_FRAME, RT_LAYOUT_SHARD = range(2)
 RT_TUNE_TRAVERSAL, RT_TUNE_FEATURE_SET, RT_TUNE_SCENE_IN_LDS, RT_TUNE_SCHEDULE, RT_TUNE_WALK, RT_TUNE_STACK_CAP, RT_TUNE_EXCHANGE, RT_TUNE_WHOLE_PIXEL_SHARE = range(8)
 RT_TUNE_RADIANCE_GROUPS = 8
+RT_TUNE_SKY_CELL = 11
 RT_TUNE_SKY_RUN = 10
 
 NO_INDEX = 0xFFFFFFFFFFFFFFFF
@@ -707,6 +708,7 @@
     "rt_selftest_short_forms",
     "rt_selftest_div_forms",
     "rt_selftest_sky_pdf_forms",
+    "rt_selftest_sky_cell",
     "rt_selftest_frame_forms",
     "rt_selftest_gen_keys",
     "rt_philox_round_keys",
diff --git a/raytracing-rust_amd/csrc/rt_api.cpp b/raytracing-rust_amd/csrc/rt_api.cpp
--- a/raytracing-rust_amd/csrc/rt_api.cpp
+++ b/raytracing-rust_amd/csrc/rt_api.cpp
@@ -310,6 +310,11 @@
 		if (!verified_reciprocal(RT_PI, &rc_pi) || !verified_reciprocal(RT_TAU, &rc_tau) || rc_pi != 1.0f / RT_PI || rc_tau != 1.0f / RT_TAU)
 			return bail(fail(RT_ERR_UNSUPPORTED, "self-check failed: division by pi / 2 pi through their reciprocals is not exact on this host (the kernels assume it)"));
 		sky_reciprocals(h.sky, &D.sky.inv_res_ok, &D.sky.inv_res_x, &D.sky.inv_res_y);
+		{
+			const SkyCellGuard g = sky_cell_guard(h.sky.sampler_res_x, h.sky.sampler_res_y, D.sky.inv_res_ok != 0u);
+			s->sky_cell_proven = g.ok;
+			s->sky_cell = DevSkyCell{g.ok, g.half_u, g.half_v, g.row_lo, g.row_span, {0u, 0u, 0u}};
+		}
 		bool tame = true;
 		for (const DevMaterial &m : h.materials) {
 			if (m.type != RT_MAT_LAMBERTIAN)
@@ -678,6 +683,11 @@
 			return fail(RT_ERR_INVALID_ARGUMENT, "sky run must be -1 (automatic), 0 (off) or 1 (on where the kernel has it)");
 		s->sky_run = value;
 		return RT_OK;
+	case RT_TUNE_SKY_CELL:
+		if (value < -1 || value > 1)
+			return fail(RT_ERR_INVALID_ARGUMENT, "sky cell must be -1 (automatic), 0 (off) or 1 (on where the guard is proven)");
+		s->sky_cell.ok = value != 0 ? s->sky_cell_proven : 0u;
+		return RT_OK;
 	default:
 		return fail(RT_ERR_INVALID_ARGUMENT, "unknown tuning key");
 	}
@@ -1384,7 +1394,7 @@
 	HIP_TRY(hipEventRecord(s->ev_start, stream));
 	HIP_TRY(launch_render(o->render_method, plan.prune, plan.fine, plan.sky_lds, plan.feature_set, plan.n_blocks, plan.lds_bytes, stream, plan.dev, cam, P,
 	                      render_target, reinterpret_cast<unsigned long long *>(d_rays_shot), s->d_work_counter, s->d_stack_ovf, plan.xchg,
-	                      plan.feature_set == 3 ? &s->pair : nullptr, plan.feature_set == 3 ? &primary : nullptr, plan.block_threads, sky_tiles));
+	                      plan.feature_set == 3 ? &s->pair : nullptr, plan.feature_set == 3 ? &primary : nullptr, plan.block_threads, sky_tiles, s->sky_cell));
 	HIP_TRY(hipEventRecord(s->ev_stop, stream));
 	if (plan.split > 1u)
 		HIP_TRY(launch_combine(stream, P, s->d_partial, d_out_rgb));
diff --git a/raytracing-rust_amd/csrc/rt_api_internal.h b/raytracing-rust_amd/csrc/rt_api_internal.h
--- a/raytracing-rust_amd/csrc/rt_api_internal.h
+++ b/raytracing-rust_amd/csrc/rt_api_internal.h
@@ -11,6 +11,7 @@
 #include "rt_layout.h"
 #include "rt_types.h"
 #include "rt_sky_tiles.h"
+#include "rt_sky_cell.h"
 
 extern thread_local std::string g_error;
 
@@ -76,6 +77,8 @@
 	int whole_share = kWholeShareDefault;
 	uint32_t radiance_groups = 0;
 	int sky_run = -1;
+	rt::DevSkyCell sky_cell = {};
+	uint32_t sky_cell_proven = 0;
 	uint32_t stack_depth_narrow = 2;
 	uint32_t *d_stack_ovf = nullptr;
 	size_t stack_ovf_words = 0;
diff --git a/raytracing-rust_amd/csrc/rt_api_query.cpp b/raytracing-rust_amd/csrc/rt_api_query.cpp
--- a/raytracing-rust_amd/csrc/rt_api_query.cpp
+++ b/raytracing-rust_amd/csrc/rt_api_query.cpp
@@ -410,6 +410,62 @@
 	return sky_finish(st, L, "selftest_sky_pdf_forms");
 }
 
+int rt_selftest_sky_cell(rt_scene *s, const uint32_t *cases, uint64_t n, uint32_t axis, uint32_t su, uint32_t sv, uint32_t *out, uint64_t counts[RT_SKY_CELL_COUNTS],
+                         uint32_t guard[RT_SKY_CELL_GUARD_WORDS])
+{
+	if (!s || !guard || (cases && (!out || n == 0 || n > (1ull << 20))))
+		return fail(RT_ERR_INVALID_ARGUMENT, "bad arguments (1 to 2^20 cases with their output, or no cases)");
+	const uint32_t rx = s->host.sky.sampler_res_x, ry = s->host.sky.sampler_res_y;
+	{
+		const SkyCellGuard g = sky_cell_guard(rx, ry, s->dev.sky.inv_res_ok != 0u);
+		const float du = (float)g.delta_u, dv = (float)g.delta_v;
+		std::memset(guard, 0, RT_SKY_CELL_GUARD_WORDS * sizeof(uint32_t));
+		guard[RT_SKY_CELL_GUARD_PROVEN] = g.ok;
+		guard[RT_SKY_CELL_GUARD_ENABLED] = s->sky_cell.ok;
+		std::memcpy(&guard[RT_SKY_CELL_GUARD_DELTA_U], &du, 4);
+		std::memcpy(&guard[RT_SKY_CELL_GUARD_DELTA_V], &dv, 4);
+		guard[RT_SKY_CELL_GUARD_ROW_LO] = g.row_lo;
+		guard[RT_SKY_CELL_GUARD_ROW_HI] = g.row_lo + g.row_span;
+		guard[RT_SKY_CELL_GUARD_IN_USE] = sky_cell_in_use() ? 1u : 0u;
+	}
+	if (!counts)
+		return cases ? fail(RT_ERR_INVALID_ARGUMENT, "bad arguments (cases need counts)") : RT_OK;
+	if ((rx | ry) == 0u)
+		return fail(RT_ERR_INVALID_ARGUMENT, "the sky is not samplable (sampler_res 0 x 0)");
+	if (!cases && (axis > 1u || su >= rx || sv >= ry))
+		return fail(RT_ERR_INVALID_ARGUMENT, "bad enumeration (axis 0 or 1, a cell of the table)");
+	if (rx >= kSkyCellMaxRes || ry >= kSkyCellMaxRes)
+		return fail(RT_ERR_UNSUPPORTED, "the cell word holds resolutions below 2^15");
+	for (uint64_t i = 0; cases && i < n; ++i) {
+		float r[2];
+		std::memcpy(r, cases + 4 * i + 2, sizeof r);
+		if (cases[4 * i] >= rx || cases[4 * i + 1] >= ry || !(r[0] >= 0.0f && r[0] < 1.0f && r[1] >= 0.0f && r[1] < 1.0f))
+			return fail(RT_ERR_INVALID_ARGUMENT, "bad case (a cell of the table, jitters in [0, 1))");
+	}
+	if (int rc = need_device(s); rc != RT_OK)
+		return rc;
+	const uint64_t n_run = cases ? n : 1ull << 24;
+	Layout L;
+	const auto p_counts = L.add<unsigned long long>(RT_SKY_CELL_COUNTS);
+	const auto p_cases = L.add<uint32_t>(cases ? 4 * n : 4), p_out = L.add<uint32_t>(cases ? RT_SKY_CELL_OUT_WORDS * n : 4);
+	RT_TRY(sky_buffer(s, L));
+	Staging st{s};
+	const unsigned long long zero[RT_SKY_CELL_COUNTS] = {};
+	unsigned long long host[RT_SKY_CELL_COUNTS] = {};
+	st.put(L, p_counts, zero);
+	if (cases)
+		st.put(L, p_cases, cases);
+	if (st.ok())
+		st.e = launch_sky_cell(s->stream, s->dev, s->sky_cell, cases ? L.at(p_cases) : nullptr, n_run, L.at(p_out), L.at(p_counts), axis, su, sv);
+	st.get(host, L, p_counts);
+	if (cases)
+		st.get(out, L, p_out);
+	const int rc = sky_finish(st, L, "selftest_sky_cell");
+	for (int k = 0; k < RT_SKY_CELL_COUNTS; ++k)
+		counts[k] = host[k];
+	return rc;
+}
+
 int rt_selftest_pair_shadow(int device, const float *cases, uint64_t n_cases, uint64_t counts[RT_PAIR_SHADOW_COUNTS])
 {
 	return run_case_table<RT_PAIR_SHADOW_COUNTS>(device, cases, n_cases, RT_PAIR_SHADOW_CASE_FLOATS * sizeof(float), counts, "selftest_pair_shadow",
diff --git a/raytracing-rust_amd/csrc/rt_lean.h b/raytracing-rust_amd/csrc/rt_lean.h
--- a/raytracing-rust_amd/csrc/rt_lean.h
+++ b/raytracing-rust_amd/csrc/rt_lean.h
@@ -88,6 +88,10 @@
 constexpr bool lean_gen_keys(bool pair) { return pair && RT_PAIR_GEN_KEYS != 0; }
 constexpr int lean_gen_keys_lead(bool pair) { return lean_gen_keys(pair) ? RT_PAIR_GEN_KEYS - 1 : 0; }
 constexpr bool lean_gen_item_product(bool pair) { return lean_gen_keys(pair) && RT_PAIR_GEN_ITEM_PRODUCT != 0; }
+#ifndef RT_PAIR_SKY_CELL
+#define RT_PAIR_SKY_CELL 1
+#endif
+constexpr bool lean_sky_cell(bool pair) { return pair && RT_PAIR_SKY_CELL != 0; }
 
 #if defined(__HIP_DEVICE_COMPILE__)
 
diff --git a/raytracing-rust_amd/csrc/rt_render.h b/raytracing-rust_amd/csrc/rt_render.h
--- a/raytracing-rust_amd/csrc/rt_render.h
+++ b/raytracing-rust_amd/csrc/rt_render.h
@@ -19,7 +19,7 @@
 hipError_t launch_render(int method, bool prune, bool fine, bool sky_lds, int feature_set, uint32_t n_blocks, size_t lds_bytes, hipStream_t stream,
                          const DevScene &S, const DevCamera &cam, const DevRenderParams &P, float *out,
                          unsigned long long *rays_shot, uint32_t *work_counter, uint32_t *stack_ovf, bool xchg, const DevPairScene *pair,
-                         const DevPairPrimary *primary, uint32_t block_threads, const DevSkyTiles &sky_tiles);
+                         const DevPairPrimary *primary, uint32_t block_threads, const DevSkyTiles &sky_tiles, const DevSkyCell &sky_cell);
 hipError_t launch_combine(hipStream_t stream, const DevRenderParams &P, const float *partial, float *out);
 hipError_t launch_scatter_shard(hipStream_t stream, const DevRenderParams &P, const float *shard, float *frame);
 hipError_t launch_sum_u64(hipStream_t stream, const unsigned long long *parts, uint32_t n, unsigned long long *out);
diff --git a/raytracing-rust_amd/csrc/rt_render.hip b/raytracing-rust_amd/csrc/rt_render.hip
--- a/raytracing-rust_amd/csrc/rt_render.hip
+++ b/raytracing-rust_amd/csrc/rt_render.hip
@@ -143,6 +143,7 @@
 	DevPairPrimary primary;
 	DevGenKeys gen_keys;
 	DevSkyTiles sky_tiles;
+	DevSkyCell sky_cell;
 };
 #if defined(__HIP_DEVICE_COMPILE__)
 typedef const __attribute__((address_space(4))) RenderArgs *KArgs;
@@ -332,6 +333,10 @@
 	PL.pdf_multiplier = 1.0f;
 	PL.t_limit = 0.0f;
 	PL.skip = kNoPrim;
+	constexpr bool kSkyCell = lean_sky_cell(F::pair);
+	static_assert(!kSkyCell || (!FINE && !XCHG), "the carried sky cell lives from do_light to do_scatter of ONE coarse iteration");
+	uint32_t light_sky_cell = 0u;
+	constexpr uint32_t kCellFromInv = (uint32_t)((offsetof(RenderArgs, sky_cell) - offsetof(RenderArgs, S) - offsetof(DevScene, sky) - offsetof(DevSky, inv_res_ok)) / 4u);
 	PL.have_shadow = PL.shadow_is_sky = false;
 
 	auto begin_walk = [&](bool shadow) {
@@ -493,6 +498,7 @@
 
 #ifdef RT_STATS
 	unsigned long long st_lane_nodes = 0, st_lane_prims = 0, st_lane_maxsp = 0, st_sky_samples = 0, st_sky_runs = 0, st_sky_clock = 0, st_allsky_clock = 0, st_allsky_iters = 0, st_iter_t0 = 0;
+	unsigned long long st_cell[4] = {};
 #endif
 	auto do_node = [&]() {
 #ifdef RT_STATS
@@ -706,7 +712,10 @@
 		g.type = g.material = 0u;
 		g.p0 = g.p1 = g.p2 = v3s(0.0f);
 		if (pick_sky) {
-			L.l_wi = sky_sample(S, T, rng);
+			if constexpr (kSkyCell)
+				L.l_wi = sky_sample_cell(S, T, rng, light_sky_cell, kCellFromInv);
+			else
+				L.l_wi = sky_sample(S, T, rng);
 			RT_SECTION(9);
 			L.t_limit = __uint_as_float(0x7FC00000u);
 			L.have_shadow = true;
@@ -747,7 +756,22 @@
 			float l_pdf = 0.0f;
 			if (L.shadow_is_sky) {
 				le = emission_of_hit<F>(S, PS, S.sky.material, true, hit, L.l_wi);
-				l_pdf = sky_pdf<F::pair>(S, T, L.l_wi) * L.pdf_multiplier;
+				if constexpr (kSkyCell) {
+#ifdef RT_STATS
+					{
+						const unsigned long long m_eval = __ballot(true), m_ok = __ballot((light_sky_cell >> 31) != 0u);
+						if (lane == (uint32_t)__builtin_ctzll(m_eval)) {
+							st_cell[0] += 1;
+							st_cell[1] += (unsigned long long)__popcll(m_eval);
+							st_cell[2] += (unsigned long long)__popcll(m_ok);
+							st_cell[3] += m_ok == m_eval ? 1ull : 0ull;
+						}
+					}
+#endif
+					l_pdf = sky_pdf_carried(S, T, L.l_wi, light_sky_cell) * L.pdf_multiplier;
+				} else {
+					l_pdf = sky_pdf<F::pair>(S, T, L.l_wi) * L.pdf_multiplier;
+				}
 				valid = true;
 			} else {
 				Hit lh;
@@ -1505,6 +1529,8 @@
 					L.pdf_multiplier = 1.0f;
 					L.t_limit = 0.0f;
 					L.skip = kNoPrim;
+					if constexpr (kSkyCell)
+						light_sky_cell = 0u;
 					L.have_shadow = L.shadow_is_sky = false;
 					Ray sray;
 					sray.o = sray.d = sray.inv = sray.shear = v3s(0.0f);
@@ -1565,6 +1591,8 @@
 	atomicAdd(&g_stats[20], st_lane_nodes);
 	atomicAdd(&g_stats[21], st_lane_prims);
 	atomicMax(&g_stats[22], st_lane_maxsp);
+	for (int k = 0; k < 4; ++k)
+		atomicAdd(&g_stats[32 + k], st_cell[k]);
 	if (lane == 0u) {
 		for (int k = 0; k < 9; ++k)
 			atomicAdd(&g_stats[40 + k], st_sect[k]);
@@ -1873,7 +1901,7 @@
 hipError_t launch_render(int method, bool prune, bool fine, bool sky_lds, int feature_set, uint32_t n_blocks, size_t lds_bytes, hipStream_t stream,
                          const DevScene &S, const DevCamera &cam, const DevRenderParams &P, float *out,
                          unsigned long long *rays_shot, uint32_t *work_counter, uint32_t *stack_ovf, bool xchg, const DevPairScene *pair,
-                         const DevPairPrimary *primary, uint32_t block_threads, const DevSkyTiles &sky_tiles)
+                         const DevPairPrimary *primary, uint32_t block_threads, const DevSkyTiles &sky_tiles, const DevSkyCell &sky_cell)
 {
 	render_fn fn = pick_render(method, prune, fine, sky_lds, feature_set, xchg);
 	if (!fn)
@@ -1888,6 +1916,7 @@
 	A.stack_ovf = stack_ovf;
 	A.pair = pair ? *pair : DevPairScene{};
 	A.primary = primary ? *primary : DevPairPrimary{};
+	A.sky_cell = sky_cell;
 	A.sky_tiles = sky_tiles;
 	philox_round_keys(((uint64_t)P.seed_hi << 32) | P.seed_lo, A.gen_keys);
 	hipLaunchKernelGGL(fn, dim3(n_blocks), dim3(block_threads ? block_threads : render_block_threads(feature_set, fine, xchg)), lds_bytes, stream, A);
diff --git a/raytracing-rust_amd/csrc/rt_selftest.h b/raytracing-rust_amd/csrc/rt_selftest.h
--- a/raytracing-rust_amd/csrc/rt_selftest.h
+++ b/raytracing-rust_amd/csrc/rt_selftest.h
@@ -53,6 +53,9 @@
 hipError_t launch_div_forms(hipStream_t stream, const DevDivForms &D);
 hipError_t launch_div_sites(hipStream_t stream, const float *operand_pairs, uint64_t n_pairs, unsigned long long *counts);
 hipError_t launch_sky_pdf_forms(hipStream_t stream, const DevScene &S, const float *dirs, uint64_t m, float *out_pair, float *out_default);
+hipError_t launch_sky_cell(hipStream_t stream, const DevScene &S, const DevSkyCell &guard, const uint32_t *cases, uint64_t n, uint32_t *out, unsigned long long *counts, uint32_t axis,
+                           uint32_t su, uint32_t sv);
+bool sky_cell_in_use();
 
 uint32_t frame_forms_in_use();
 hipError_t launch_frame_forms(hipStream_t stream, const float *vectors, uint64_t n_vectors, unsigned long long *counts);
diff --git a/raytracing-rust_amd/csrc/rt_selftest_forms.hip b/raytracing-rust_amd/csrc/rt_selftest_forms.hip
--- a/raytracing-rust_amd/csrc/rt_selftest_forms.hip
+++ b/raytracing-rust_amd/csrc/rt_selftest_forms.hip
@@ -297,6 +297,89 @@
 	return launch_cases(sky_pdf_forms_kernel, stream, m, 2048u, A);
 }
 
+struct SkyCellSelftestArgs {
+	DevScene S;
+	DevSkyCell guard;
+	const uint32_t *cases;
+	uint64_t n;
+	uint32_t *out;
+	unsigned long long *counts;
+	uint32_t axis, su, sv;
+};
+constexpr uint32_t kCellFromInv =
+    (uint32_t)((offsetof(SkyCellSelftestArgs, guard) - offsetof(SkyCellSelftestArgs, S) - offsetof(DevScene, sky) - offsetof(DevSky, inv_res_ok)) / 4u);
+__global__ __launch_bounds__(256) void sky_cell_kernel(const SkyCellSelftestArgs args_by_value)
+{
+#if defined(__HIP_DEVICE_COMPILE__)
+	const auto *A = (const __attribute__((address_space(4))) SkyCellSelftestArgs *)__builtin_amdgcn_kernarg_segment_ptr();
+	(void)args_by_value;
+#else
+	const SkyCellSelftestArgs *A = &args_by_value;
+#endif
+	const DevScene S = A->S;
+	SkyTables T;
+	T.row_cdf = S.sky.row_cdf;
+	T.marginal_cdf = S.sky.marginal_cdf;
+	T.guide = S.sky.guide;
+	T.guide_k = S.sky.guide_k;
+	T.inv_res = reinterpret_cast<KWords>(&A->S.sky.inv_res_ok);
+	const uint32_t *const cases = A->cases;
+	uint32_t *const out = A->out;
+	const uint32_t axis = A->axis, su0 = A->su, sv0 = A->sv;
+	Tally<RT_SKY_CELL_COUNTS> tally;
+	for_each_case(A->n, [&](uint64_t i) {
+		uint32_t su = su0, sv = sv0;
+		float r_u = 0.5f, r_v = 0.5f;
+		if (cases) {
+			su = cases[4u * i];
+			sv = cases[4u * i + 1u];
+			r_u = __uint_as_float(cases[4u * i + 2u]);
+			r_v = __uint_as_float(cases[4u * i + 3u]);
+		} else {
+			(axis == 0u ? r_u : r_v) = (float)(uint32_t)i * 0x1p-24f;
+		}
+		uint32_t cell, unused;
+		const float nu = next_float((float)su + r_u), nv = next_float((float)sv + r_v);
+		const V3 d = sky_direction_<true>(T, S.sky.res_x, S.sky.res_y, su, sv, r_u, r_v, nu, nv, cell, kCellFromInv);
+		const V3 d_default = sky_direction_<false>(T, S.sky.res_x, S.sky.res_y, su, sv, r_u, r_v, nu, nv, unused);
+		uint32_t ui, vi, rx, ry;
+		const float got = sky_pdf_carried_(S, T, d, cell, ui, vi);
+		const float want = sky_pdf<true>(S, T, d_default);
+		const SkyCell c = sky_pdf_cell<true>(S, d_default, rx, ry);
+		const bool guarded = (cell >> 31) != 0u, agree = c.ui == su && c.vi == sv;
+		tally.add(RT_SKY_CELL_GUARDED_DISAGREE, guarded && !agree);
+		tally.add(RT_SKY_CELL_UNGUARDED, !guarded);
+		tally.add(RT_SKY_CELL_UNGUARDED_AGREE, !guarded && agree);
+		tally.add(RT_SKY_CELL_PDF_MISMATCHES, !same_f32(got, want));
+		tally.add(RT_SKY_CELL_TESTED);
+		if (cases) {
+			uint32_t *o = out + RT_SKY_CELL_OUT_WORDS * i;
+			o[0] = __float_as_uint(got);
+			o[1] = __float_as_uint(want);
+			const bool reads = sqrt_unit_(1.0f - d_default.z * d_default.z) > 0.0f;
+			o[2] = reads ? ui | vi << 16 | (cell & 0x80000000u) : RT_SKY_CELL_NO_CELL | (cell & 0x80000000u);
+			o[3] = reads ? c.ui | c.vi << 16 : RT_SKY_CELL_NO_CELL;
+		}
+	});
+	tally.flush(A->counts);
+}
+hipError_t launch_sky_cell(hipStream_t stream, const DevScene &S, const DevSkyCell &guard, const uint32_t *cases, uint64_t n, uint32_t *out, unsigned long long *counts, uint32_t axis,
+                           uint32_t su, uint32_t sv)
+{
+	SkyCellSelftestArgs A;
+	A.S = S;
+	A.guard = guard;
+	A.cases = cases;
+	A.n = n;
+	A.out = out;
+	A.counts = counts;
+	A.axis = axis;
+	A.su = su;
+	A.sv = sv;
+	return launch_cases(sky_cell_kernel, stream, n, 2048u, A);
+}
+bool sky_cell_in_use() { return lean_sky_cell(true); }
+
 __device__ __noinline__ Coord coord_from_z_plain(V3 z) { return coord_from_z(z); }
 __device__ __forceinline__ Coord pair_kernels_frame(V3 z)
 {
diff --git a/raytracing-rust_amd/csrc/rt_shade.h b/raytracing-rust_amd/csrc/rt_shade.h
--- a/raytracing-rust_amd/csrc/rt_shade.h
+++ b/raytracing-rust_amd/csrc/rt_shade.h
@@ -336,35 +336,47 @@
 
 __device__ __forceinline__ bool sky_can_sample(const DevScene &S) { return (S.sky.res_x | S.sky.res_y) != 0u; }
 
-template <bool SHORT = false> __device__ __forceinline__ float sky_pdf(const DevScene &S, const SkyTables &T, V3 wi)
-{
-	const float sin_theta = sqrt_unit_(1.0f - wi.z * wi.z);
-	if (sin_theta <= 0.0f)
-		return 0.0f;
+struct SkyCell {
+	uint32_t ui, vi;
+};
+template <bool SHORT = false> __device__ __forceinline__ SkyCell sky_pdf_cell(const DevScene &S, V3 wi, uint32_t &rx, uint32_t &ry)
+{
 	const float theta = lean_acos_dev(wi.z);
 	float phi = SHORT ? lean_atan2_for<true>(wi.y, wi.x) : lean_atan2(wi.y, wi.x);
 	if (phi < 0.0f)
 		phi += 2.0f * kPi;
 	const float u = div_by_verified(phi, kTau, kRcpTau);
 	const float v = div_by_verified(theta, kPi, kRcpPi);
-	const uint32_t rx = here_(S.sky.res_x), ry = here_(S.sky.res_y);
-	uint32_t ui = f32_as_index((float)rx * u);
-	uint32_t vi = f32_as_index((float)ry * v);
-	ui = ui > rx - 1u ? rx - 1u : ui;
-	vi = vi > ry - 1u ? ry - 1u : vi;
+	rx = here_(S.sky.res_x);
+	ry = here_(S.sky.res_y);
+	SkyCell c;
+	c.ui = f32_as_index((float)rx * u);
+	c.vi = f32_as_index((float)ry * v);
+	c.ui = c.ui > rx - 1u ? rx - 1u : c.ui;
+	c.vi = c.vi > ry - 1u ? ry - 1u : c.vi;
+	return c;
+}
+__device__ __forceinline__ float sky_pdf_from_cell(const SkyTables &T, uint32_t ui, uint32_t vi, uint32_t rx, uint32_t ry, float sin_theta)
+{
 	const float ypdf = T.marginal_cdf[vi + 1u] - T.marginal_cdf[vi];
 	const float *row = T.row_cdf + (size_t)vi * (rx + 1u);
 	const float xpdf = row[ui + 1u] - row[ui];
 	return (float)rx * (float)ry * (ypdf * xpdf) / (sin_theta * kTau * kPi);
 }
-
-__device__ __forceinline__ V3 sky_sample(const DevScene &S, const SkyTables &T, rt_rng &rng)
-{
-	const uint32_t rx = here_(S.sky.res_x), ry = here_(S.sky.res_y);
-	const bool guided = T.guide_k != 0u;
-	const uint32_t sv = dist1d_sample(T.marginal_cdf, ry, guided ? T.guide + (size_t)ry * T.guide_k : nullptr, T.guide_k, rng);
-	const uint32_t su = dist1d_sample(T.row_cdf + (size_t)sv * (rx + 1u), rx, guided ? T.guide + (size_t)sv * T.guide_k : nullptr, T.guide_k, rng);
-	const float nu = next_float((float)su + rt_rng_f32(&rng)), nv = next_float((float)sv + rt_rng_f32(&rng));
+template <bool SHORT = false> __device__ __forceinline__ float sky_pdf(const DevScene &S, const SkyTables &T, V3 wi)
+{
+	const float sin_theta = sqrt_unit_(1.0f - wi.z * wi.z);
+	if (sin_theta <= 0.0f)
+		return 0.0f;
+	uint32_t rx, ry;
+	const SkyCell c = sky_pdf_cell<SHORT>(S, wi, rx, ry);
+	return sky_pdf_from_cell(T, c.ui, c.vi, rx, ry, sin_theta);
+}
+
+template <bool CELL>
+__device__ __forceinline__ V3 sky_direction_(const SkyTables &T, uint32_t rx, uint32_t ry, uint32_t su, uint32_t sv, float r_u, float r_v, float nu, float nv,
+                                             uint32_t &cell, uint32_t cell_from_inv = 0u)
+{
 	float u, v;
 	KWords inv = T.inv_res;
 #if defined(__HIP_DEVICE_COMPILE__)
@@ -373,9 +385,17 @@
 	if (inv != nullptr && inv[0] != 0u) {
 		u = div_by_verified(nu, (float)rx, __uint_as_float(inv[1]));
 		v = div_by_verified(nv, (float)ry, __uint_as_float(inv[2]));
+		if constexpr (CELL) {
+			const KWords g = inv + cell_from_inv;
+			const bool in_u = fabsf(r_u - 0.5f) <= __uint_as_float(g[1]), in_v = fabsf(r_v - 0.5f) <= __uint_as_float(g[2]);
+			const bool in_rows = sv - g[3] <= g[4];
+			cell = su | sv << 16 | (((g[0] != 0u) & in_u & in_v & in_rows) ? 0x80000000u : 0u);
+		}
 	} else {
 		u = nu / (float)rx;
 		v = nv / (float)ry;
+		if constexpr (CELL)
+			cell = su | sv << 16;
 	}
 	const float phi = u * 2.0f * kPi;
 	const float theta = v * kPi;
@@ -383,6 +403,56 @@
 	lean_sincos(theta, st, ct);
 	lean_sincos(phi, sp, cp);
 	return v3(st * cp, st * sp, ct);
+}
+template <bool CELL> __device__ __forceinline__ V3 sky_sample_(const DevScene &S, const SkyTables &T, rt_rng &rng, uint32_t &cell, uint32_t cell_from_inv = 0u)
+{
+	const uint32_t rx = here_(S.sky.res_x), ry = here_(S.sky.res_y);
+	const bool guided = T.guide_k != 0u;
+	const uint32_t sv = dist1d_sample(T.marginal_cdf, ry, guided ? T.guide + (size_t)ry * T.guide_k : nullptr, T.guide_k, rng);
+	const uint32_t su = dist1d_sample(T.row_cdf + (size_t)sv * (rx + 1u), rx, guided ? T.guide + (size_t)sv * T.guide_k : nullptr, T.guide_k, rng);
+	const float f_u = (float)su;
+	const float r_u = rt_rng_f32(&rng);
+	const float nu = next_float(f_u + r_u);
+	const float f_v = (float)sv;
+	const float r_v = rt_rng_f32(&rng);
+	const float nv = next_float(f_v + r_v);
+	return sky_direction_<CELL>(T, rx, ry, su, sv, r_u, r_v, nu, nv, cell, cell_from_inv);
+}
+__device__ __forceinline__ V3 sky_sample(const DevScene &S, const SkyTables &T, rt_rng &rng)
+{
+	uint32_t unused;
+	return sky_sample_<false>(S, T, rng, unused);
+}
+__device__ __forceinline__ V3 sky_sample_cell(const DevScene &S, const SkyTables &T, rt_rng &rng, uint32_t &cell, uint32_t cell_from_inv)
+{
+	return sky_sample_<true>(S, T, rng, cell, cell_from_inv);
+}
+
+__device__ __forceinline__ float sky_pdf_carried_(const DevScene &S, const SkyTables &T, V3 wi, uint32_t cell, uint32_t &ui, uint32_t &vi)
+{
+	ui = cell & 0x7FFFu;
+	vi = (cell >> 16) & 0x7FFFu;
+	const float sin_theta = sqrt_unit_(1.0f - wi.z * wi.z);
+	if (sin_theta <= 0.0f)
+		return 0.0f;
+#if defined(__HIP_DEVICE_COMPILE__)
+	const bool guarded = (cell >> 31) != 0u;
+	if (__ballot(!guarded) != 0ull) {
+		if (!guarded) {
+			uint32_t rx_, ry_;
+			const SkyCell c = sky_pdf_cell<true>(S, wi, rx_, ry_);
+			ui = c.ui;
+			vi = c.vi;
+		}
+	}
+#endif
+	const uint32_t rx = here_(S.sky.res_x), ry = here_(S.sky.res_y);
+	return sky_pdf_from_cell(T, ui, vi, rx, ry, sin_theta);
+}
+__device__ __forceinline__ float sky_pdf_carried(const DevScene &S, const SkyTables &T, V3 wi, uint32_t cell)
+{
+	uint32_t ui, vi;
+	return sky_pdf_carried_(S, T, wi, cell, ui, vi);
 }
 
 __device__ __forceinline__ V3 lambertian_sample(V3 normal, rt_rng &rng)
diff --git a/raytracing-rust_amd/csrc/rt_sky_cell.h b/raytracing-rust_amd/csrc/rt_sky_cell.h
--- /dev/null
+++ b/raytracing-rust_amd/csrc/rt_sky_cell.h
@@ -0,0 +1,49 @@
+#pragma once
+#include <cmath>
+#include <cstdint>
+
+namespace rt {
+
+struct SkyCellGuard {
+	uint32_t ok;
+	float half_u, half_v;
+	uint32_t row_lo, row_span;
+	double e_u, e_v;
+	double delta_u, delta_v;
+	double s_edge;
+};
+
+constexpr double kSkyCellSafety = 2.0;
+constexpr double kSkyCellOutward = 1.0 + 0x1p-30;
+constexpr uint32_t kSkyCellMaxRes = 1u << 15;
+
+inline SkyCellGuard sky_cell_guard(uint32_t rx, uint32_t ry, bool reciprocals_verified)
+{
+	SkyCellGuard g = {};
+	if (!reciprocals_verified || rx == 0u || ry < 3u || rx >= kSkyCellMaxRes || ry >= kSkyCellMaxRes)
+		return g;
+	const double e = 0x1p-24, pi = 3.14159265358979323846, k_pi = (double)3.14159274101257324219f;
+	const uint32_t row_lo = 1u, row_hi = ry - 2u;
+	const double s_lo = std::sin(k_pi * row_lo / ry), s_hi = std::sin(pi - k_pi * (row_hi + 1u) / ry);
+	const double s_edge = std::fmin(s_lo, s_hi) / kSkyCellOutward;
+	if (!(s_edge >= 0x1p-8))
+		return g;
+	const double e_v = ((double)ry * (12.0 * e) + ((double)ry / pi) * (4.0 * e + 0x1p-45) / s_edge) * kSkyCellOutward;
+	const double e_u = ((double)rx * (7.0 * e) + ((double)rx / (2.0 * pi)) * (40.0 * e + 0x1p-44)) * kSkyCellOutward;
+	const double d_u = std::ceil(kSkyCellSafety * e_u * 0x1p24) * e, d_v = std::ceil(kSkyCellSafety * e_v * 0x1p24) * e;
+	g.e_u = e_u;
+	g.e_v = e_v;
+	g.delta_u = d_u;
+	g.delta_v = d_v;
+	g.s_edge = s_edge;
+	if (!(d_u < 0.25 && d_v < 0.25))
+		return g;
+	g.half_u = (float)(0.5 - d_u);
+	g.half_v = (float)(0.5 - d_v);
+	g.row_lo = row_lo;
+	g.row_span = row_hi - row_lo;
+	g.ok = 1u;
+	return g;
+}
+
+}
diff --git a/raytracing-rust_amd/csrc/rt_types.h b/raytracing-rust_amd/csrc/rt_types.h
--- a/raytracing-rust_amd/csrc/rt_types.h
+++ b/raytracing-rust_amd/csrc/rt_types.h
@@ -105,6 +105,13 @@
 	uint32_t inv_res_ok;
 	float inv_res_x, inv_res_y;
 };
+struct DevSkyCell {
+	uint32_t ok;
+	float half_u, half_v;
+	uint32_t row_lo, row_span;
+	uint32_t pad[3];
+};
+static_assert(sizeof(DevSkyCell) == 32, "DevSkyCell: eight words");
 
 struct DevScene {
 	const DevNode *nodes;
diff --git a/raytracing-rust_amd/hip_backend.py b/raytracing-rust_amd/hip_backend.py
--- a/raytracing-rust_amd/hip_backend.py
+++ b/raytracing-rust_amd/hip_backend.py
@@ -212,6 +212,35 @@
     return a, b
 
 
+SKY_CELL_COUNT_NAMES = ("guarded_disagree", "unguarded", "unguarded_agree", "pdf_mismatches", "tested")
+
+
+def sky_cell_guard(scene):
+    guard = np.zeros(8, dtype=np.uint32)
+    _check(lib().rt_selftest_sky_cell(scene._h, None, C.c_uint64(0), C.c_uint32(0), C.c_uint32(0), C.c_uint32(0), None, None, _p(guard, C.c_uint32)))
+    return _sky_cell_guard_dict(guard)
+
+
+def _sky_cell_guard_dict(guard):
+    return {"proven": bool(guard[0]), "enabled": bool(guard[1]), "delta_u": float(guard[2:3].view(np.float32)[0]), "delta_v": float(guard[3:4].view(np.float32)[0]),
+            "row_lo": int(guard[4]), "row_hi": int(guard[5]), "in_use": bool(guard[6])}
+
+
+def selftest_sky_cell(scene, cases=None, *, axis=0, su=0, sv=0):
+    counts, guard = (C.c_uint64 * 5)(), np.zeros(8, dtype=np.uint32)
+    out = None
+    if cases is not None:
+        cases = np.ascontiguousarray(cases, dtype=np.uint32)
+        if cases.ndim != 2 or cases.shape[1] != 4:
+            raise ValueError(f"cases must be (n, 4), got {cases.shape}")
+        out = np.zeros((cases.shape[0], 4), dtype=np.uint32)
+        _check(lib().rt_selftest_sky_cell(scene._h, _p(cases, C.c_uint32), C.c_uint64(cases.shape[0]), C.c_uint32(0), C.c_uint32(0), C.c_uint32(0),
+                                          _p(out, C.c_uint32), counts, _p(guard, C.c_uint32)))
+    else:
+        _check(lib().rt_selftest_sky_cell(scene._h, None, C.c_uint64(0), C.c_uint32(axis), C.c_uint32(su), C.c_uint32(sv), None, counts, _p(guard, C.c_uint32)))
+    return out, dict(zip(SKY_CELL_COUNT_NAMES, (int(x) for x in counts))), _sky_cell_guard_dict(guard)
+
+
 def selftest_frame_forms(vectors, device=0):
     return _selftest_cases("frame_forms", vectors, device)
 
```

After: 44840 (median of 6 runs). +4.3%, better.
